# zzzzxxxx111/Rover-SLAM

Hardware: AMD Instinct MI355X
Metric: frames/s SuperPoint+LightGlue 640x480 (higher is better)
Workload: dtype f32; 1 GPU; configs[3] per GPU: 33 synthetic 640x480 u8 frames resident in HBM, SuperPoint extract (Kmax=1024, thr=0.0005) + LightGlue match of 32 consecutive pairs (9 layers, filter 0.1); 32 frames counted per GPU per step; seeded synthetic weights (centred descriptor head + calibrated LightGlue law, frames shifted by multiples of 8 px); the same resident frames every step (compute-bound path, no data-depend; frames_per_gpu=32, kmax=1024, lg_fold_wo=1, pairing=calibrated

## Files before the change

### include/rover_fe.h

```cpp
#ifndef ROVER_FE_H
#define ROVER_FE_H
#include <stddef.h>
#include <stdint.h>

#ifdef __cplusplus
extern "C" {
#endif

typedef struct rfe_ctx rfe_ctx;

typedef enum {
    RFE_OK = 0,
    RFE_ERR_INVALID = -1,
    RFE_ERR_NO_DEVICE = -2,
    RFE_ERR_HIP = -3,
    RFE_ERR_IO = -4,
    RFE_ERR_NO_WEIGHTS = -5,
    RFE_ERR_OOM = -6
} rfe_status;

#define RFE_DESC_DIM 256
#define RFE_KIND_SUPERPOINT 1
#define RFE_KIND_LIGHTGLUE 2

int rfe_init(int device, rfe_ctx** out);
void rfe_destroy(rfe_ctx* ctx);
const char* rfe_last_error(rfe_ctx* ctx);
const char* rfe_version(void);

int rfe_load_weights(rfe_ctx* ctx, const char* sp_path, const char* lg_path);
int rfe_load_onnx(rfe_ctx* ctx, const char* sp_path, const char* lg_path);
int rfe_set_weights(rfe_ctx* ctx, int kind, const float* blob, int64_t count);
int64_t rfe_weight_count(int kind);
uint64_t rfe_weights_id(rfe_ctx* ctx, int kind);

typedef struct rfe_hparams {
    int32_t sp_max_keypoints;
    float sp_detection_threshold;
    int32_t sp_nms_radius;
    int32_t sp_remove_borders;
    int32_t sp_topk_always;
    int32_t lg_layers;
    int32_t lg_heads;
    float lg_filter_threshold;
} rfe_hparams;
int rfe_get_hparams(rfe_ctx* ctx, rfe_hparams* out);
int rfe_set_hparams(rfe_ctx* ctx, const rfe_hparams* in);

#define RFE_OPT_LG_FOLD_WO 1
#define RFE_OPT_LG_FP16X2 2
#define RFE_OPT_HOST_GRAPH 3
int rfe_set_option(rfe_ctx* ctx, int option, int value);
int rfe_get_option(rfe_ctx* ctx, int option, int* value);

int rfe_set_stream(rfe_ctx* ctx, void* hip_stream);
int rfe_synchronize(rfe_ctx* ctx);
int rfe_malloc(rfe_ctx* ctx, size_t bytes, void** dev_ptr);
int rfe_free(rfe_ctx* ctx, void* dev_ptr);
int rfe_host_malloc(size_t bytes, void** host_ptr);
void rfe_host_free(void* host_ptr);
int64_t rfe_workspace_bytes(rfe_ctx* ctx);
int rfe_memcpy_h2d(rfe_ctx* ctx, void* dst_dev, const void* src_host, size_t bytes);
int rfe_memcpy_d2h(rfe_ctx* ctx, void* dst_host, const void* src_dev, size_t bytes);

int rfe_extract_u8(rfe_ctx* ctx, const uint8_t* img, int H, int W, int stride, int B, int Kmax,
                   float thr, int32_t* n, int32_t* kxy, float* score, float* desc);
int rfe_extract_u8_dev(rfe_ctx* ctx, const uint8_t* img_dev, int H, int W, int stride, int B,
                       int Kmax, float thr, int32_t* n_dev, int32_t* kxy_dev, float* score_dev,
                       float* desc_dev);

int rfe_extract_f32(rfe_ctx* ctx, const float* img, int H, int W, int stride, int B, int Kmax,
                    float thr, int32_t* n, int32_t* kxy, float* score, float* desc);
int rfe_extract_f32_dev(rfe_ctx* ctx, const float* img_dev, int H, int W, int stride, int B,
                        int Kmax, float thr, int32_t* n_dev, int32_t* kxy_dev, float* score_dev,
                        float* desc_dev);

int rfe_extract_u8_bin(rfe_ctx* ctx, const uint8_t* img, int H, int W, int stride, int B, int Kmax, float thr, int32_t* n,
                       int32_t* kxy, float* score, float* desc, uint8_t* desc_bin);
int rfe_extract_u8_bin_dev(rfe_ctx* ctx, const uint8_t* img_dev, int H, int W, int stride, int B, int Kmax, float thr,
                           int32_t* n_dev, int32_t* kxy_dev, float* score_dev, float* desc_dev, uint8_t* desc_bin_dev);

#define RFE_MAX_LEVELS 16
int rfe_pyramid_geometry(int H, int W, int nlevels, float scale_factor, int32_t* level_h, int32_t* level_w, float* level_scale);
int rfe_extract_pyramid_u8(rfe_ctx* ctx, const uint8_t* img, int H, int W, int stride, int B, int nlevels, float scale_factor,
                           const int32_t* kmax, float thr, int32_t* n, int32_t* level_n, float* kpts, int32_t* octave,
                           float* score, float* desc, uint8_t* levels);
int rfe_extract_pyramid_u8_dev(rfe_ctx* ctx, const uint8_t* img_dev, int H, int W, int stride, int B, int nlevels, float scale_factor,
                               const int32_t* kmax, float thr, int32_t* n_dev, int32_t* level_n_dev, float* kpts_dev,
                               int32_t* octave_dev, float* score_dev, float* desc_dev, uint8_t* levels_dev);

int rfe_match(rfe_ctx* ctx, const float* k0n, const float* k1n, const float* d0, const float* d1,
              const int32_t* m, const int32_t* n, int P, int Mmax, int Nmax, float filter_thr,
              int32_t* S, int32_t* pairs, float* ms);
int rfe_match_dev(rfe_ctx* ctx, const float* k0n, const float* k1n, const float* d0,
                  const float* d1, const int32_t* m, const int32_t* n, int P, int Mmax, int Nmax,
                  float filter_thr, int32_t* S, int32_t* pairs, float* ms);

int rfe_match_fused(rfe_ctx* ctx, const float* kpts0_xy, int M, const float* kpts1_xy, int N,
                    const float* desc0, const float* desc1, int rows, int cols, float filter_thr,
                    float match_thresh, int32_t* vnMatches12);

int rfe_extract_match_stream_dev(rfe_ctx* ctx, const uint8_t* img_dev, int H, int W, int stride,
                                 int B, int Kmax, float thr, float filter_thr, int32_t* n_dev,
                                 int32_t* kxy_dev, float* score_dev, float* desc_dev,
                                 int32_t* S_dev, int32_t* pairs_dev, float* ms_dev);

int rfe_stereo_match(rfe_ctx* ctx, const uint8_t* imgL, const uint8_t* imgR, int H, int W, int stride,
                     const float* kL, int N, const float* kR, int Nr, const float* dL, const float* dR,
                     float mb, float mbf, float* uRight, float* depth);
int rfe_stereo_match_dev(rfe_ctx* ctx, const uint8_t* imgL, const uint8_t* imgR, int H, int W, int stride,
                         const float* kL, int N, const float* kR, int Nr, const float* dL, const float* dR,
                         float mb, float mbf, float* uRight, float* depth);

int rfe_stereo_frame_dev(rfe_ctx* ctx, const uint8_t* imgL_dev, const uint8_t* imgR_dev, int H, int W, int stride, int Kmax,
                         float thr, float filter_thr, float mb, float mbf, int reset, int32_t* n_dev, int32_t* kxy_dev,
                         float* score_dev, float* desc_dev, float* uRight_dev, float* depth_dev, int32_t* S_dev,
                         int32_t* pairs_dev, float* ms_dev);

#define RFE_STEREO_SAD_LEVEL  0
#define RFE_STEREO_SAD_LEVEL0 1
int rfe_stereo_match_pyramid(rfe_ctx* ctx, const uint8_t* levelsL, const uint8_t* levelsR, int H, int W, int nlevels, float scale_factor,
                             const float* kL, const int32_t* octL, int N, const float* kR, const int32_t* octR, int Nr,
                             const float* dL, const float* dR, float mb, float mbf, int sad_source, float* uRight, float* depth);
int rfe_stereo_match_pyramid_dev(rfe_ctx* ctx, const uint8_t* levelsL, const uint8_t* levelsR, int H, int W, int nlevels, float scale_factor,
                                 const float* kL, const int32_t* octL, int N, const float* kR, const int32_t* octR, int Nr,
                                 const float* dL, const float* dR, float mb, float mbf, int sad_source, float* uRight, float* depth);
int rfe_stereo_frame_pyramid_dev(rfe_ctx* ctx, const uint8_t* imgL_dev, const uint8_t* imgR_dev, int H, int W, int stride,
                                 int nlevels, float scale_factor, const int32_t* kmax, float thr, float filter_thr, float mb, float mbf,
                                 int sad_source, int reset, int32_t* n_dev, int32_t* level_n_dev, float* kpts_dev, int32_t* octave_dev,
                                 float* score_dev, float* desc_dev, float* uRight_dev, float* depth_dev, int32_t* S_dev,
                                 int32_t* pairs_dev, float* ms_dev);

int rfe_l2_distance_matrix(rfe_ctx* ctx, const float* a, int M, const float* b, int N, float* out);
int rfe_binarize_descriptors(rfe_ctx* ctx, const float* desc, int rows, uint8_t* out);

int rfe_search_candidates(rfe_ctx* ctx, const float* q, int Nq, const float* f, int Nf, const int32_t* offsets,
                          const int32_t* cand, const uint8_t* skip, int32_t* best_idx, float* best_dist, float* second_dist);
int rfe_distinctive_descriptors(rfe_ctx* ctx, const float* desc, const int32_t* offsets, int Np, int32_t* best, float* median);

int rfe_l2_distance_matrix_dev(rfe_ctx* ctx, const float* a_dev, int M, const float* b_dev, int N, float* out_dev);
int rfe_binarize_descriptors_dev(rfe_ctx* ctx, const float* desc_dev, int rows, uint8_t* out_dev);
int rfe_search_candidates_dev(rfe_ctx* ctx, const float* q_dev, int Nq, const float* f_dev, int Nf, const int32_t* offsets_dev,
                              const int32_t* cand_dev, const uint8_t* skip_dev, int32_t* best_idx_dev, float* best_dist_dev,
                              float* second_dist_dev);
int rfe_distinctive_descriptors_dev(rfe_ctx* ctx, const float* desc_dev, const int32_t* offsets_dev, int Np, int total, int maxn,
                                    int32_t* best_dev, float* median_dev);

int rfe_search_by_projection_dev(rfe_ctx* ctx, const float* q_dev, const float* proj_dev, const float* radius_dev,
                                 const int32_t* pred_level_dev, const uint8_t* observed_dev, int Nq, const float* f_dev,
                                 const float* kpts_dev, const int32_t* kxy_dev, const int32_t* octave_dev, const uint8_t* skip_dev, int Nf,
                                 const int32_t* nf_dev, float min_x, float min_y, float max_x, float max_y, float th_high, int cand_cap,
                                 int32_t* assign_dev, int32_t* best_idx_dev, float* best_dist_dev, float* second_dist_dev,
                                 int32_t* stats_dev);
int rfe_search_by_projection(rfe_ctx* ctx, const float* q, const float* proj, const float* radius, const int32_t* pred_level,
                             const uint8_t* observed, int Nq, const float* f, const float* kpts, const int32_t* kxy, const int32_t* octave,
                             const uint8_t* skip, int Nf, float min_x, float min_y, float max_x, float max_y, float th_high,
                             int32_t* assign, int32_t* best_idx, float* best_dist, float* second_dist, int32_t* stats);

typedef struct rfe_pool rfe_pool;
#define RFE_POOL_AUTO 0
#define RFE_POOL_RCCL 1
#define RFE_POOL_COPY 2
int rfe_pool_create(const int* devices, int n, rfe_pool** out);
void rfe_pool_destroy(rfe_pool* pool);
const char* rfe_pool_last_error(rfe_pool* pool);
int rfe_pool_size(rfe_pool* pool);
rfe_ctx* rfe_pool_ctx(rfe_pool* pool, int member);
int rfe_pool_has_rccl(rfe_pool* pool);
int rfe_pool_set_weights(rfe_pool* pool, int kind, const float* blob, int64_t count);
int rfe_pool_load_weights(rfe_pool* pool, const char* sp_path, const char* lg_path);
int rfe_pool_set_option(rfe_pool* pool, int option, int value);
int rfe_pool_set_hparams(rfe_pool* pool, const rfe_hparams* in);
int rfe_pool_shard(int F, int n, int member, int* first_frame, int* frames, int* pairs);
int rfe_pool_extract_match_stream(rfe_pool* pool, const uint8_t* img_host, int H, int W, int stride, int F, int Kmax, float thr,
                                  float filter_thr, int transport, int32_t* n, int32_t* kxy, float* score, float* desc,
                                  int32_t* S, int32_t* pairs, float* ms);

int rfe_profile_enable(rfe_ctx* ctx, int on);
int rfe_profile_filter(rfe_ctx* ctx, const char* stage);
int rfe_profile_reset(rfe_ctx* ctx);
int rfe_profile_read(rfe_ctx* ctx, char* names, size_t names_cap, double* ms, int64_t* calls, int cap);

int rfe_k_conv3x3(rfe_ctx* ctx, const float* in_dev, int B, int H, int W, int Cin,
                  const float* w_oihw_host, const float* bias_host, int Cout, int relu, int pool,
                  float* out_dev);
int rfe_k_linear(rfe_ctx* ctx, const float* a_dev, int M, int K, const float* w_nk_host,
                 const float* bias_host, int N, int relu, float* out_dev);
int rfe_k_scoremap(rfe_ctx* ctx, const uint8_t* img_dev, int H, int W, int stride, int B,
                   float* scoremap_dev ,
                   float* nms_dev , float* descmap_dev );
int rfe_k_select(rfe_ctx* ctx, const float* nms_dev , int B, int H, int W, int Kmax, float thr, int topk_always,
                 int32_t* n_dev, int32_t* kxy_dev, float* score_dev);
int rfe_k_select_keys(rfe_ctx* ctx, const float* nms_dev , int B, int H, int W, int Kmax, float thr, int topk_always,
                      int32_t* n_dev, int32_t* kxy_dev, float* score_dev);
int rfe_k_lightglue_taps(rfe_ctx* ctx, const float* k0n, const float* k1n, const float* d0,
                         const float* d1, int M, int N, float* x0_dev, float* x1_dev,
                         float* scores_dev );

int rfe_k_lightglue_ffn(rfe_ctx* ctx, int layer, int cross, const float* x_dev, const float* second_dev, int rows, float* out_dev);
int rfe_k_attention(rfe_ctx* ctx, const float* q_dev, const float* k_dev, const float* v_dev, int ld, float* out_dev, int nseq, int Lq, int Lk,
                    const int32_t* qlen_dev, const int32_t* klen_dev, const int32_t* kv_map_dev, const float* rope_dev);
int rfe_k_lightglue_self_attention(rfe_ctx* ctx, int layer, const float* x_dev, const float* csn_dev, const int32_t* lens_dev, int nseq, int L,
                                   float* qkv_out_dev, float* ctx_out_dev, int32_t* qk_rotated);
int rfe_k_set_lightglue_tap(rfe_ctx* ctx, int pair, float* x0_dev, float* x1_dev, float* scores_dev);
int rfe_k_pool_inject_gather_failure(rfe_pool* pool, int member);
int rfe_k_onnx_convert(const char* path, int kind, int weights_only, float* blob, rfe_hparams* hp, char* err, int errlen);

#ifdef __cplusplus
}
#endif
#endif
```

### rover-slam_amd/capi.py

```python
import ctypes as C
import os

import numpy as np

_HERE = os.path.dirname(os.path.abspath(__file__))
LIB_PATH = os.environ.get("RFE_LIBRARY") or os.path.join(_HERE, "librover_fe.so")

KIND_SUPERPOINT, KIND_LIGHTGLUE = 1, 2
OPT_LG_FOLD_WO = 1
OPT_LG_FP16X2 = 2
OPT_HOST_GRAPH = 3

EXPORTS = [
    "rfe_init", "rfe_destroy", "rfe_last_error", "rfe_version", "rfe_load_weights", "rfe_load_onnx", "rfe_set_weights",
    "rfe_weight_count", "rfe_weights_id", "rfe_get_hparams", "rfe_set_hparams", "rfe_set_option", "rfe_get_option", "rfe_set_stream", "rfe_synchronize", "rfe_malloc", "rfe_free", "rfe_host_malloc", "rfe_host_free", "rfe_workspace_bytes", "rfe_memcpy_h2d",
    "rfe_memcpy_d2h", "rfe_extract_u8", "rfe_extract_u8_dev", "rfe_extract_f32", "rfe_extract_f32_dev", "rfe_extract_u8_bin", "rfe_extract_u8_bin_dev",
    "rfe_pyramid_geometry", "rfe_extract_pyramid_u8", "rfe_extract_pyramid_u8_dev", "rfe_match", "rfe_match_dev", "rfe_match_fused",
    "rfe_extract_match_stream_dev", "rfe_stereo_match", "rfe_stereo_match_dev", "rfe_stereo_frame_dev", "rfe_stereo_match_pyramid", "rfe_stereo_match_pyramid_dev", "rfe_stereo_frame_pyramid_dev",
    "rfe_l2_distance_matrix", "rfe_binarize_descriptors",
    "rfe_search_candidates", "rfe_distinctive_descriptors",
    "rfe_l2_distance_matrix_dev", "rfe_binarize_descriptors_dev", "rfe_search_candidates_dev", "rfe_distinctive_descriptors_dev",
    "rfe_search_by_projection", "rfe_search_by_projection_dev",
    "rfe_pool_create", "rfe_pool_destroy", "rfe_pool_last_error", "rfe_pool_size", "rfe_pool_ctx", "rfe_pool_has_rccl", "rfe_pool_set_weights",
    "rfe_pool_load_weights", "rfe_pool_set_option", "rfe_pool_set_hparams", "rfe_pool_shard", "rfe_pool_extract_match_stream",
    "rfe_profile_enable", "rfe_profile_filter", "rfe_profile_reset", "rfe_profile_read",
    "rfe_k_conv3x3", "rfe_k_linear", "rfe_k_scoremap", "rfe_k_select", "rfe_k_select_keys", "rfe_k_lightglue_taps", "rfe_k_set_lightglue_tap", "rfe_k_lightglue_ffn", "rfe_k_attention", "rfe_k_lightglue_self_attention", "rfe_k_pool_inject_gather_failure", "rfe_k_onnx_convert",
]

if not os.path.exists(LIB_PATH):
    raise ImportError(f"{LIB_PATH} is missing: build it with `python -c 'import __graft_entry__ as g; g.build()'` "
                      "(rover-slam_amd/csrc/Makefile). There is no CPU fallback.")

lib = C.CDLL(LIB_PATH)

_vp, _fp, _ip, _u8p = C.c_void_p, C.c_void_p, C.c_void_p, C.c_void_p
lib.rfe_init.argtypes = [C.c_int, C.POINTER(C.c_void_p)]
lib.rfe_destroy.argtypes = [C.c_void_p]
lib.rfe_destroy.restype = None
lib.rfe_last_error.argtypes = [C.c_void_p]
lib.rfe_last_error.restype = C.c_char_p
lib.rfe_version.restype = C.c_char_p
lib.rfe_load_weights.argtypes = [C.c_void_p, C.c_char_p, C.c_char_p]
lib.rfe_set_weights.argtypes = [C.c_void_p, C.c_int, _fp, C.c_int64]
lib.rfe_weight_count.argtypes = [C.c_int]
lib.rfe_weight_count.restype = C.c_int64
lib.rfe_weights_id.restype = C.c_uint64
lib.rfe_weights_id.argtypes = [C.c_void_p, C.c_int]


class HParams(C.Structure):
    _fields_ = [("sp_max_keypoints", C.c_int32), ("sp_detection_threshold", C.c_float), ("sp_nms_radius", C.c_int32),
                ("sp_remove_borders", C.c_int32), ("sp_topk_always", C.c_int32), ("lg_layers", C.c_int32), ("lg_heads", C.c_int32), ("lg_filter_threshold", C.c_float)]

    def as_dict(self):
        return {k: getattr(self, k) for k, _ in self._fields_}


lib.rfe_get_hparams.argtypes = [C.c_void_p, C.POINTER(HParams)]
lib.rfe_set_hparams.argtypes = [C.c_void_p, C.POINTER(HParams)]
lib.rfe_pool_set_hparams.argtypes = [C.c_void_p, C.POINTER(HParams)]
lib.rfe_set_option.argtypes = [C.c_void_p, C.c_int, C.c_int]
lib.rfe_get_option.argtypes = [C.c_void_p, C.c_int, C.POINTER(C.c_int)]
lib.rfe_set_stream.argtypes = [C.c_void_p, C.c_void_p]
lib.rfe_synchronize.argtypes = [C.c_void_p]
lib.rfe_malloc.argtypes = [C.c_void_p, C.c_size_t, C.POINTER(C.c_void_p)]
lib.rfe_free.argtypes = [C.c_void_p, C.c_void_p]
lib.rfe_memcpy_h2d.argtypes = [C.c_void_p, C.c_void_p, C.c_void_p, C.c_size_t]
lib.rfe_memcpy_d2h.argtypes = [C.c_void_p, C.c_void_p, C.c_void_p, C.c_size_t]
_ext = [C.c_void_p, _u8p, C.c_int, C.c_int, C.c_int, C.c_int, C.c_int, C.c_float, _ip, _ip, _fp, _fp]
lib.rfe_extract_u8.argtypes = _ext
lib.rfe_extract_f32.argtypes = _ext
lib.rfe_extract_f32_dev.argtypes = _ext
lib.rfe_extract_u8_dev.argtypes = _ext
lib.rfe_extract_u8_bin.argtypes = _ext + [_u8p]
lib.rfe_extract_u8_bin_dev.argtypes = _ext + [_u8p]
lib.rfe_pyramid_geometry.argtypes = [C.c_int, C.c_int, C.c_int, C.c_float, _ip, _ip, _fp]
_pyr = [C.c_void_p, _u8p, C.c_int, C.c_int, C.c_int, C.c_int, C.c_int, C.c_float, _ip, C.c_float, _ip, _ip, _fp, _ip, _fp, _fp, _u8p]
lib.rfe_extract_pyramid_u8.argtypes = _pyr
lib.rfe_extract_pyramid_u8_dev.argtypes = _pyr
_mt = [C.c_void_p, _fp, _fp, _fp, _fp, _ip, _ip, C.c_int, C.c_int, C.c_int, C.c_float, _ip, _ip, _fp]
lib.rfe_match.argtypes = _mt
lib.rfe_match_dev.argtypes = _mt
lib.rfe_match_fused.argtypes = [C.c_void_p, _fp, C.c_int, _fp, C.c_int, _fp, _fp, C.c_int, C.c_int, C.c_float,
                                C.c_float, _ip]
lib.rfe_extract_match_stream_dev.argtypes = [C.c_void_p, _u8p, C.c_int, C.c_int, C.c_int, C.c_int, C.c_int, C.c_float,
                                             C.c_float, _ip, _ip, _fp, _fp, _ip, _ip, _fp]
_st = [C.c_void_p, _u8p, _u8p, C.c_int, C.c_int, C.c_int, _fp, C.c_int, _fp, C.c_int, _fp, _fp, C.c_float, C.c_float, _fp, _fp]
lib.rfe_stereo_match.argtypes = _st
lib.rfe_stereo_match_dev.argtypes = _st
lib.rfe_stereo_frame_dev.argtypes = [C.c_void_p, _u8p, _u8p, C.c_int, C.c_int, C.c_int, C.c_int, C.c_float, C.c_float, C.c_float, C.c_float,
                                     C.c_int, _ip, _ip, _fp, _fp, _fp, _fp, _ip, _ip, _fp]
_stp = [C.c_void_p, _u8p, _u8p, C.c_int, C.c_int, C.c_int, C.c_float, _fp, _ip, C.c_int, _fp, _ip, C.c_int, _fp, _fp, C.c_float, C.c_float,
        C.c_int, _fp, _fp]
lib.rfe_stereo_match_pyramid.argtypes = _stp
lib.rfe_stereo_match_pyramid_dev.argtypes = _stp
lib.rfe_stereo_frame_pyramid_dev.argtypes = [C.c_void_p, _u8p, _u8p, C.c_int, C.c_int, C.c_int, C.c_int, C.c_float, _ip, C.c_float, C.c_float,
                                             C.c_float, C.c_float, C.c_int, C.c_int, _ip, _ip, _fp, _ip, _fp, _fp, _fp, _fp, _ip, _ip, _fp]
lib.rfe_l2_distance_matrix.argtypes = [C.c_void_p, _fp, C.c_int, _fp, C.c_int, _fp]
lib.rfe_binarize_descriptors.argtypes = [C.c_void_p, _fp, C.c_int, _u8p]
lib.rfe_search_candidates.argtypes = [C.c_void_p, _fp, C.c_int, _fp, C.c_int, _ip, _ip, _u8p, _ip, _fp, _fp]
lib.rfe_distinctive_descriptors.argtypes = [C.c_void_p, _fp, _ip, C.c_int, _ip, _fp]
lib.rfe_l2_distance_matrix_dev.argtypes = [C.c_void_p, _fp, C.c_int, _fp, C.c_int, _fp]
lib.rfe_binarize_descriptors_dev.argtypes = [C.c_void_p, _fp, C.c_int, _u8p]
lib.rfe_search_candidates_dev.argtypes = [C.c_void_p, _fp, C.c_int, _fp, C.c_int, _ip, _ip, _u8p, _ip, _fp, _fp]
lib.rfe_distinctive_descriptors_dev.argtypes = [C.c_void_p, _fp, _ip, C.c_int, C.c_int, C.c_int, _ip, _fp]
_psq = [C.c_void_p, _fp, _fp, _fp, _ip, _u8p, C.c_int, _fp, _fp, _ip, _ip, _u8p, C.c_int]
_psb = [C.c_float, C.c_float, C.c_float, C.c_float, C.c_float]
lib.rfe_search_by_projection.argtypes = _psq + _psb + [_ip, _ip, _fp, _fp, _ip]
lib.rfe_search_by_projection_dev.argtypes = _psq + [_ip] + _psb + [C.c_int, _ip, _ip, _fp, _fp, _ip]
lib.rfe_profile_enable.argtypes = [C.c_void_p, C.c_int]
lib.rfe_profile_filter.argtypes = [C.c_void_p, C.c_char_p]
lib.rfe_profile_reset.argtypes = [C.c_void_p]
lib.rfe_profile_read.argtypes = [C.c_void_p, C.c_char_p, C.c_size_t, C.POINTER(C.c_double), C.POINTER(C.c_int64), C.c_int]
lib.rfe_k_conv3x3.argtypes = [C.c_void_p, _fp, C.c_int, C.c_int, C.c_int, C.c_int, _fp, _fp, C.c_int, C.c_int, C.c_int, _fp]
lib.rfe_k_linear.argtypes = [C.c_void_p, _fp, C.c_int, C.c_int, _fp, _fp, C.c_int, C.c_int, _fp]
lib.rfe_k_scoremap.argtypes = [C.c_void_p, _u8p, C.c_int, C.c_int, C.c_int, C.c_int, _fp, _fp, _fp]
lib.rfe_k_select.argtypes = [C.c_void_p, _fp, C.c_int, C.c_int, C.c_int, C.c_int, C.c_float, C.c_int, _ip, _ip, _fp]
lib.rfe_k_select_keys.argtypes = lib.rfe_k_select.argtypes
lib.rfe_k_lightglue_taps.argtypes = [C.c_void_p, _fp, _fp, _fp, _fp, C.c_int, C.c_int, _fp, _fp, _fp]
lib.rfe_k_set_lightglue_tap.argtypes = [C.c_void_p, C.c_int, _fp, _fp, _fp]
lib.rfe_k_lightglue_ffn.argtypes = [C.c_void_p, C.c_int, C.c_int, _fp, _fp, C.c_int, _fp]
lib.rfe_k_lightglue_self_attention.argtypes = [C.c_void_p, C.c_int, _fp, _fp, C.c_void_p, C.c_int, C.c_int, _fp, _fp, C.POINTER(C.c_int32)]
lib.rfe_k_attention.argtypes = [C.c_void_p, _fp, _fp, _fp, C.c_int, _fp, C.c_int, C.c_int, C.c_int, C.c_void_p, C.c_void_p, C.c_void_p, _fp]


POOL_AUTO, POOL_RCCL, POOL_COPY = 0, 1, 2
lib.rfe_pool_create.argtypes = [C.POINTER(C.c_int), C.c_int, C.POINTER(C.c_void_p)]
lib.rfe_pool_destroy.argtypes = [C.c_void_p]
lib.rfe_pool_destroy.restype = None
lib.rfe_pool_last_error.argtypes = [C.c_void_p]
lib.rfe_pool_last_error.restype = C.c_char_p
lib.rfe_pool_size.argtypes = [C.c_void_p]
lib.rfe_pool_ctx.argtypes = [C.c_void_p, C.c_int]
lib.rfe_pool_ctx.restype = C.c_void_p
lib.rfe_pool_has_rccl.argtypes = [C.c_void_p]
lib.rfe_k_pool_inject_gather_failure.argtypes = [C.c_void_p, C.c_int]
lib.rfe_load_onnx.argtypes = [C.c_void_p, C.c_char_p, C.c_char_p]
lib.rfe_k_onnx_convert.argtypes = [C.c_char_p, C.c_int, C.c_int, C.POINTER(C.c_float), C.c_void_p, C.c_char_p, C.c_int]
lib.rfe_host_malloc.argtypes = [C.c_size_t, C.POINTER(C.c_void_p)]
lib.rfe_host_free.argtypes = [C.c_void_p]
lib.rfe_host_free.restype = None
lib.rfe_workspace_bytes.argtypes = [C.c_void_p]
lib.rfe_workspace_bytes.restype = C.c_int64
lib.rfe_pool_set_weights.argtypes = [C.c_void_p, C.c_int, _fp, C.c_int64]
lib.rfe_pool_load_weights.argtypes = [C.c_void_p, C.c_char_p, C.c_char_p]
lib.rfe_pool_set_option.argtypes = [C.c_void_p, C.c_int, C.c_int]
lib.rfe_pool_shard.argtypes = [C.c_int, C.c_int, C.c_int, C.POINTER(C.c_int), C.POINTER(C.c_int), C.POINTER(C.c_int)]
lib.rfe_pool_extract_match_stream.argtypes = [C.c_void_p, _u8p, C.c_int, C.c_int, C.c_int, C.c_int, C.c_int, C.c_float, C.c_float, C.c_int,
                                              _ip, _ip, _fp, _fp, _ip, _ip, _fp]


class RfeError(RuntimeError):
    pass


def _addr(a):
    if a is None:
        return None
    if isinstance(a, int):
        return a
    if isinstance(a, np.ndarray):
        assert a.flags["C_CONTIGUOUS"]
        return a.ctypes.data
    if hasattr(a, "data_ptr"):
        return a.data_ptr()
    raise TypeError(type(a))


class DevBuf:

    def __init__(self, ctx, nbytes):
        self.ctx, self.nbytes = ctx, int(nbytes)
        p = C.c_void_p()
        ctx._chk(lib.rfe_malloc(ctx.h, self.nbytes, C.byref(p)))
        self.ptr = p.value

    def upload(self, arr):
        arr = np.ascontiguousarray(arr)
        assert arr.nbytes <= self.nbytes
        self.ctx._chk(lib.rfe_memcpy_h2d(self.ctx.h, self.ptr, arr.ctypes.data, arr.nbytes))
        return self

    def download(self, shape, dtype):
        out = np.empty(shape, dtype)
        assert out.nbytes <= self.nbytes
        self.ctx._chk(lib.rfe_memcpy_d2h(self.ctx.h, out.ctypes.data, self.ptr, out.nbytes))
        return out

    def free(self):
        if self.ptr:
            lib.rfe_free(self.ctx.h, self.ptr)
            self.ptr = None


def split_levels(flat, level_h, level_w):
    out, off = [], 0
    for h, w in zip(level_h, level_w):
        out.append(flat[:, off:off + int(h) * int(w)].reshape(flat.shape[0], int(h), int(w)))
        off += int(h) * int(w)
    return out


class StereoStream:

    def __init__(self, ctx, H, W, kmax=1024, mb=0.11, mbf=0.11 * 435.0, thr=0.0005, filter_thr=0.1):
        self.ctx, self.H, self.W, self.K = ctx, H, W, kmax
        self.mb, self.mbf, self.thr, self.filter_thr = mb, mbf, thr, filter_thr
        K = kmax
        self._spec = [("n", np.int32, (2,)), ("kxy", np.int32, (2, K, 2)), ("score", np.float32, (2, K)), ("desc", np.float32, (2, K, 256)),
                      ("u_right", np.float32, (K,)), ("depth", np.float32, (K,)), ("S", np.int32, (1,)), ("pairs", np.int32, (K, 2)),
                      ("ms", np.float32, (K,))]
        self.bufs = {name: ctx.alloc(int(np.prod(shape)) * np.dtype(dt).itemsize) for name, dt, shape in self._spec}
        self.first = True

    def push(self, img_l_dev, img_r_dev, stride=None, reset=False):
        b = self.bufs
        self.ctx._chk(lib.rfe_stereo_frame_dev(self.ctx.h, _addr(img_l_dev), _addr(img_r_dev), self.H, self.W, stride or self.W, self.K,
                                               self.thr, self.filter_thr, self.mb, self.mbf, int(reset or self.first), b["n"].ptr,
                                               b["kxy"].ptr, b["score"].ptr, b["desc"].ptr, b["u_right"].ptr, b["depth"].ptr,
                                               b["S"].ptr, b["pairs"].ptr, b["ms"].ptr))
        self.first = False

    def results(self):
        self.ctx.synchronize()
        out = {name: self.bufs[name].download(shape, dt) for name, dt, shape in self._spec}
        out["S"] = int(out["S"][0])
        return out

    def close(self):
        for b in self.bufs.values():
            b.free()
        self.bufs = {}


STEREO_SAD_LEVEL, STEREO_SAD_LEVEL0 = 0, 1


class StereoPyramidStream:

    def __init__(self, ctx, H, W, nlevels=8, scale_factor=1.2, kmax=128, mb=0.11, mbf=0.11 * 435.0, thr=0.0005, filter_thr=0.1,
                 sad_source=STEREO_SAD_LEVEL):
        self.ctx, self.H, self.W, self.L, self.sf = ctx, H, W, int(nlevels), scale_factor
        self.kmax = np.full((max(self.L, 1),), int(kmax), np.int32) if np.isscalar(kmax) else np.ascontiguousarray(kmax, np.int32)
        self.mb, self.mbf, self.thr, self.filter_thr, self.sad_source = mb, mbf, thr, filter_thr, sad_source
        K = self.K = int(self.kmax.sum())
        self._spec = [("n", np.int32, (2,)), ("level_n", np.int32, (2, max(self.L, 1))), ("kpts", np.float32, (2, K, 2)),
                      ("octave", np.int32, (2, K)), ("score", np.float32, (2, K)), ("desc", np.float32, (2, K, 256)),
                      ("u_right", np.float32, (K,)), ("depth", np.float32, (K,)), ("S", np.int32, (1,)), ("pairs", np.int32, (K, 2)),
                      ("ms", np.float32, (K,))]
        self.bufs = {name: ctx.alloc(max(int(np.prod(shape)), 1) * np.dtype(dt).itemsize) for name, dt, shape in self._spec}
        self.first = True

    def push(self, img_l_dev, img_r_dev, stride=None, reset=False):
        b = self.bufs
        self.ctx._chk(lib.rfe_stereo_frame_pyramid_dev(self.ctx.h, _addr(img_l_dev), _addr(img_r_dev), self.H, self.W, stride or self.W, self.L,
                                                       self.sf, self.kmax.ctypes.data, self.thr, self.filter_thr, self.mb, self.mbf,
                                                       self.sad_source, int(reset or self.first), b["n"].ptr, b["level_n"].ptr, b["kpts"].ptr,
                                                       b["octave"].ptr, b["score"].ptr, b["desc"].ptr, b["u_right"].ptr, b["depth"].ptr,
                                                       b["S"].ptr, b["pairs"].ptr, b["ms"].ptr))
        self.first = False

    def results(self):
        self.ctx.synchronize()
        out = {name: self.bufs[name].download(shape, dt) for name, dt, shape in self._spec}
        out["S"] = int(out["S"][0])
        return out

    def close(self):
        for b in self.bufs.values():
            b.free()
        self.bufs = {}


MAX_LEVELS = 16


def pyramid_geometry(H, W, nlevels, scale_factor):
    L = max(int(nlevels), 1)
    h, w, s = np.zeros((L,), np.int32), np.zeros((L,), np.int32), np.zeros((L,), np.float32)
    rc = lib.rfe_pyramid_geometry(H, W, nlevels, scale_factor, h.ctypes.data, w.ctypes.data, s.ctypes.data)
    if rc < 0:
        raise RfeError(f"rfe_pyramid_geometry({H}, {W}, {nlevels}, {scale_factor}) failed ({rc})")
    return h, w, s


def pool_shard(F, n, member):
    a, b, c = C.c_int(), C.c_int(), C.c_int()
    rc = lib.rfe_pool_shard(F, n, member, C.byref(a), C.byref(b), C.byref(c))
    if rc < 0:
        raise RfeError(f"rfe_pool_shard({F}, {n}, {member}) failed ({rc})")
    return a.value, b.value, c.value


class Pool:

    def __init__(self, devices):
        devs = (C.c_int * len(devices))(*devices)
        h = C.c_void_p()
        rc = lib.rfe_pool_create(devs, len(devices), C.byref(h))
        if rc != 0:
            raise RfeError(f"rfe_pool_create failed ({rc}): {lib.rfe_pool_last_error(None).decode()}")
        self.h = h

    def close(self):
        if self.h:
            lib.rfe_pool_destroy(self.h)
            self.h = None

    def __del__(self):
        try:
            self.close()
        except Exception:
            pass

    def _chk(self, rc):
        if rc < 0:
            raise RfeError(f"librover_fe pool error {rc}: {lib.rfe_pool_last_error(self.h).decode()}")
        return rc

    @property
    def size(self):
        return lib.rfe_pool_size(self.h)

    @property
    def has_rccl(self):
        return bool(lib.rfe_pool_has_rccl(self.h))

    def set_weights(self, kind, blob):
        blob = np.ascontiguousarray(blob, np.float32)
        self._chk(lib.rfe_pool_set_weights(self.h, kind, blob.ctypes.data, blob.size))

    def set_option(self, option, value):
        self._chk(lib.rfe_pool_set_option(self.h, option, int(value)))

    def set_hparams(self, **kw):
        h = HParams()
        rc = lib.rfe_get_hparams(lib.rfe_pool_ctx(self.h, 0), C.byref(h))
        if rc < 0:
            raise RfeError(f"rfe_get_hparams on pool member 0 failed ({rc})")
        for k, v in kw.items():
            if not hasattr(h, k):
                raise KeyError(k)
            setattr(h, k, v)
        self._chk(lib.rfe_pool_set_hparams(self.h, C.byref(h)))

    def extract_match_stream(self, frames_u8, kmax=1024, thr=0.0005, filter_thr=0.1, transport=POOL_AUTO, with_desc=True):
        img = np.ascontiguousarray(frames_u8, np.uint8)
        F, H, W = img.shape
        P = max(F - 1, 1)
        out = {"n": np.zeros((F,), np.int32), "kxy": np.zeros((F, kmax, 2), np.int32), "S": np.zeros((P,), np.int32),
               "pairs": np.zeros((P, kmax, 2), np.int32), "ms": np.zeros((P, kmax), np.float32)}
        if with_desc:
            out["score"] = np.zeros((F, kmax), np.float32)
            out["desc"] = np.zeros((F, kmax, 256), np.float32)
        self._chk(lib.rfe_pool_extract_match_stream(self.h, img.ctypes.data, H, W, W, F, kmax, thr, filter_thr, transport, out["n"].ctypes.data,
                                                    out["kxy"].ctypes.data, out["score"].ctypes.data if with_desc else None,
                                                    out["desc"].ctypes.data if with_desc else None, out["S"].ctypes.data,
                                                    out["pairs"].ctypes.data, out["ms"].ctypes.data))
        return out


class Context:

    def __init__(self, device=0):
        h = C.c_void_p()
        rc = lib.rfe_init(device, C.byref(h))
        if rc != 0:
            raise RfeError(f"rfe_init failed ({rc}): {lib.rfe_last_error(None).decode()}")
        self.h = h

    def close(self):
        if self.h:
            lib.rfe_destroy(self.h)
            self.h = None

    def __del__(self):
        try:
            self.close()
        except Exception:
            pass

    def _chk(self, rc):
        if rc < 0:
            raise RfeError(f"librover_fe error {rc}: {lib.rfe_last_error(self.h).decode()}")
        return rc

    def set_weights(self, kind, blob):
        blob = np.ascontiguousarray(blob, np.float32)
        self._chk(lib.rfe_set_weights(self.h, kind, blob.ctypes.data, blob.size))

    def load_weights(self, sp_path=None, lg_path=None):
        self._chk(lib.rfe_load_weights(self.h, sp_path.encode() if sp_path else None, lg_path.encode() if lg_path else None))

    def get_hparams(self):
        h = HParams()
        self._chk(lib.rfe_get_hparams(self.h, C.byref(h)))
        return h.as_dict()

    def set_hparams(self, **kw):
        h = HParams()
        self._chk(lib.rfe_get_hparams(self.h, C.byref(h)))
        for k, v in kw.items():
            if not hasattr(h, k):
                raise KeyError(k)
            setattr(h, k, v)
        self._chk(lib.rfe_set_hparams(self.h, C.byref(h)))

    def set_option(self, option, value):
        self._chk(lib.rfe_set_option(self.h, option, int(value)))

    def get_option(self, option):
        v = C.c_int()
        self._chk(lib.rfe_get_option(self.h, option, C.byref(v)))
        return v.value

    def set_stream(self, stream_ptr):
        self._chk(lib.rfe_set_stream(self.h, stream_ptr))

    def workspace_bytes(self):
        return int(lib.rfe_workspace_bytes(self.h))

    def synchronize(self):
        self._chk(lib.rfe_synchronize(self.h))

    def alloc(self, nbytes):
        return DevBuf(self, nbytes)

    def extract(self, img_u8, kmax=1024, thr=0.0005, pad_cols=0, binarized=False):
        img = np.ascontiguousarray(img_u8, np.uint8)
        if img.ndim == 2:
            img = img[None]
        B, H, W = img.shape
        stride = W + pad_cols
        if pad_cols:
            wide = np.full((B, H, stride), 255, np.uint8)
            wide[:, :, :W] = img
            img = wide
        n = np.zeros((B,), np.int32)
        kxy = np.zeros((B, kmax, 2), np.int32)
        score = np.zeros((B, kmax), np.float32)
        desc = np.zeros((B, kmax, 256), np.float32)
        if binarized:
            dbin = np.zeros((B, kmax, 256), np.uint8)
            self._chk(lib.rfe_extract_u8_bin(self.h, img.ctypes.data, H, W, stride, B, kmax, thr, n.ctypes.data, kxy.ctypes.data,
                                             score.ctypes.data, desc.ctypes.data, dbin.ctypes.data))
            return n, kxy, score, desc, dbin
        self._chk(lib.rfe_extract_u8(self.h, img.ctypes.data, H, W, stride, B, kmax, thr, n.ctypes.data, kxy.ctypes.data,
                                     score.ctypes.data, desc.ctypes.data))
        return n, kxy, score, desc

    def extract_pyramid(self, frames_u8, nlevels=8, scale_factor=1.2, kmax=1024, thr=0.0005, with_levels=False, pad_cols=0):
        img = np.ascontiguousarray(frames_u8, np.uint8)
        if img.ndim == 2:
            img = img[None]
        B, H, W = img.shape
        stride = W + pad_cols
        if pad_cols:
            wide = np.full((B, H, stride), 255, np.uint8)
            wide[:, :, :W] = img
            img = wide
        L = int(nlevels)
        km = np.full((max(L, 1),), int(kmax), np.int32) if np.isscalar(kmax) else np.ascontiguousarray(kmax, np.int32)
        K = int(km.sum())
        out = {"n": np.zeros((B,), np.int32), "level_n": np.zeros((B, max(L, 1)), np.int32), "kpts": np.zeros((B, K, 2), np.float32),
               "octave": np.zeros((B, K), np.int32), "score": np.zeros((B, K), np.float32), "desc": np.zeros((B, K, 256), np.float32)}
        lv = None
        if with_levels:
            lh, lw, _ = pyramid_geometry(H, W, L, scale_factor)
            lv = np.zeros((B, int((lh.astype(np.int64) * lw).sum())), np.uint8)
        self._chk(lib.rfe_extract_pyramid_u8(self.h, img.ctypes.data, H, W, stride, B, L, scale_factor, km.ctypes.data, thr,
                                             out["n"].ctypes.data, out["level_n"].ctypes.data, out["kpts"].ctypes.data,
                                             out["octave"].ctypes.data, out["score"].ctypes.data, out["desc"].ctypes.data,
                                             None if lv is None else lv.ctypes.data))
        if with_levels:
            out["levels"] = split_levels(lv, lh, lw)
        return out

    def extract_f32(self, img_f32, kmax=1024, thr=0.0005):
        img = np.ascontiguousarray(img_f32, np.float32)
        if img.ndim == 2:
            img = img[None]
        B, H, W = img.shape
        n = np.zeros((B,), np.int32)
        kxy = np.zeros((B, kmax, 2), np.int32)
        score = np.zeros((B, kmax), np.float32)
        desc = np.zeros((B, kmax, 256), np.float32)
        self._chk(lib.rfe_extract_f32(self.h, img.ctypes.data, H, W, W, B, kmax, thr, n.ctypes.data, kxy.ctypes.data,
                                      score.ctypes.data, desc.ctypes.data))
        return n, kxy, score, desc

    def match(self, k0n, k1n, d0, d1, m, n, filter_thr=0.1):
        k0n = np.ascontiguousarray(k0n, np.float32); k1n = np.ascontiguousarray(k1n, np.float32)
        d0 = np.ascontiguousarray(d0, np.float32); d1 = np.ascontiguousarray(d1, np.float32)
        m = np.ascontiguousarray(m, np.int32); n = np.ascontiguousarray(n, np.int32)
        P, Mmax = k0n.shape[0], k0n.shape[1]
        Nmax = k1n.shape[1]
        cap = min(Mmax, Nmax)
        S = np.zeros((P,), np.int32)
        pairs = np.zeros((P, cap, 2), np.int32)
        ms = np.zeros((P, cap), np.float32)
        self._chk(lib.rfe_match(self.h, k0n.ctypes.data, k1n.ctypes.data, d0.ctypes.data, d1.ctypes.data, m.ctypes.data,
                                n.ctypes.data, P, Mmax, Nmax, filter_thr, S.ctypes.data, pairs.ctypes.data, ms.ctypes.data))
        return S, pairs, ms

    def match_fused(self, kpts0, kpts1, desc0, desc1, rows, cols, filter_thr=0.1, match_thresh=0.0):
        kpts0 = np.ascontiguousarray(kpts0, np.float32).reshape(-1, 2)
        kpts1 = np.ascontiguousarray(kpts1, np.float32).reshape(-1, 2)
        desc0 = np.ascontiguousarray(desc0, np.float32); desc1 = np.ascontiguousarray(desc1, np.float32)
        M, N = kpts0.shape[0], kpts1.shape[0]
        vn = np.full((max(M, 1),), -1, np.int32)
        size = self._chk(lib.rfe_match_fused(self.h, kpts0.ctypes.data, M, kpts1.ctypes.data, N, desc0.ctypes.data,
                                             desc1.ctypes.data, rows, cols, filter_thr, match_thresh, vn.ctypes.data))
        return size, vn[:M]

    def stereo_match(self, img_l, img_r, k_l, k_r, d_l, d_r, mb, mbf):
        il = np.ascontiguousarray(img_l, np.uint8); ir = np.ascontiguousarray(img_r, np.uint8)
        kl = np.ascontiguousarray(k_l, np.float32).reshape(-1, 2); kr = np.ascontiguousarray(k_r, np.float32).reshape(-1, 2)
        dl = np.ascontiguousarray(d_l, np.float32); dr = np.ascontiguousarray(d_r, np.float32)
        H, W = il.shape
        N, Nr = kl.shape[0], kr.shape[0]
        u = np.full((max(N, 1),), -1, np.float32); z = np.full((max(N, 1),), -1, np.float32)
        self._chk(lib.rfe_stereo_match(self.h, il.ctypes.data, ir.ctypes.data, H, W, W, kl.ctypes.data, N, kr.ctypes.data, Nr,
                                       dl.ctypes.data, dr.ctypes.data, mb, mbf, u.ctypes.data, z.ctypes.data))
        return u[:N], z[:N]

    def stereo_match_pyramid(self, levels_l, levels_r, H, W, nlevels, scale_factor, k_l, oct_l, k_r, oct_r, d_l, d_r, mb, mbf, sad_source=0):
        def flat(lv):
            if isinstance(lv, (list, tuple)):
                return np.concatenate([np.ascontiguousarray(a, np.uint8).reshape(-1) for a in lv])
            return np.ascontiguousarray(lv, np.uint8).reshape(-1)
        vl, vr = flat(levels_l), flat(levels_r)
        lh, lw, _ = pyramid_geometry(H, W, nlevels, scale_factor)
        need = int((lh.astype(np.int64) * lw).sum())
        if vl.size != need or vr.size != need:
            raise RfeError(f"stereo_match_pyramid: level buffers hold {vl.size} / {vr.size} bytes, the geometry needs {need}")
        kl = np.ascontiguousarray(k_l, np.float32).reshape(-1, 2); kr = np.ascontiguousarray(k_r, np.float32).reshape(-1, 2)
        ol = np.ascontiguousarray(oct_l, np.int32).reshape(-1); orr = np.ascontiguousarray(oct_r, np.int32).reshape(-1)
        dl = np.ascontiguousarray(d_l, np.float32).reshape(-1, 256); dr = np.ascontiguousarray(d_r, np.float32).reshape(-1, 256)
        N, Nr = kl.shape[0], kr.shape[0]
        assert ol.shape[0] == N and orr.shape[0] == Nr and dl.shape[0] == N and dr.shape[0] == Nr
        u = np.full((max(N, 1),), -1, np.float32); z = np.full((max(N, 1),), -1, np.float32)
        self._chk(lib.rfe_stereo_match_pyramid(self.h, vl.ctypes.data, vr.ctypes.data, H, W, nlevels, scale_factor, kl.ctypes.data,
                                               ol.ctypes.data, N, kr.ctypes.data, orr.ctypes.data, Nr, dl.ctypes.data, dr.ctypes.data,
                                               mb, mbf, sad_source, u.ctypes.data, z.ctypes.data))
        return u[:N], z[:N]

    def search_candidates(self, q, f, offsets, cand, skip=None):
        qa = np.ascontiguousarray(q, np.float32).reshape(-1, 256); fa = np.ascontiguousarray(f, np.float32).reshape(-1, 256)
        off = np.ascontiguousarray(offsets, np.int32); cd = np.ascontiguousarray(cand, np.int32)
        sk = None if skip is None else np.ascontiguousarray(skip, np.uint8)
        Nq = qa.shape[0]
        bi = np.empty((max(Nq, 1),), np.int32); bd = np.empty((max(Nq, 1),), np.float32); sd = np.empty((max(Nq, 1),), np.float32)
        self._chk(lib.rfe_search_candidates(self.h, qa.ctypes.data, Nq, fa.ctypes.data, fa.shape[0], off.ctypes.data,
                                            cd.ctypes.data, None if sk is None else sk.ctypes.data, bi.ctypes.data,
                                            bd.ctypes.data, sd.ctypes.data))
        return bi[:Nq], bd[:Nq], sd[:Nq]

    def search_by_projection(self, q, proj, radius, f, bounds, kpts=None, kxy=None, pred_level=None, observed=None, octave=None, skip=None,
                             th_high=1.4):
        qa = np.ascontiguousarray(q, np.float32).reshape(-1, 256); fa = np.ascontiguousarray(f, np.float32).reshape(-1, 256)
        pa = np.ascontiguousarray(proj, np.float32).reshape(-1, 2); ra = np.ascontiguousarray(radius, np.float32).reshape(-1)
        Nq, Nf = qa.shape[0], fa.shape[0]
        assert pa.shape[0] == Nq and ra.shape[0] == Nq
        opt = lambda a, dt, n: None if a is None else np.ascontiguousarray(a, dt).reshape(-1)
        ka, xa = opt(kpts, np.float32, Nf), opt(kxy, np.int32, Nf)
        lv, ob = opt(pred_level, np.int32, Nq), opt(observed, np.uint8, Nq)
        oc, sk = opt(octave, np.int32, Nf), opt(skip, np.uint8, Nf)
        asg = np.full((max(Nf, 1),), -1, np.int32); st = np.zeros((4,), np.int32)
        bi = np.full((max(Nq, 1),), -1, np.int32); bd = np.full((max(Nq, 1),), 256, np.float32); sd = np.full((max(Nq, 1),), 256, np.float32)
        n = self._chk(lib.rfe_search_by_projection(self.h, qa.ctypes.data, pa.ctypes.data, ra.ctypes.data, _addr(lv), _addr(ob), Nq,
                                                   fa.ctypes.data, _addr(ka), _addr(xa), _addr(oc), _addr(sk), Nf, *[float(b) for b in bounds],
                                                   th_high, asg.ctypes.data, bi.ctypes.data, bd.ctypes.data, sd.ctypes.data, st.ctypes.data))
        return {"assign": asg[:Nf], "best_idx": bi[:Nq], "best_dist": bd[:Nq], "second_dist": sd[:Nq], "nmatches": n, "stats": st}

    def search_by_projection_dev(self, q, proj, radius, Nq, f, Nf, bounds, cand_cap, assign, stats, kpts=None, kxy=None, pred_level=None,
                                 observed=None, octave=None, skip=None, nf_dev=None, th_high=1.4, best_idx=None, best_dist=None,
                                 second_dist=None):
        a = lambda x: x.ptr if isinstance(x, DevBuf) else _addr(x)
        self._chk(lib.rfe_search_by_projection_dev(self.h, a(q), a(proj), a(radius), a(pred_level), a(observed), Nq, a(f), a(kpts), a(kxy),
                                                   a(octave), a(skip), Nf, a(nf_dev), *[float(b) for b in bounds], th_high, cand_cap,
                                                   a(assign), a(best_idx), a(best_dist), a(second_dist), a(stats)))

    def distinctive_descriptors(self, desc, offsets):
        da = np.ascontiguousarray(desc, np.float32).reshape(-1, 256)
        off = np.ascontiguousarray(offsets, np.int32)
        Np = off.shape[0] - 1
        b = np.empty((max(Np, 1),), np.int32); m = np.empty((max(Np, 1),), np.float32)
        self._chk(lib.rfe_distinctive_descriptors(self.h, da.ctypes.data, off.ctypes.data, Np, b.ctypes.data, m.ctypes.data))
        return b[:Np], m[:Np]

    def profile(self, on=True):
        self._chk(lib.rfe_profile_enable(self.h, int(on)))

    def profile_filter(self, stage=None):
        self._chk(lib.rfe_profile_filter(self.h, stage.encode() if stage else None))

    def profile_reset(self):
        self._chk(lib.rfe_profile_reset(self.h))

    def profile_read(self):
        names = C.create_string_buffer(4096)
        ms = (C.c_double * 64)()
        calls = (C.c_int64 * 64)()
        k = self._chk(lib.rfe_profile_read(self.h, names, 4096, ms, calls, 64))
        nm = names.value.decode().split(";") if k else []
        return {nm[i]: (ms[i], calls[i]) for i in range(k)}
```

### rover-slam_amd/csrc/api_extract.hip

```cpp
#include <string.h>
#include "api_internal.h"

using namespace rfe;

namespace rfe {

static void sp_layout(Bump& a, int B, int H, int W, SpBuffers& b) {
    const size_t hw = (size_t)B * H * W, cells = hw / 64;
    b.p1 = a.take<float>(hw / 4 * 64); b.a2 = a.take<float>(hw / 4 * 64);
    b.p2 = a.take<float>(hw / 16 * 64); b.a3 = a.take<float>(hw / 16 * 128);
    b.p3 = a.take<float>(cells * 128); b.a4 = a.take<float>(cells * 128); b.f4 = a.take<float>(cells * 128);
    b.pa = a.take<float>(cells * 256); b.da = a.take<float>(cells * 256); b.dmap = a.take<float>(cells * 256);
    b.logits = a.take<float>(cells * 65);
    b.smap = a.take<float>(hw); b.nmap = a.take<float>(hw); b.ss = a.take<float>(hw);
    b.mask = a.take<uint8_t>(hw); b.supp = a.take<uint8_t>(hw);
    b.cand_score = a.take<float>(hw); b.cand_idx = a.take<int32_t>(hw);
    b.sel_keys = a.take<unsigned long long>((size_t)B * 4096); b.sel_n = a.take<int32_t>(B);
}
size_t sp_ws_bytes(int B, int H, int W) { SpBuffers b; return layout_bytes([&](Bump& a) { sp_layout(a, B, H, W, b); }); }
int sp_carve(rfe_ctx* c, int B, int H, int W, SpBuffers& b) {
    return ws_carve(c, &c->ws_sp, &c->ws_sp_bytes, [&](Bump& a) { sp_layout(a, B, H, W, b); });
}

GemmArgs gemm_plain(const float* A, int lda, const float* Bw, int ldb, const float* bias, float* C, int ldc, int M, int N, int K) {
    GemmArgs g;
    memset(&g, 0, sizeof(g));
    g.A = A; g.lda = lda; g.B = Bw; g.ldb = ldb; g.bias = bias; g.C = C; g.ldc = ldc;
    g.M = M; g.N = N; g.K = K; g.alpha = 1.0f; g.batch = 1;
    return g;
}

int sp_check(rfe_ctx* c, int H, int W, int B, int Kmax) {
    if (!c) return RFE_ERR_INVALID;
    if (!c->has_sp) return fail(c, RFE_ERR_NO_WEIGHTS, "SuperPoint weights not loaded (rfe_load_weights / rfe_set_weights)");
    if (H < 8 || W < 8 || B <= 0) return fail(c, RFE_ERR_INVALID, "extract: H and W must be at least 8, B > 0");
    if (Kmax <= 0 || Kmax > 4096) return fail(c, RFE_ERR_INVALID, "extract: Kmax must be in 1..4096");
    return RFE_OK;
}

int sp_forward_maps(rfe_ctx* c, const void* img, int H, int W, int stride, int B, SpBuffers& b, bool join, bool& forked, bool img_f32, long long frame_step,
                    float thr, bool want_maps) {
    forked = false;
    int rc = sp_carve(c, B, H, W, b);
    if (rc) return rc;
    hipStream_t s = c->stream;
    const SpWeightsDev& w = c->sp;
    const int H1 = H / 2, W1 = W / 2, H2 = H1 / 2, W2 = W1 / 2, Hc = H2 / 2, Wc = W2 / 2, cells = B * Hc * Wc;
    { ProfScope p(c, "conv1ab");
      launch_conv1ab_fused(s, img, img_f32, stride, B, H, W, w.conv1a_w, w.bias[L_1A], w.packed[L_1B], w.bias[L_1B], b.p1, frame_step); }
    { ProfScope p(c, "conv2a"); launch_conv3x3(s, b.p1, B, H1, W1, 64, w.packed[L_2A], w.bias[L_2A], 64, true, kSpLayers[L_2A].pool, b.a2, L_2A); }
    { ProfScope p(c, "conv2b"); launch_conv3x3(s, b.a2, B, H1, W1, 64, w.packed[L_2B], w.bias[L_2B], 64, true, kSpLayers[L_2B].pool, b.p2, L_2B); }
    { ProfScope p(c, "conv3a"); launch_conv3x3(s, b.p2, B, H2, W2, 64, w.packed[L_3A], w.bias[L_3A], 128, true, kSpLayers[L_3A].pool, b.a3, L_3A); }
    { ProfScope p(c, "conv3b"); launch_conv3x3(s, b.a3, B, H2, W2, 128, w.packed[L_3B], w.bias[L_3B], 128, true, kSpLayers[L_3B].pool, b.p3, L_3B); }
    { ProfScope p(c, "conv4a"); launch_conv3x3(s, b.p3, B, Hc, Wc, 128, w.packed[L_4A], w.bias[L_4A], 128, true, kSpLayers[L_4A].pool, b.a4, L_4A); }
    { ProfScope p(c, "conv4b"); launch_conv3x3(s, b.a4, B, Hc, Wc, 128, w.packed[L_4B], w.bias[L_4B], 128, true, kSpLayers[L_4B].pool, b.f4, L_4B); }
    const bool fork = !(c->prof && c->prof_filter.empty());
    hipStream_t sd = fork ? c->side_stream : s;
    if (fork) { RFE_HIP(c, hipEventRecord(c->ev_fork, s)); RFE_HIP(c, hipStreamWaitEvent(sd, c->ev_fork, 0)); }
    { ProfScope p(c, "convDa", sd); launch_conv3x3(sd, b.f4, B, Hc, Wc, 128, w.packed[L_DA], w.bias[L_DA], 256, true, kSpLayers[L_DA].pool, b.da, L_DA); }
    { ProfScope p(c, "convDb", sd); launch_gemm_nt(sd, gemm_plain(b.da, 256, w.packed[L_DB], 256, w.bias[L_DB], b.dmap, 256, cells, 256, 256)); }
    { ProfScope p(c, "sp_post", sd); launch_descmap_norm(sd, b.dmap, cells); }
    if (fork) RFE_HIP(c, hipEventRecord(c->ev_join, sd));
    { ProfScope p(c, "convPa"); launch_conv3x3(s, b.f4, B, Hc, Wc, 128, w.packed[L_PA], w.bias[L_PA], 256, true, kSpLayers[L_PA].pool, b.pa, L_PA); }
    { ProfScope p(c, "convPb"); launch_gemm_nt(s, gemm_plain(b.pa, 256, w.packed[L_PB], 256, w.bias[L_PB], b.logits, 65, cells, 65, 256)); }
    { ProfScope p(c, "sp_post");
      if (B <= 4 && c->hp.sp_nms_radius == 4) {
          if (!c->sp_cnt) { RFE_HIP(c, hipMalloc((void**)&c->sp_cnt, 8 * sizeof(int32_t))); c->sp_cnt_dirty = true; }
          if (c->sp_cnt_dirty) { RFE_HIP(c, hipMemsetAsync(c->sp_cnt, 0, 8 * sizeof(int32_t), s)); c->sp_cnt_dirty = false; }
          b.tail_fused = launch_sp_tail_lat(s, b.logits, B, Hc, Wc, c->hp.sp_nms_radius, c->hp.sp_remove_borders, thr, (unsigned long long*)b.cand_score, c->sp_cnt,
                                            want_maps ? b.smap : nullptr, want_maps ? b.nmap : nullptr);
          if (b.tail_fused) c->sp_cnt_dirty = true;
      }
      if (!b.tail_fused) {
          launch_softmax65_d2s(s, b.logits, 65, B, Hc, Wc, b.smap);
          launch_nms(s, b.smap, B, 8 * Hc, 8 * Wc, c->hp.sp_nms_radius, c->hp.sp_remove_borders, b.ss, b.mask, b.supp, b.nmap);
      } }
    if (fork && join) RFE_HIP(c, hipStreamWaitEvent(s, c->ev_join, 0));
    forked = fork && !join;
    RFE_HIP(c, hipGetLastError());
    return RFE_OK;
}

int sp_forward(rfe_ctx* c, const void* img, int H, int W, int stride, int B, int Kmax, float thr,
               int32_t* n, int32_t* kxy, float* score, float* desc, uint8_t* desc_bin, bool img_f32, long long frame_step) {
    SpBuffers b;
    bool forked;
    int rc = sp_forward_maps(c, img, H, W, stride, B, b, false, forked, img_f32, frame_step, thr);
    if (rc) return rc;
    const int Hc = H / 2 / 2 / 2, Wc = W / 2 / 2 / 2, Hs = 8 * Hc, Ws = 8 * Wc;
    { ProfScope p(c, "sp_select");
      if (b.tail_fused) {
          launch_select_keys(c->stream, (const unsigned long long*)b.cand_score, c->sp_cnt, B, Hs, Ws, Kmax, c->hp.sp_topk_always != 0, n, kxy, score);
          c->sp_cnt_dirty = false;
      } else
      launch_select(c->stream, b.nmap, B, Hs, Ws, Kmax, thr, b.cand_score, b.cand_idx, n, kxy, score, (int32_t*)b.ss , c->hp.sp_topk_always != 0, b.sel_keys, b.sel_n);
      if (forked) RFE_HIP(c, hipStreamWaitEvent(c->stream, c->ev_join, 0));
      launch_desc_sample(c->stream, b.dmap, B, Hc, Wc, Hs, Ws, n, kxy, Kmax, desc, desc_bin); }
    RFE_HIP(c, hipGetLastError());
    return RFE_OK;
}

}

static int extract_check(rfe_ctx* c, const void* img, int H, int W, int stride, int B, int Kmax, const void* n, const void* kxy, const void* score,
                         const void* desc) {
    int rc = sp_check(c, H, W, B, Kmax);
    if (rc) return rc;
    if (!img || !n || !kxy || !score || !desc || stride < W) return fail(c, RFE_ERR_INVALID, "extract: null pointer or stride < W");
    RFE_HIP(c, hipSetDevice(c->device));
    return RFE_OK;
}

extern "C" int rfe_extract_u8_bin_dev(rfe_ctx* c, const uint8_t* img, int H, int W, int stride, int B, int Kmax,
                                      float thr, int32_t* n, int32_t* kxy, float* score, float* desc, uint8_t* desc_bin) {
    int rc = extract_check(c, img, H, W, stride, B, Kmax, n, kxy, score, desc);
    if (rc) return rc;
    return sp_forward(c, img, H, W, stride, B, Kmax, thr, n, kxy, score, desc, desc_bin);
}

extern "C" int rfe_extract_u8_dev(rfe_ctx* c, const uint8_t* img, int H, int W, int stride, int B, int Kmax,
                                  float thr, int32_t* n, int32_t* kxy, float* score, float* desc) {
    return rfe_extract_u8_bin_dev(c, img, H, W, stride, B, Kmax, thr, n, kxy, score, desc, nullptr);
}

extern "C" int rfe_extract_f32_dev(rfe_ctx* c, const float* img, int H, int W, int stride, int B, int Kmax,
                                   float thr, int32_t* n, int32_t* kxy, float* score, float* desc) {
    int rc = extract_check(c, img, H, W, stride, B, Kmax, n, kxy, score, desc);
    if (rc) return rc;
    return sp_forward(c, img, H, W, stride, B, Kmax, thr, n, kxy, score, desc, nullptr, true);
}

static int extract_host(rfe_ctx* c, const void* img, size_t px, int H, int W, int stride, int B, int Kmax, float thr, int32_t* n, int32_t* kxy,
                        float* score, float* desc, uint8_t* desc_bin) {
    int rc = extract_check(c, img, H, W, stride, B, Kmax, n, kxy, score, desc);
    if (rc) return rc;
    const size_t K = (size_t)B * Kmax;
    uint8_t *d_img, *d_b; int32_t *d_n, *d_k; float *d_s, *d_d;
    HostIo io(c, HostIo::PINNED);
    io.image(d_img, (const uint8_t*)img, (size_t)W * px, (size_t)B * H, (size_t)stride * px);
    io.out(d_n, n, B); io.out(d_k, kxy, K * 2); io.out(d_s, score, K);
    io.out(d_d, desc, K * 256, true);
    io.out_opt(d_b, desc_bin, K * 256);
    if ((rc = io.upload())) return rc;
    if ((rc = ensure_ws(c, &c->ws_sp, &c->ws_sp_bytes, sp_ws_bytes(B, H, W)))) return rc;
    int thr_bits; memcpy(&thr_bits, &thr, 4);
    const std::string key = px == 1 ? host_graph_key(c, "xu8", {H, W, B, Kmax, thr_bits, desc_bin != nullptr}) : host_graph_key(c, "xf32", {H, W, B, Kmax, thr_bits});
    if ((rc = run_host_graph(c, c->g_extract, key, [&] { return sp_forward(c, d_img, H, W, W, B, Kmax, thr, d_n, d_k, d_s, d_d, d_b, px == 4); }))) return rc;
    return io.download();
}

extern "C" int rfe_extract_u8(rfe_ctx* c, const uint8_t* img, int H, int W, int stride, int B, int Kmax, float thr,
                              int32_t* n, int32_t* kxy, float* score, float* desc) {
    return extract_host(c, img, 1, H, W, stride, B, Kmax, thr, n, kxy, score, desc, nullptr);
}
extern "C" int rfe_extract_u8_bin(rfe_ctx* c, const uint8_t* img, int H, int W, int stride, int B, int Kmax, float thr,
                                  int32_t* n, int32_t* kxy, float* score, float* desc, uint8_t* desc_bin) {
    return extract_host(c, img, 1, H, W, stride, B, Kmax, thr, n, kxy, score, desc, desc_bin);
}
extern "C" int rfe_extract_f32(rfe_ctx* c, const float* img, int H, int W, int stride, int B, int Kmax, float thr,
                               int32_t* n, int32_t* kxy, float* score, float* desc) {
    return extract_host(c, img, 4, H, W, stride, B, Kmax, thr, n, kxy, score, desc, nullptr);
}

extern "C" int rfe_pyramid_geometry(int H, int W, int nlevels, float scale_factor, int32_t* level_h, int32_t* level_w, float* level_scale) {
    return pyramid_geometry(H, W, nlevels, scale_factor, level_h, level_w, level_scale);
}

namespace rfe {

int pyr_check(rfe_ctx* c, int H, int W, int stride, int B, int L, float sf, const int32_t* kmax, PyrPlan& P) {
    if (!c) return RFE_ERR_INVALID;
    if (!c->has_sp) return fail(c, RFE_ERR_NO_WEIGHTS, "SuperPoint weights not loaded (rfe_load_weights / rfe_set_weights)");
    if (L < 1 || L > RFE_MAX_LEVELS) return fail(c, RFE_ERR_INVALID, "extract_pyramid: nlevels must be in 1..16");
    if (L > 1 && !(sf > 1.0f && sf <= 4.0f)) return fail(c, RFE_ERR_INVALID, "extract_pyramid: scale_factor must be in (1, 4] when nlevels > 1");
    if (H < 8 || W < 8 || B < 1 || stride < W) return fail(c, RFE_ERR_INVALID, "extract_pyramid: H and W must be at least 8, B > 0, stride >= W");
    if (!kmax) return fail(c, RFE_ERR_INVALID, "extract_pyramid: null pointer");
    P.L = L; P.Ktot = 0;
    for (int l = 0; l < L; ++l) {
        if (kmax[l] < 0 || kmax[l] > 4096) return fail(c, RFE_ERR_INVALID, "extract_pyramid: every kmax[l] must be in 0..4096");
        P.kmax[l] = kmax[l]; P.Ktot += kmax[l];
    }
    if (P.Ktot == 0) return fail(c, RFE_ERR_INVALID, "extract_pyramid: every kmax[l] is 0");
    if (pyramid_geometry(H, W, L, sf, P.h, P.w, P.s) != RFE_OK) return fail(c, RFE_ERR_INVALID, "extract_pyramid: a level rounds to zero pixels");
    P.frame = 0;
    for (int l = 0; l < L; ++l) {
        P.off[l] = P.frame; P.frame += (size_t)P.h[l] * P.w[l];
        P.run[l] = P.kmax[l] > 0 && P.h[l] >= 8 && P.w[l] >= 8;
    }
    return RFE_OK;
}

struct PyrStage { uint8_t* levels; int32_t *n[RFE_MAX_LEVELS], *kxy[RFE_MAX_LEVELS]; float *sc[RFE_MAX_LEVELS], *desc[RFE_MAX_LEVELS]; };
static void pyr_layout(Bump& a, const PyrPlan& P, int B, bool own_levels, PyrStage& st) {
    st.levels = own_levels ? a.take<uint8_t>((size_t)B * P.frame) : nullptr;
    for (int l = 0; l < P.L; ++l) {
        if (!P.run[l]) continue;
        st.n[l] = a.take<int32_t>((size_t)B); st.kxy[l] = a.take<int32_t>((size_t)B * P.kmax[l] * 2);
        st.sc[l] = a.take<float>((size_t)B * P.kmax[l]); st.desc[l] = a.take<float>((size_t)B * P.kmax[l] * 256);
    }
}

int pyr_prepare(rfe_ctx* c, int H, int W, int B, float sf, const PyrPlan& P, bool own_levels) {
    int rc;
    if ((rc = ensure_ws(c, &c->ws_sp, &c->ws_sp_bytes, sp_ws_bytes(B, H, W)))) return rc;
    PyrStage st;
    if ((rc = ensure_ws(c, &c->ws_pyr, &c->ws_pyr_bytes, layout_bytes([&](Bump& a) { pyr_layout(a, P, B, own_levels, st); })))) return rc;
    if (!c->sp_cnt) { RFE_HIP(c, hipMalloc((void**)&c->sp_cnt, 8 * sizeof(int32_t))); c->sp_cnt_dirty = true; }
    int sf_bits; memcpy(&sf_bits, &sf, 4);
    const std::string key = std::to_string(H) + "x" + std::to_string(W) + "|" + std::to_string(P.L) + "|" + std::to_string(P.L > 1 ? sf_bits : 0);
    if (P.L > 1 && key != c->ptab_key) {
        std::vector<int2> tab;
        pyramid_tables(P.L, P.h, P.w, tab, c->ptab_off);
        c->ptab_key.clear();
        const void* before = c->ws_ptab;
        if ((rc = ensure_ws(c, &c->ws_ptab, &c->ws_ptab_bytes, tab.size() * sizeof(int2)))) return rc;
        if (before == c->ws_ptab) RFE_HIP(c, hipStreamSynchronize(c->stream));
        RFE_HIP(c, hipMemcpy(c->ws_ptab, tab.data(), tab.size() * sizeof(int2), hipMemcpyHostToDevice));
        c->ptab_key = key;
    }
    return RFE_OK;
}

int pyr_forward(rfe_ctx* c, const uint8_t* img, int H, int W, int stride, int B, const PyrPlan& P, float thr, uint8_t* lv, bool copy_level0,
                int32_t* n, int32_t* level_n, float* kpts, int32_t* octave, float* score, float* desc, long long img_frame) {
    if (img_frame == 0) img_frame = (long long)stride * H;
    hipStream_t s = c->stream;
    const bool side = !(c->prof && c->prof_filter.empty());
    hipStream_t sc = side ? c->side_stream : s;
    if (side) { RFE_HIP(c, hipEventRecord(c->ev_fork, s)); RFE_HIP(c, hipStreamWaitEvent(sc, c->ev_fork, 0)); }
    { ProfScope p(c, "sp_pyramid", sc);
      if (copy_level0) launch_pyr_resample(sc, img, img_frame, stride, H, W, lv, (long long)P.frame, H, W, B, nullptr, nullptr);
      const int2* tab = (const int2*)c->ws_ptab;
      for (int l = 1; l < P.L; ++l) {
          const uint8_t* src = l == 1 ? img : lv + P.off[l - 1];
          const long long src_frame = l == 1 ? img_frame : (long long)P.frame;
          const int src_stride = l == 1 ? stride : P.w[l - 1];
          launch_pyr_resample(sc, src, src_frame, src_stride, P.h[l - 1], P.w[l - 1], lv + P.off[l], (long long)P.frame, P.h[l], P.w[l], B,
                              tab + c->ptab_off[l], tab + c->ptab_off[l] + P.w[l]);
      } }
    if (side) RFE_HIP(c, hipEventRecord(c->ev_pyr, sc));
    PyrMergeArgs m;
    memset(&m, 0, sizeof(m));
    m.L = P.L; m.Ktot = P.Ktot;
    PyrStage st;
    Bump a(c->ws_pyr);
    pyr_layout(a, P, B, lv == (uint8_t*)c->ws_pyr, st);
    int rc;
    bool joined = !side;
    for (int l = 0; l < P.L; ++l) {
        m.kmax[l] = P.kmax[l]; m.scale[l] = P.s[l];
        if (!P.run[l]) continue;
        int32_t* ln = st.n[l]; int32_t* lk = st.kxy[l]; float* ls = st.sc[l]; float* ld = st.desc[l];
        if (l >= 1 && !joined) { RFE_HIP(c, hipStreamWaitEvent(s, c->ev_pyr, 0)); joined = true; }
        if (l == 0) rc = sp_forward(c, img, H, W, stride, B, P.kmax[0], thr, ln, lk, ls, ld, nullptr, false, img_frame);
        else rc = sp_forward(c, lv + P.off[l], P.h[l], P.w[l], P.w[l], B, P.kmax[l], thr, ln, lk, ls, ld, nullptr, false, (long long)P.frame);
        if (rc) return rc;
        m.n[l] = ln; m.kxy[l] = lk; m.sc[l] = ls; m.desc_l[l] = ld;
    }
    if (!joined) RFE_HIP(c, hipStreamWaitEvent(s, c->ev_pyr, 0));
    m.n_out = n; m.level_n = level_n; m.kpts = kpts; m.octave = octave; m.score = score; m.desc = desc;
    { ProfScope p(c, "sp_merge"); launch_pyr_merge(s, m, B); }
    RFE_HIP(c, hipGetLastError());
    return RFE_OK;
}

}

static int pyr_entry_check(rfe_ctx* c, const void* img, int H, int W, int stride, int B, int nlevels, float scale_factor, const int32_t* kmax, const void* n,
                           const void* kpts, const void* octave, const void* score, const void* desc, PyrPlan& P) {
    int rc = pyr_check(c, H, W, stride, B, nlevels, scale_factor, kmax, P);
    if (rc) return rc;
    if (!img || !n || !kpts || !octave || !score || !desc) return fail(c, RFE_ERR_INVALID, "extract_pyramid: null pointer");
    RFE_HIP(c, hipSetDevice(c->device));
    return RFE_OK;
}

extern "C" int rfe_extract_pyramid_u8_dev(rfe_ctx* c, const uint8_t* img, int H, int W, int stride, int B, int nlevels, float scale_factor,
                                          const int32_t* kmax, float thr, int32_t* n, int32_t* level_n, float* kpts, int32_t* octave,
                                          float* score, float* desc, uint8_t* levels) {
    PyrPlan P;
    int rc = pyr_entry_check(c, img, H, W, stride, B, nlevels, scale_factor, kmax, n, kpts, octave, score, desc, P);
    if (rc) return rc;
    if ((rc = pyr_prepare(c, H, W, B, scale_factor, P, levels == nullptr))) return rc;
    return pyr_forward(c, img, H, W, stride, B, P, thr, levels ? levels : (uint8_t*)c->ws_pyr, levels != nullptr, n, level_n, kpts, octave,
                       score, desc);
}

extern "C" int rfe_extract_pyramid_u8(rfe_ctx* c, const uint8_t* img, int H, int W, int stride, int B, int nlevels, float scale_factor,
                                      const int32_t* kmax, float thr, int32_t* n, int32_t* level_n, float* kpts, int32_t* octave,
                                      float* score, float* desc, uint8_t* levels) {
    PyrPlan P;
    int rc = pyr_entry_check(c, img, H, W, stride, B, nlevels, scale_factor, kmax, n, kpts, octave, score, desc, P);
    if (rc) return rc;
    const size_t K = (size_t)B * P.Ktot;
    uint8_t *d_img, *d_v; int32_t *d_n, *d_ln, *d_o; float *d_k, *d_s, *d_d;
    HostIo io(c, HostIo::PINNED);
    io.image(d_img, img, (size_t)W, (size_t)B * H, (size_t)stride);
    io.out(d_n, n, B); io.out(d_ln, level_n, (size_t)B * nlevels); io.out(d_k, kpts, K * 2); io.out(d_o, octave, K); io.out(d_s, score, K);
    io.out(d_d, desc, K * 256, true);
    io.out_opt(d_v, levels, (size_t)B * P.frame);
    if ((rc = pyr_prepare(c, H, W, B, scale_factor, P, levels == nullptr))) return rc;
    if ((rc = io.upload())) return rc;
    if ((rc = pyr_forward(c, d_img, H, W, W, B, P, thr, d_v ? d_v : (uint8_t*)c->ws_pyr, d_v != nullptr, d_n, d_ln, d_k, d_o, d_s, d_d))) return rc;
    return io.download();
}
```

### rover-slam_amd/csrc/api_hooks.hip

```cpp
#include <algorithm>
#include "api_internal.h"

using namespace rfe;

extern "C" int rfe_k_conv3x3(rfe_ctx* c, const float* in, int B, int H, int W, int Cin, const float* w, const float* bias,
                             int Cout, int relu, int pool, float* out) {
    if (!c) return RFE_ERR_INVALID;
    if ((Cin != 16 && Cin != 32 && Cin != 64 && Cin != 128) || (Cout % 64)) return fail(c, RFE_ERR_INVALID, "k_conv3x3: Cin in {16,32,64,128}, Cout % 64 == 0");
    RFE_HIP(c, hipSetDevice(c->device));
    std::vector<float> packed;
    pack_conv3x3_weights(w, Cin, Cout, pool != 0, packed);
    float *dw, *db;
    int rc = ws_carve(c, &c->ws_tmp, &c->ws_tmp_bytes, [&](Bump& a) { dw = a.take<float>(packed.size()); db = a.take<float>(Cout); });
    if (rc) return rc;
    RFE_HIP(c, hipMemcpyAsync(dw, packed.data(), packed.size() * 4, hipMemcpyHostToDevice, c->stream));
    RFE_HIP(c, hipMemcpyAsync(db, bias, (size_t)Cout * 4, hipMemcpyHostToDevice, c->stream));
    launch_conv3x3(c->stream, in, B, H, W, Cin, dw, db, Cout, relu != 0, pool != 0, out, 0);
    RFE_HIP(c, hipGetLastError());
    RFE_HIP(c, hipStreamSynchronize(c->stream));
    return RFE_OK;
}

extern "C" int rfe_k_linear(rfe_ctx* c, const float* a, int M, int K, const float* w, const float* bias, int N, int relu,
                            float* out) {
    if (!c) return RFE_ERR_INVALID;
    if (K % 32) return fail(c, RFE_ERR_INVALID, "k_linear: K % 32 == 0 required");
    RFE_HIP(c, hipSetDevice(c->device));
    float *dw, *db;
    int rc = ws_carve(c, &c->ws_tmp, &c->ws_tmp_bytes, [&](Bump& a) { dw = a.take<float>((size_t)N * K); db = a.take<float>(N); });
    if (rc) return rc;
    RFE_HIP(c, hipMemcpyAsync(dw, w, (size_t)N * K * 4, hipMemcpyHostToDevice, c->stream));
    if (bias) RFE_HIP(c, hipMemcpyAsync(db, bias, (size_t)N * 4, hipMemcpyHostToDevice, c->stream));
    GemmArgs g = gemm_plain(a, K, dw, K, bias ? db : nullptr, out, N, M, N, K);
    g.relu = relu;
    launch_gemm_nt(c->stream, g);
    RFE_HIP(c, hipGetLastError());
    RFE_HIP(c, hipStreamSynchronize(c->stream));
    return RFE_OK;
}

extern "C" int rfe_k_scoremap(rfe_ctx* c, const uint8_t* img, int H, int W, int stride, int B, float* scoremap,
                              float* nms, float* descmap) {
    int rc = sp_check(c, H, W, B, 1);
    if (rc) return rc;
    RFE_HIP(c, hipSetDevice(c->device));
    SpBuffers b;
    bool forked;
    if ((rc = sp_forward_maps(c, img, H, W, stride, B, b, true, forked, false, 0, 0.0005f, true))) return rc;
    const size_t hw = (size_t)B * (H / 8 * 8) * (W / 8 * 8);
    if (scoremap) RFE_HIP(c, hipMemcpyAsync(scoremap, b.smap, hw * 4, hipMemcpyDeviceToDevice, c->stream));
    if (nms) RFE_HIP(c, hipMemcpyAsync(nms, b.nmap, hw * 4, hipMemcpyDeviceToDevice, c->stream));
    if (descmap) RFE_HIP(c, hipMemcpyAsync(descmap, b.dmap, hw / 64 * 256 * 4, hipMemcpyDeviceToDevice, c->stream));
    RFE_HIP(c, hipStreamSynchronize(c->stream));
    return RFE_OK;
}

extern "C" int rfe_k_select(rfe_ctx* c, const float* nms, int B, int H, int W, int Kmax, float thr, int topk_always, int32_t* n, int32_t* kxy,
                            float* score) {
    int rc = sp_check(c, H, W, B, Kmax);
    if (rc) return rc;
    if (!nms || !n || !kxy || !score) return fail(c, RFE_ERR_INVALID, "k_select: null pointer");
    RFE_HIP(c, hipSetDevice(c->device));
    SpBuffers b;
    if ((rc = sp_carve(c, B, H, W, b))) return rc;
    launch_select(c->stream, nms, B, H, W, Kmax, thr, b.cand_score, b.cand_idx, n, kxy, score, (int32_t*)b.ss, topk_always != 0, b.sel_keys, b.sel_n);
    RFE_HIP(c, hipGetLastError());
    RFE_HIP(c, hipStreamSynchronize(c->stream));
    return RFE_OK;
}

extern "C" int rfe_k_select_keys(rfe_ctx* c, const float* nms, int B, int H, int W, int Kmax, float thr, int topk_always, int32_t* n, int32_t* kxy,
                                 float* score) {
    int rc = sp_check(c, H, W, B, Kmax);
    if (rc) return rc;
    if (!nms || !n || !kxy || !score || B > 4) return fail(c, RFE_ERR_INVALID, "k_select_keys: null pointer or more than four frames");
    RFE_HIP(c, hipSetDevice(c->device));
    SpBuffers b;
    if ((rc = sp_carve(c, B, H, W, b))) return rc;
    if (!c->sp_cnt) RFE_HIP(c, hipMalloc((void**)&c->sp_cnt, 8 * sizeof(int32_t)));
    RFE_HIP(c, hipMemsetAsync(c->sp_cnt, 0, 8 * sizeof(int32_t), c->stream));
    launch_keys_from_map(c->stream, nms, B, H * W, thr, (unsigned long long*)b.cand_score, c->sp_cnt);
    launch_select_keys(c->stream, (const unsigned long long*)b.cand_score, c->sp_cnt, B, H, W, Kmax, topk_always != 0, n, kxy, score);
    c->sp_cnt_dirty = false;
    RFE_HIP(c, hipGetLastError());
    RFE_HIP(c, hipStreamSynchronize(c->stream));
    int32_t left[8];
    RFE_HIP(c, hipMemcpy(left, c->sp_cnt, sizeof(left), hipMemcpyDeviceToHost));
    for (int q = 0; q < 8; ++q) if (left[q] != 0) return fail(c, RFE_ERR_HIP, "k_select_keys: the ranking kernel did not leave the candidate counters at zero");
    return RFE_OK;
}

extern "C" int rfe_k_lightglue_ffn(rfe_ctx* c, int layer, int cross, const float* x, const float* second, int rows, float* out) {
    int rc = lg_check(c, 1, 4, 4);
    if (rc) return rc;
    if (layer < 0 || layer >= LG_LAYERS || rows <= 0 || !x || !second || !out) return fail(c, RFE_ERR_INVALID, "k_lightglue_ffn: bad argument");
    RFE_HIP(c, hipSetDevice(c->device));
    const int L = 1024, P = (rows + 2 * L - 1) / (2 * L);
    LgBuffers b;
    if ((rc = lg_carve(c, P, L, b))) return rc;
    const LgLayerDev& Lw = c->lg.L[layer];
    RFE_HIP(c, hipMemcpyAsync(out, x, (size_t)rows * 1024, hipMemcpyDeviceToDevice, c->stream));
    if (cross) lg_ffn(c, b, out, second, rows, Lw.cw1, Lw.cb1, Lw.clng, Lw.clnb, Lw.cw2, Lw.cb2);
    else lg_ffn(c, b, out, second, rows, Lw.w1, Lw.b1, Lw.lng, Lw.lnb, Lw.w2, Lw.b2);
    RFE_HIP(c, hipGetLastError());
    RFE_HIP(c, hipStreamSynchronize(c->stream));
    return RFE_OK;
}

extern "C" int rfe_k_attention(rfe_ctx* c, const float* q, const float* k, const float* v, int ld, float* out, int nseq, int Lq, int Lk,
                               const int32_t* qlen, const int32_t* klen, const int32_t* kv_map, const float* rope) {
    if (!c) return RFE_ERR_INVALID;
    if (!q || !k || !v || !out || nseq <= 0 || Lq <= 0 || Lk <= 0 || ld < 256) return fail(c, RFE_ERR_INVALID, "k_attention: bad argument");
    RFE_HIP(c, hipSetDevice(c->device));
    float* part = nullptr;
    const size_t pb = lg_attention_part_bytes(nseq, Lq);
    if (pb) RFE_HIP(c, hipMalloc((void**)&part, pb));
    launch_lg_attention(c->stream, q, k, v, ld, out, nseq, Lq, Lk, qlen, klen, kv_map, part, rope, c->opt_lg_fp16x2);
    hipError_t e = hipGetLastError();
    if (e == hipSuccess) e = hipStreamSynchronize(c->stream);
    if (part) (void)hipFree(part);
    RFE_HIP(c, e);
    return RFE_OK;
}

extern "C" int rfe_k_set_lightglue_tap(rfe_ctx* c, int pair, float* x0, float* x1, float* scores) {
    if (!c) return RFE_ERR_INVALID;
    if (pair < 0) { c->tap.armed = false; return RFE_OK; }
    c->tap.armed = true; c->tap.pair = pair; c->tap.x0 = x0; c->tap.x1 = x1; c->tap.scores = scores;
    return RFE_OK;
}

extern "C" int rfe_k_lightglue_self_attention(rfe_ctx* c, int layer, const float* x, const float* csn, const int32_t* lens, int nseq, int L,
                                              float* qkv_out, float* ctx_out, int32_t* qk_rotated) {
    int rc = lg_check(c, 1, 4, 4);
    if (rc) return rc;
    if (layer < 0 || layer >= LG_LAYERS || nseq <= 0 || L <= 0 || (L % 4) || !x || !csn || !lens) return fail(c, RFE_ERR_INVALID, "k_lightglue_self_attention: bad argument");
    RFE_HIP(c, hipSetDevice(c->device));
    const int P = (nseq + 1) / 2;
    LgBuffers b;
    if ((rc = lg_carve(c, P, L, b))) return rc;
    const bool rot = lg_self_qkv_attention(c, b, c->lg.L[layer], x, csn, lens, nseq, L);
    RFE_HIP(c, hipGetLastError());
    if (qkv_out) RFE_HIP(c, hipMemcpyAsync(qkv_out, b.qkv, (size_t)nseq * L * 768 * 4, hipMemcpyDeviceToDevice, c->stream));
    if (ctx_out) RFE_HIP(c, hipMemcpyAsync(ctx_out, b.ctx, (size_t)nseq * L * 256 * 4, hipMemcpyDeviceToDevice, c->stream));
    RFE_HIP(c, hipStreamSynchronize(c->stream));
    if (qk_rotated) *qk_rotated = rot ? 1 : 0;
    return RFE_OK;
}

extern "C" int rfe_k_lightglue_taps(rfe_ctx* c, const float* k0n, const float* k1n, const float* d0, const float* d1,
                                    int M, int N, float* x0, float* x1, float* scores) {
    int rc = lg_check(c, 1, M, N);
    if (rc) return rc;
    RFE_HIP(c, hipSetDevice(c->device));
    const int L = ((std::max(M, N) + 3) / 4) * 4, cap = std::min(M, N);
    LgBuffers b;
    float *sc, *dms; int32_t *dm, *dn, *dS, *dp;
    if ((rc = lg_carve(c, 1, L, b, [&](Bump& a) {
             sc = a.take<float>((size_t)L * L);
             dm = a.take<int32_t>(1); dn = a.take<int32_t>(1); dS = a.take<int32_t>(1);
             dp = a.take<int32_t>((size_t)cap * 2); dms = a.take<float>(cap);
         }))) return rc;
    RFE_HIP(c, hipMemcpyAsync(dm, &M, 4, hipMemcpyHostToDevice, c->stream));
    RFE_HIP(c, hipMemcpyAsync(dn, &N, 4, hipMemcpyHostToDevice, c->stream));
    RFE_HIP(c, hipStreamSynchronize(c->stream));
    if ((rc = lg_stage(c, b, k0n, k1n, d0, d1, dm, dn, 1, M, N, L))) return rc;
    if ((rc = lg_forward(c, b, 1, L, 0.1f, cap, dS, dp, dms, scores ? sc : nullptr, false, true))) return rc;
    if (x0) RFE_HIP(c, hipMemcpyAsync(x0, b.x, (size_t)M * 1024, hipMemcpyDeviceToDevice, c->stream));
    if (x1) RFE_HIP(c, hipMemcpyAsync(x1, b.x + (size_t)L * 256, (size_t)N * 1024, hipMemcpyDeviceToDevice, c->stream));
    if (scores) RFE_HIP(c, hipMemcpy2DAsync(scores, (size_t)N * 4, sc, (size_t)L * 4, (size_t)N * 4, M, hipMemcpyDeviceToDevice, c->stream));
    RFE_HIP(c, hipStreamSynchronize(c->stream));
    return RFE_OK;
}
```

### rover-slam_amd/csrc/api_weights.hip

```cpp
#include <stdio.h>
#include <stdlib.h>
#include <string.h>
#include <map>
#include <mutex>
#include <tuple>
#include "api_internal.h"

using namespace rfe;

extern "C" int64_t rfe_weight_count(int kind) {
    return kind == RFE_KIND_SUPERPOINT ? SP_COUNT : kind == RFE_KIND_LIGHTGLUE ? LG_COUNT : -1;
}

namespace {
struct SpShared {
    rfe::SpWeightsDev w; int device = 0; std::vector<float> host;
    ~SpShared() {
        (void)hipSetDevice(device);
        if (w.conv1a_w) (void)hipFree(w.conv1a_w);
        for (int l = 0; l < 12; ++l) { if (w.packed[l]) (void)hipFree(w.packed[l]); if (w.bias[l]) (void)hipFree(w.bias[l]); }
    }
};
struct LgShared {
    rfe::LgWeightsDev w; int device = 0; std::vector<float> host;
    ~LgShared() { (void)hipSetDevice(device); if (w.blob) (void)hipFree(w.blob); if (w.extra) (void)hipFree(w.extra); if (w.h2) (void)hipFree(w.h2); }
};
std::mutex g_weights_mu;
std::map<std::tuple<int, int, uint64_t, int>, std::weak_ptr<void>> g_weights;

uint64_t fnv1a64(const float* p, size_t n) {
    const unsigned char* b = reinterpret_cast<const unsigned char*>(p);
    uint64_t h = 1469598103934665603ull;
    for (size_t i = 0; i < n * sizeof(float); ++i) { h ^= b[i]; h *= 1099511628211ull; }
    return h;
}
}

static int upload(rfe_ctx* c, float** dst, const float* src, size_t n) {
    if (*dst) { RFE_HIP(c, hipFree(*dst)); *dst = nullptr; }
    RFE_HIP(c, hipMalloc((void**)dst, n * sizeof(float)));
    RFE_HIP(c, hipMemcpy(*dst, src, n * sizeof(float), hipMemcpyHostToDevice));
    return RFE_OK;
}

static int set_sp_upload(rfe_ctx* c, const float* blob);
static int set_lg_upload(rfe_ctx* c, const float* blob);

template <typename Shared, typename Dev>
static int set_shared(rfe_ctx* c, int kind, const float* blob, size_t count, std::shared_ptr<void>& hold, Dev& dev, bool& has, int (*upload_fn)(rfe_ctx*, const float*)) {
    const uint64_t hash = fnv1a64(blob, count);
    std::lock_guard<std::mutex> lk(g_weights_mu);
    auto key = std::make_tuple(c->device, kind, hash, 0);
    for (;; ++std::get<3>(key)) {
        auto it = g_weights.find(key);
        if (it == g_weights.end()) break;
        auto sp = it->second.lock();
        if (!sp) break;
        if (memcmp(static_cast<Shared*>(sp.get())->host.data(), blob, count * sizeof(float)) != 0) continue;
        hold = sp; dev = static_cast<Shared*>(sp.get())->w; has = true;
        return RFE_OK;
    }
    has = false; hold.reset(); dev = Dev();
    int rc = upload_fn(c, blob);
    auto sp = std::make_shared<Shared>();
    sp->w = dev; sp->device = c->device;
    if (rc) { dev = Dev(); return rc; }
    sp->host.assign(blob, blob + count);
    hold = sp; g_weights[key] = sp;
    return RFE_OK;
}
static int set_sp(rfe_ctx* c, const float* blob) {
    return set_shared<SpShared>(c, RFE_KIND_SUPERPOINT, blob, (size_t)SP_COUNT, c->sp_hold, c->sp, c->has_sp, set_sp_upload);
}
static int set_lg(rfe_ctx* c, const float* blob) {
    return set_shared<LgShared>(c, RFE_KIND_LIGHTGLUE, blob, (size_t)LG_COUNT, c->lg_hold, c->lg, c->has_lg, set_lg_upload);
}

static int set_sp_upload(rfe_ctx* c, const float* blob) {
    size_t off = 0;
    for (int l = 0; l < 12; ++l) {
        const SpLayer& L = kSpLayers[l];
        const float* w = blob + off;
        const size_t wn = (size_t)L.cout * L.cin * L.k * L.k;
        const float* b = w + wn;
        off += wn + L.cout;
        int rc;
        if (l == L_1A) {
            std::vector<float> t(9 * 64);
            for (int co = 0; co < 64; ++co) for (int k = 0; k < 9; ++k) t[k * 64 + co] = w[co * 9 + k];
            if ((rc = upload(c, &c->sp.conv1a_w, t.data(), t.size()))) return rc;
        } else if (L.k == 3) {
            std::vector<float> t;
            pack_conv3x3_weights(w, L.cin, L.cout, L.pool, t);
            if ((rc = upload(c, &c->sp.packed[l], t.data(), t.size()))) return rc;
        } else {
            if ((rc = upload(c, &c->sp.packed[l], w, wn))) return rc;
        }
        if ((rc = upload(c, &c->sp.bias[l], b, L.cout))) return rc;
    }
    c->has_sp = true;
    return RFE_OK;
}

static int set_lg_upload(rfe_ctx* c, const float* blob) {
    int rc = upload(c, &c->lg.blob, blob, (size_t)LG_COUNT);
    if (rc) return rc;
    size_t taken = 0;
    auto take = [&](size_t n) { float* r = c->lg.blob + taken; taken += n; return r; };
    LgWeightsDev& W = c->lg;
    W.wr = take(64);
    for (int l = 0; l < LG_LAYERS; ++l) {
        LgLayerDev& L = W.L[l];
        L.wqkv = take(768 * 256); L.bqkv = take(768); L.wo = take(256 * 256); L.bo = take(256);
        L.w1 = take(512 * 512); L.b1 = take(512); L.lng = take(512); L.lnb = take(512);
        L.w2 = take(256 * 512); L.b2 = take(256);
        L.cwqk = take(256 * 256); L.cbqk = take(256); L.cwv = take(256 * 256); L.cbv = take(256);
        L.cwo = take(256 * 256); L.cbo = take(256);
        L.cw1 = take(512 * 512); L.cb1 = take(512); L.clng = take(512); L.clnb = take(512);
        L.cw2 = take(256 * 512); L.cb2 = take(256);
    }
    W.wp = take(256 * 256); W.bp = take(256); W.wm = take(256); W.bm = take(1);
    if (taken != (size_t)LG_COUNT) return fail(c, RFE_ERR_INVALID, "internal: LightGlue blob layout mismatch");
    if (W.extra) { RFE_HIP(c, hipFree(W.extra)); W.extra = nullptr; }
    const size_t per = 512 * 256 + 512 + 2 * (512 * 512 + 512);
    RFE_HIP(c, hipMalloc((void**)&W.extra, per * LG_LAYERS * sizeof(float)));
    {
        std::vector<float> w1f(512 * 512), b1f(512);
        std::vector<double> acc(256);
        size_t off = 64;
        for (int l = 0; l < LG_LAYERS; ++l) {
            LgLayerDev& L = W.L[l];
            float* base = W.extra + per * l + 512 * 256 + 512;
            L.w1f = base; L.b1f = base + 512 * 512; L.cw1f = L.b1f + 512; L.cb1f = L.cw1f + 512 * 512;
            const float* h = blob + off;
            const float* s_wo = h + 768 * 256 + 768; const float* s_bo = s_wo + 256 * 256;
            const float* s_w1 = s_bo + 256; const float* s_b1 = s_w1 + 512 * 512;
            const float* cr = s_b1 + 512 + 512 + 512 + 256 * 512 + 256;
            const float* c_wo = cr + 2 * (256 * 256 + 256); const float* c_bo = c_wo + 256 * 256;
            const float* c_w1 = c_bo + 256; const float* c_b1 = c_w1 + 512 * 512;
            off += 1250560;
            for (int blk = 0; blk < 2; ++blk) {
                const float* wo = blk ? c_wo : s_wo; const float* bo = blk ? c_bo : s_bo;
                const float* w1 = blk ? c_w1 : s_w1; const float* b1 = blk ? c_b1 : s_b1;
                for (int i = 0; i < 512; ++i) {
                    const float* w1row = w1 + (size_t)i * 512;
                    for (int j = 0; j < 256; ++j) { w1f[(size_t)i * 512 + j] = w1row[j]; acc[j] = 0.0; }
                    double bacc = b1[i];
                    for (int k = 0; k < 256; ++k) {
                        const double wv = w1row[256 + k];
                        const float* worow = wo + (size_t)k * 256;
                        for (int j = 0; j < 256; ++j) acc[j] += wv * (double)worow[j];
                        bacc += wv * (double)bo[k];
                    }
                    for (int j = 0; j < 256; ++j) w1f[(size_t)i * 512 + 256 + j] = (float)acc[j];
                    b1f[i] = (float)bacc;
                }
                RFE_HIP(c, hipMemcpy(blk ? L.cw1f : L.w1f, w1f.data(), w1f.size() * 4, hipMemcpyHostToDevice));
                RFE_HIP(c, hipMemcpy(blk ? L.cb1f : L.b1f, b1f.data(), b1f.size() * 4, hipMemcpyHostToDevice));
            }
        }
    }
    for (int l = 0; l < LG_LAYERS; ++l) {
        LgLayerDev& L = W.L[l];
        L.cwqkv = W.extra + per * l; L.cbqkv = L.cwqkv + 512 * 256;
        RFE_HIP(c, hipMemcpy(L.cwqkv, L.cwqk, 256 * 256 * 4, hipMemcpyDeviceToDevice));
        RFE_HIP(c, hipMemcpy(L.cwqkv + 256 * 256, L.cwv, 256 * 256 * 4, hipMemcpyDeviceToDevice));
        RFE_HIP(c, hipMemcpy(L.cbqkv, L.cbqk, 256 * 4, hipMemcpyDeviceToDevice));
        RFE_HIP(c, hipMemcpy(L.cbqkv + 256, L.cbv, 256 * 4, hipMemcpyDeviceToDevice));
    }
    if (W.h2) { RFE_HIP(c, hipFree(W.h2)); W.h2 = nullptr; }
    W.n_blob = ((size_t)LG_COUNT + 63) & ~(size_t)63; W.n_extra = per * LG_LAYERS;
    RFE_HIP(c, hipMalloc((void**)&W.h2, 2 * (W.n_blob + W.n_extra) * sizeof(uint16_t)));
    launch_split_f16(c->stream, W.blob, W.h2, W.h2 + W.n_blob, (size_t)LG_COUNT);
    launch_split_f16(c->stream, W.extra, W.h2 + 2 * W.n_blob, W.h2 + 2 * W.n_blob + W.n_extra, W.n_extra);
    RFE_HIP(c, hipGetLastError());
    RFE_HIP(c, hipStreamSynchronize(c->stream));
    c->has_lg = true;
    return RFE_OK;
}

static void take_hparams(rfe_hparams& to, const rfe_hparams& from, int kind) {
    if (kind == RFE_KIND_SUPERPOINT) {
        to.sp_max_keypoints = from.sp_max_keypoints; to.sp_detection_threshold = from.sp_detection_threshold; to.sp_nms_radius = from.sp_nms_radius;
        to.sp_remove_borders = from.sp_remove_borders; to.sp_topk_always = from.sp_topk_always;
    } else {
        to.lg_layers = from.lg_layers; to.lg_heads = from.lg_heads; to.lg_filter_threshold = from.lg_filter_threshold;
    }
}

extern "C" int rfe_set_weights(rfe_ctx* c, int kind, const float* blob, int64_t count) {
    if (!c || !blob) return fail(c, RFE_ERR_INVALID, "rfe_set_weights: null argument");
    RFE_HIP(c, hipSetDevice(c->device));
    if (count != rfe_weight_count(kind)) return fail(c, RFE_ERR_INVALID, "rfe_set_weights: wrong float count for this model kind");
    RFE_HIP(c, hipStreamSynchronize(c->stream));
    const int rc = kind == RFE_KIND_SUPERPOINT ? set_sp(c, blob) : set_lg(c, blob);
    ++c->settings_gen;
    if (rc == RFE_OK) {
        take_hparams(c->hp, rfe_default_hparams(), kind);
    }
    return rc;
}

extern "C" uint64_t rfe_weights_id(rfe_ctx* c, int kind) {
    if (!c) return 0;
    const void* p = kind == RFE_KIND_SUPERPOINT ? c->sp_hold.get() : kind == RFE_KIND_LIGHTGLUE ? c->lg_hold.get() : nullptr;
    return (uint64_t)(uintptr_t)p;
}

static int check_hparams(rfe_ctx* c, const rfe_hparams& h, const char* who) {
    if (h.sp_max_keypoints < 1 || h.sp_max_keypoints > 4096) return fail(c, RFE_ERR_INVALID, std::string(who) + ": sp_max_keypoints must be in 1..4096");
    if (!(h.sp_detection_threshold >= 0.f) || !(h.sp_detection_threshold < 1.f)) return fail(c, RFE_ERR_INVALID, std::string(who) + ": sp_detection_threshold must be in [0, 1)");
    if (h.sp_nms_radius < 1 || h.sp_nms_radius > NMS_MAX_RADIUS) return fail(c, RFE_ERR_INVALID, std::string(who) + ": sp_nms_radius must be in 1.." + std::to_string(NMS_MAX_RADIUS));
    if (h.sp_remove_borders < 0 || h.sp_remove_borders > 64) return fail(c, RFE_ERR_INVALID, std::string(who) + ": sp_remove_borders must be in 0..64");
    if (h.sp_topk_always != 0 && h.sp_topk_always != 1) return fail(c, RFE_ERR_INVALID, std::string(who) + ": sp_topk_always must be 0 or 1");
    if (h.lg_layers != LG_LAYERS || h.lg_heads != 4)
        return fail(c, RFE_ERR_INVALID, std::string(who) + ": the LightGlue kernels are built for 9 layers of 4 heads x 64, the file / caller says " +
                                        std::to_string(h.lg_layers) + " layers of " + std::to_string(h.lg_heads) + " heads");
    if (!(h.lg_filter_threshold >= 0.f) || !(h.lg_filter_threshold < 1.f)) return fail(c, RFE_ERR_INVALID, std::string(who) + ": lg_filter_threshold must be in [0, 1)");
    return RFE_OK;
}

static int load_rfew(rfe_ctx* c, const char* path, int want_kind) {
    FILE* f = fopen(path, "rb");
    if (!f) return fail(c, RFE_ERR_IO, std::string("cannot open weight file ") + path);
    unsigned char head[20];
    if (fread(head, 1, 20, f) != 20 || memcmp(head, "RFEW", 4) != 0) { fclose(f); return fail(c, RFE_ERR_IO, std::string("not an RFEW file: ") + path); }
    uint32_t ver, kind; uint64_t cnt;
    memcpy(&ver, head + 4, 4); memcpy(&kind, head + 8, 4); memcpy(&cnt, head + 12, 8);
    if ((ver != 1 && ver != 2) || (int)kind != want_kind || (int64_t)cnt != rfe_weight_count(want_kind)) { fclose(f); return fail(c, RFE_ERR_IO, std::string("RFEW header mismatch in ") + path); }
    rfe_hparams hp = c->hp;
    if (ver == 2) {
        uint32_t hb = 0;
        unsigned char blk[256];
        const uint32_t need = want_kind == RFE_KIND_SUPERPOINT ? 20u : 12u;
        if (fread(&hb, 4, 1, f) != 1 || hb < need || hb > sizeof(blk) || fread(blk, 1, hb, f) != hb) { fclose(f); return fail(c, RFE_ERR_IO, std::string("RFEW v2 hyper-parameter block damaged in ") + path); }
        if (want_kind == RFE_KIND_SUPERPOINT) {
            memcpy(&hp.sp_max_keypoints, blk, 4); memcpy(&hp.sp_detection_threshold, blk + 4, 4);
            memcpy(&hp.sp_nms_radius, blk + 8, 4); memcpy(&hp.sp_remove_borders, blk + 12, 4); memcpy(&hp.sp_topk_always, blk + 16, 4);
        } else {
            memcpy(&hp.lg_layers, blk, 4); memcpy(&hp.lg_heads, blk + 4, 4); memcpy(&hp.lg_filter_threshold, blk + 8, 4);
        }
        const int rc = check_hparams(c, hp, path);
        if (rc) { fclose(f); c->err = "RFEW v2 hyper-parameters refused: " + c->err; return RFE_ERR_IO; }
    }
    std::vector<float> blob(cnt);
    size_t got = fread(blob.data(), sizeof(float), cnt, f);
    fclose(f);
    if (got != cnt) return fail(c, RFE_ERR_IO, std::string("short read on ") + path);
    const int rc = rfe_set_weights(c, want_kind, blob.data(), (int64_t)cnt);
    if (rc == RFE_OK && ver == 2) take_hparams(c->hp, hp, want_kind);
    return rc;
}

extern "C" int rfe_get_hparams(rfe_ctx* c, rfe_hparams* out) {
    if (!c || !out) return RFE_ERR_INVALID;
    *out = c->hp;
    return RFE_OK;
}
extern "C" int rfe_set_hparams(rfe_ctx* c, const rfe_hparams* in) {
    if (!c || !in) return RFE_ERR_INVALID;
    const int rc = check_hparams(c, *in, "rfe_set_hparams");
    if (rc) return rc;
    c->hp = *in;
    ++c->settings_gen;
    return RFE_OK;
}

static int load_onnx(rfe_ctx* c, const char* path, int want_kind) {
    std::vector<float> blob;
    rfe_hparams hp = rfe_default_hparams();
    std::string err;
    if (!rfe::onnx_convert(path, want_kind, blob, &hp, err)) return fail(c, RFE_ERR_IO, err);
    int rc = check_hparams(c, hp, path);
    if (rc) { c->err = "graph hyper-parameters refused: " + c->err; return RFE_ERR_IO; }
    if ((int64_t)blob.size() != rfe_weight_count(want_kind)) return fail(c, RFE_ERR_IO, std::string("converted weight count mismatch for ") + path);
    rc = rfe_set_weights(c, want_kind, blob.data(), (int64_t)blob.size());
    if (rc == RFE_OK) take_hparams(c->hp, hp, want_kind);
    return rc;
}

static int load_any(rfe_ctx* c, const char* path, int want_kind) {
    FILE* f = fopen(path, "rb");
    if (!f) return fail(c, RFE_ERR_IO, std::string("cannot open weight file ") + path);
    unsigned char magic[4] = {0, 0, 0, 0};
    const size_t got = fread(magic, 1, 4, f);
    fclose(f);
    if (got == 4 && memcmp(magic, "RFEW", 4) == 0) return load_rfew(c, path, want_kind);
    return load_onnx(c, path, want_kind);
}

static int load_pair(rfe_ctx* c, const char* sp_path, const char* lg_path, int (*load)(rfe_ctx*, const char*, int)) {
    if (!c) return RFE_ERR_INVALID;
    int rc;
    if (sp_path && (rc = load(c, sp_path, RFE_KIND_SUPERPOINT))) return rc;
    if (lg_path && (rc = load(c, lg_path, RFE_KIND_LIGHTGLUE))) return rc;
    return RFE_OK;
}
extern "C" int rfe_load_weights(rfe_ctx* c, const char* sp_path, const char* lg_path) { return load_pair(c, sp_path, lg_path, load_any); }
extern "C" int rfe_load_onnx(rfe_ctx* c, const char* sp_path, const char* lg_path) { return load_pair(c, sp_path, lg_path, load_onnx); }
```

### rover-slam_amd/csrc/rfe_internal.h

```cpp
#pragma once
#include <hip/hip_runtime.h>
#include <stdint.h>
#include <stdlib.h>
#include <memory>
#include <string>
#include <vector>
#include "../../include/rover_fe.h"

typedef float f32x16 __attribute__((ext_vector_type(16)));
typedef float f32x4 __attribute__((ext_vector_type(4)));

namespace rfe {


struct SpLayer { int cin, cout, k; bool pool; };
static const SpLayer kSpLayers[12] = {
    {1, 64, 3, false}, {64, 64, 3, true}, {64, 64, 3, false}, {64, 64, 3, true}, {64, 128, 3, false}, {128, 128, 3, true},
    {128, 128, 3, false}, {128, 128, 3, false}, {128, 256, 3, false}, {256, 65, 1, false}, {128, 256, 3, false}, {256, 256, 1, false}};
enum { L_1A, L_1B, L_2A, L_2B, L_3A, L_3B, L_4A, L_4B, L_PA, L_PB, L_DA, L_DB };

constexpr int LG_LAYERS = 9;
constexpr int64_t SP_COUNT = 1300865;
constexpr int64_t LG_COUNT = 11321153;

constexpr int CONV_CK = 8;
constexpr int CONV_NT = 64;

struct SpWeightsDev {
    float* conv1a_w = nullptr;
    float* packed[12] = {nullptr};
    float* bias[12] = {nullptr};
};

struct LgLayerDev {
    float *wqkv, *bqkv, *wo, *bo, *w1, *b1, *lng, *lnb, *w2, *b2;
    float *cwqk, *cbqk, *cwv, *cbv, *cwo, *cbo, *cw1, *cb1, *clng, *clnb, *cw2, *cb2;
    float *cwqkv, *cbqkv;
    float *w1f, *b1f, *cw1f, *cb1f;
};
struct LgWeightsDev {
    float* blob = nullptr;
    float* extra = nullptr;
    float* wr;
    LgLayerDev L[LG_LAYERS];
    float *wp, *bp, *wm, *bm;
    uint16_t* h2 = nullptr;
    size_t n_blob = 0, n_extra = 0;
};

struct Stage { std::string name; double ms = 0; int64_t calls = 0; };

struct GemmArgs {
    const float* A; int lda;
    const float* A2; int lda2; int K1;
    const float* B; int ldb;
    const float* bias;
    const float* R; int ldr;
    float* C; int ldc;
    int M, N, K;
    float alpha; int relu;
    long long sA, sA2, sB, sC, sR;
    const int* m_valid;
    int batch;
    float* stats_out;
    const float* stats_in; int stats_p; const float* ln_g; const float* ln_b;
    const uint16_t* Bh; const uint16_t* Bl;
    int kperm;
    const float* rope_csn; int rope_c0, rope_c1;
};

}

inline rfe_hparams rfe_default_hparams() { return rfe_hparams{1024, 0.0005f, 4, 4, 0, rfe::LG_LAYERS, 4, 0.1f}; }

struct rfe_ctx {
    int device = 0;
    hipStream_t own_stream = nullptr;
    hipStream_t stream = nullptr;
    hipStream_t side_stream = nullptr;
    hipEvent_t ev_fork = nullptr, ev_join = nullptr;
    hipEvent_t ev_pyr = nullptr;
    std::string err;
    bool has_sp = false, has_lg = false;
    bool opt_lg_fold = true;
    bool opt_lg_fp16x2 = false;
    bool opt_host_graph = false;
    struct HostGraph {
        struct Slot { std::string key; hipGraphExec_t exec = nullptr; unsigned long long used = 0; };
        struct Seen { std::string key; int count = 0; unsigned long long used = 0; };
        Slot slot[4]; Seen seen[8]; unsigned long long tick = 0;
    };
    HostGraph g_extract, g_match;
    unsigned long long settings_gen = 0;
    rfe_hparams hp = rfe_default_hparams();
    rfe::SpWeightsDev sp;
    rfe::LgWeightsDev lg;
    std::shared_ptr<void> sp_hold, lg_hold;
    void* ws_sp = nullptr; size_t ws_sp_bytes = 0;
    void* ws_lg = nullptr; size_t ws_lg_bytes = 0;
    void* ws_io = nullptr; size_t ws_io_bytes = 0;
    void* h_pin = nullptr; size_t h_pin_bytes = 0;
    void* ws_tmp = nullptr; size_t ws_tmp_bytes = 0;
    void* ws_pyr = nullptr; size_t ws_pyr_bytes = 0;
    void* ws_ptab = nullptr; size_t ws_ptab_bytes = 0; std::string ptab_key; std::vector<size_t> ptab_off;
    int32_t* sp_cnt = nullptr;
    bool sp_cnt_dirty = false;
    void* ws_ps = nullptr; size_t ws_ps_bytes = 0;
    int ps_cap = 0;
    void* ws_st = nullptr; size_t ws_st_bytes = 0;
    int st_H = 0, st_W = 0, st_K = 0; bool st_have_prev = false; int st_flip = 0; std::string st_pyr_key;
    struct { bool armed = false; int pair = 0; float *x0 = nullptr, *x1 = nullptr, *scores = nullptr; } tap;
    bool prof = false;
    std::string prof_filter;
    std::vector<rfe::Stage> stages;
    std::vector<std::pair<int, std::pair<hipEvent_t, hipEvent_t>>> pending;
    std::vector<hipEvent_t> ev_pool;
};

namespace rfe {

int fail(rfe_ctx* c, int code, const std::string& msg);
#define RFE_HIP(ctx, call)                                                                      \
    do {                                                                                        \
        hipError_t e_ = (call);                                                                 \
        if (e_ != hipSuccess)                                                                   \
            return rfe::fail((ctx), RFE_ERR_HIP, std::string(#call) + ": " + hipGetErrorString(e_)); \
    } while (0)

struct ProfScope {
    rfe_ctx* c; int idx; hipEvent_t e0 = nullptr, e1 = nullptr;
    hipStream_t st;
    ProfScope(rfe_ctx* ctx, const char* name, hipStream_t on = nullptr);
    ~ProfScope();
};
void prof_collect(rfe_ctx* c);

int ensure_ws(rfe_ctx* c, void** p, size_t* cur, size_t need);

bool conv3x3_reads_t16(int cin, int cout, bool pool);
void pack_conv3x3_weights(const float* w_oihw, int cin, int cout, bool pool, std::vector<float>& out);
size_t packed_conv3x3_count(int cin, int cout, bool pool);
void launch_conv3x3(hipStream_t s, const float* in, int B, int H, int W, int cin,
                    const float* wpacked, const float* bias, int cout, bool relu, bool pool, float* out,
                    int tag = 0);
void launch_conv1ab_fused(hipStream_t s, const void* img, bool img_f32, int stride, int B, int H, int W, const float* w1a,
                          const float* b1a, const float* wp, const float* bias, float* out, long long frame_step = 0 );
inline void ensure_dynamic_lds(const void* kernel, int bytes, bool* done) {
    int dev = 0;
    (void)hipGetDevice(&dev);
    if (dev < 0 || dev >= 64 || !done[dev]) {
        (void)hipFuncSetAttribute(kernel, hipFuncAttributeMaxDynamicSharedMemorySize, bytes);
        if (dev >= 0 && dev < 64) done[dev] = true;
    }
}
int launch_gemm_h2(hipStream_t s, const GemmArgs& g);
void launch_split_f16(hipStream_t s, const float* x, uint16_t* hi, uint16_t* lo, size_t n);
bool gemm_nt_rope_ok(const GemmArgs& g);
int launch_gemm_nt(hipStream_t s, const GemmArgs& g);
inline bool gemm_latency_regime(const GemmArgs& g) {
    const long long b = g.batch > 0 ? g.batch : 1;
    auto tiles = [&](int bm, int bn) { return (long long)((g.M + bm - 1) / bm) * ((g.N + bn - 1) / bn) * b; };
    const bool big = (g.N % 256 == 0 && tiles(128, 256) >= 256) || tiles(128, 128) >= 256 || g.M > 8192;
    return !big;
}
bool launch_gemm_lat(hipStream_t s, const GemmArgs& g, const float* rope_csn, int rope_cols);
bool onnx_convert(const std::string& path, int kind, std::vector<float>& blob, rfe_hparams* hp, std::string& err);
bool launch_ffn2_ln_lat(hipStream_t s, const float* h, const float* w2, const float* b2, const float* ln_g, const float* ln_b, const float* R, int ldr,
                        float* C, int ldc, int M);
bool launch_lg_attention_lat(hipStream_t s, const float* q, const float* k, const float* v, int ld, float* out, int nseq, int Lq, int Lk,
                             const int* qlen, const int* klen, const int* kv_map, bool h2 = false );
void launch_softmax65_d2s(hipStream_t s, const float* logits, int ld, int B, int Hc, int Wc, float* score);
constexpr int NMS_MAX_RADIUS = 8;
void launch_nms(hipStream_t s, const float* score, int B, int H, int W, int radius , int border, float* tmp_ss,
                uint8_t* tmp_mask, uint8_t* tmp_supp, float* out);
void launch_select(hipStream_t s, const float* nms, int B, int H, int W, int Kmax, float thr,
                   float* cand_score, int32_t* cand_idx, int32_t* n_out, int32_t* kxy, float* score,
                   int32_t* chunk_cnt , bool topk_always ,
                   unsigned long long* sel_keys , int32_t* sel_n );
bool launch_sp_tail_lat(hipStream_t s, const float* logits, int B, int Hc, int Wc, int radius, int border, float thr, unsigned long long* cand_keys ,
                        int32_t* cand_cnt , float* smap_out , float* nmap_out );
void launch_select_keys(hipStream_t s, const unsigned long long* cand_keys, int32_t* cand_cnt, int B, int H, int W, int Kmax, bool topk_always,
                        int32_t* n_out, int32_t* kxy, float* score);
void launch_keys_from_map(hipStream_t s, const float* nms, int B, int HW, float thr, unsigned long long* cand_keys, int32_t* cand_cnt);
void launch_descmap_norm(hipStream_t s, float* dmap, int64_t cells);
void launch_desc_sample(hipStream_t s, const float* dmap, int B, int Hc, int Wc, int H, int W,
                        const int32_t* n, const int32_t* kxy, int Kmax, float* desc, uint8_t* desc_bin );
void launch_lg_posenc(hipStream_t s, const float* kn, const float* wr, int rows, float* csn );
void launch_lg_attention(hipStream_t s, const float* q, const float* k, const float* v, int ld ,
                         float* out, int nseq, int Lq, int Lk, const int* qlen, const int* klen,
                         const int* kv_map ,
                         float* part ,
                         const float* rope_csn = nullptr ,
                         bool fp16x2 = false );
void launch_lg_attention_h2(hipStream_t s, const float* q, const float* k, const float* v, int ld, float* out, int nseq, int Lq, int Lk,
                            const int* qlen, const int* klen, const int* kv_map, const float* rope_csn);
size_t lg_attention_part_bytes(int nseq, int Lq);
void launch_lg_ln_gelu(hipStream_t s, float* h, const float* g, const float* b, int64_t rows);
void launch_lg_assign(hipStream_t s, const float* sim, const float* z0, const float* z1, int P, int L,
                      int cap, const int* m, const int* n, float thr, float* scores_opt, float* rowlse,
                      float* collse, int32_t* a0, float* mx0, int32_t* a1, int32_t* S, int32_t* pairs,
                      float* ms, int scores_pair ,
                      const float* x, const float* wm, const float* bm, float* z );
bool lg_assign_few_pairs(int P, int L);
void launch_lg_frame_prologue(hipStream_t s, const int32_t* kxy, const float* desc, const float* wr, const int32_t* nkp, int B, int L, int rows, int cols,
                              float* kn, float* csn, float* x, int32_t* lens, int32_t* kvmap);
void launch_lg_matchability(hipStream_t s, const float* x, const float* w, const float* b, int64_t rows, float* z);
void launch_copy_f32(hipStream_t s, const float* src, float* dst, int64_t n);
void launch_normalize_kpts(hipStream_t s, const int32_t* kxy, int64_t n, int rows, int cols, float* out);

void launch_stereo_match(hipStream_t s, const uint8_t* imgL, const uint8_t* imgR, int H, int W, int stride,
                         const float* kL, int N, const float* kR, int Nr, const float* dL, const float* dR, float mb,
                         float mbf, float* uRight, float* depth, int32_t* sadv);

void launch_stereo_match_counts(hipStream_t s, const uint8_t* imgL, const uint8_t* imgR, int H, int W, int stride,
                                const int32_t* kL, const int32_t* kR, int Kmax, const int32_t* counts, const float* dL,
                                const float* dR, float mb, float mbf, float* uRight, float* depth, int32_t* sadv);

int pyramid_geometry(int H, int W, int nlevels, float scale_factor, int32_t* level_h, int32_t* level_w, float* level_scale);
void pyramid_tables(int nlevels, const int32_t* level_h, const int32_t* level_w, std::vector<int2>& tab, std::vector<size_t>& off);
void launch_pyr_resample(hipStream_t s, const uint8_t* src, long long src_frame, int src_stride, int Hs, int Ws, uint8_t* dst, long long dst_frame,
                         int Hd, int Wd, int B, const int2* cx, const int2* cy);
struct PyrMergeArgs {
    int L, Ktot;
    const int32_t* n[RFE_MAX_LEVELS];
    const int32_t* kxy[RFE_MAX_LEVELS];
    const float* sc[RFE_MAX_LEVELS];
    const float* desc_l[RFE_MAX_LEVELS];
    int kmax[RFE_MAX_LEVELS];
    float scale[RFE_MAX_LEVELS];
    int32_t* n_out; int32_t* level_n ; float* kpts; int32_t* octave; float* score; float* desc;
};
void launch_pyr_merge(hipStream_t s, const PyrMergeArgs& a, int B);

struct StereoPyrTable {
    int L;
    int32_t h[RFE_MAX_LEVELS], w[RFE_MAX_LEVELS];
    uint32_t off[RFE_MAX_LEVELS];
    float s[RFE_MAX_LEVELS], inv[RFE_MAX_LEVELS];
};
void launch_stereo_match_pyr(hipStream_t s, const uint8_t* levL, const uint8_t* levR, const StereoPyrTable& T, const float* kL,
                             const int32_t* octL, int N, const float* kR, const int32_t* octR, int Nr, const int32_t* counts,
                             const float* dL, const float* dR, float mb, float mbf, int sad_level0, float* uRight, float* depth,
                             int32_t* sadv);

void launch_l2_matrix(hipStream_t s, const float* a, int M, const float* b, int N, float* out);
void launch_binarize(hipStream_t s, const float* d, int64_t rows, uint8_t* out);
void launch_search_candidates(hipStream_t s, const float* q, int Nq, const float* f, int Nf, const int32_t* offsets, const int32_t* cand,
                              const uint8_t* skip, int32_t* best_idx, float* best_dist, float* second_dist);
void launch_distinctive(hipStream_t s, const float* desc, const int32_t* offsets, int total , int Np, int maxn,
                        float* med , int32_t* best, float* median);

__device__ __forceinline__ float desc_dist_wave(const float4 a, const float4 b) {
    const float d0 = a.x - b.x, d1 = a.y - b.y, d2 = a.z - b.z, d3 = a.w - b.w;
    double p = 0.0;
    p += (double)d0 * (double)d0; p += (double)d1 * (double)d1; p += (double)d2 * (double)d2; p += (double)d3 * (double)d3;
#pragma unroll
    for (int off = 32; off >= 1; off >>= 1) p = p + __shfl_xor(p, off);
    return (float)sqrt(p);
}

void launch_proj_grid(hipStream_t s, const float* kpts, const int32_t* kxy, int Nf, const int32_t* nf_dev, float min_x, float min_y,
                      float inv_w, float inv_h, int32_t* cell_start, int32_t* cell_items, float* fxy);
void launch_proj_count(hipStream_t s, const float* proj, const float* radius, const int32_t* pred_level, int Nq, const int32_t* cell_start,
                       const int32_t* cell_items, const float* fxy, const int32_t* octave, float min_x, float min_y, float inv_w,
                       float inv_h, int cand_cap, int32_t* seg_off, int32_t* cand_idx, int32_t* stats);
void launch_proj_fill(hipStream_t s, const float* q, int Nq, const float* f, int Nf, const int32_t* seg_off, const int32_t* cand_idx,
                      const uint8_t* skip, float* cand_dist);
void launch_proj_resolve(hipStream_t s, const int32_t* seg_off, const int32_t* cand_idx, const float* cand_dist, const uint8_t* observed,
                         int Nq, int Nf, float th_high, int32_t* assign, int32_t* best_idx, float* best_dist, float* second_dist,
                         int32_t* stats);

}
```

### rover-slam_amd/csrc/sp_conv.hip

```cpp
#include <stdlib.h>
#include "rfe_internal.h"

namespace rfe {

constexpr int TH = 8, TW = 32, IH = TH + 2, IW = TW + 2;
constexpr int TWS = IW;
constexpr int PLANE = IH * TWS;
constexpr int NT = CONV_NT;

constexpr int CK = CONV_CK;

size_t packed_conv3x3_count(int cin, int cout, bool pool) { return (size_t)cout * cin * 9 * (conv3x3_reads_t16(cin, cout, pool) ? 2 : 1); }

void pack_conv3x3_weights(const float* w, int cin, int cout, bool pool, std::vector<float>& out) {
    out.assign(packed_conv3x3_count(cin, cout, pool), 0.f);
    const int KCH = CK * 9;
    const int nch = cin / CK, nct = cout / NT;
    for (int ct = 0; ct < nct; ++ct)
        for (int ch = 0; ch < nch; ++ch)
            for (int kl = 0; kl < KCH; ++kl)
                for (int j = 0; j < NT; ++j) {
                    int co = ct * NT + j, ci = ch * CK + kl / 9, tap = kl % 9;
                    out[(((size_t)ct * nch + ch) * KCH + kl) * NT + j] = w[((size_t)co * cin + ci) * 9 + tap];
                }
    if (!conv3x3_reads_t16(cin, cout, pool)) return;
    float* t16 = out.data() + (size_t)cout * cin * 9;
    const int nst = cin / 16;
    for (int b = 0; b < cout / 16; ++b)
        for (int st = 0; st < nst; ++st)
            for (int g = 0; g < 9; ++g)
                for (int q = 0; q < 4; ++q)
                    for (int co = 0; co < 16; ++co)
                        for (int sq = 0; sq < 4; ++sq) {
                            const int kap = 16 * g + 4 * sq + q, ci = st * 16 + kap / 9, tap = kap % 9;
                            t16[((((((size_t)b * nst + st) * 9 + g) * 4 + q) * 16 + co) * 4) + sq] = w[((size_t)(b * 16 + co) * cin + ci) * 9 + tap];
                        }
}

__device__ __forceinline__ void conv_a_offsets(int (&aoff)[9], int h, int wave, int col) {
#pragma unroll
    for (int s = 0; s < 9; ++s) {
        const int k0 = 2 * s, k1 = 2 * s + 1;
        const int o0 = (k0 / 9) * PLANE + ((k0 % 9) / 3) * TWS + (k0 % 9) % 3;
        const int o1 = (k1 / 9) * PLANE + ((k1 % 9) / 3) * TWS + (k1 % 9) % 3;
        aoff[s] = (h ? o1 : o0) + (2 * wave) * TWS + col;
    }
}

template <int PLANE_ = PLANE, int BLK1_ = TWS>
__device__ __forceinline__ void conv_chunk_mma(const float* lds_in, const float* lds_w, const int (&aoff)[9], int boff,
                                               f32x16 (&acc)[2][2]) {
#pragma unroll 1
    for (int cp = 0; cp < CK / 2; ++cp) {
        const float* ap = lds_in + cp * 2 * PLANE_;
        const float* bp = lds_w + cp * 18 * NT + boff;
#pragma unroll
        for (int s = 0; s < 9; ++s) {
            const float a0 = ap[aoff[s]], a1 = ap[aoff[s] + BLK1_];
            const float b0 = bp[2 * s * NT], b1 = bp[2 * s * NT + 32];
            acc[0][0] = __builtin_amdgcn_mfma_f32_32x32x2f32(a0, b0, acc[0][0], 0, 0, 0);
            acc[0][1] = __builtin_amdgcn_mfma_f32_32x32x2f32(a0, b1, acc[0][1], 0, 0, 0);
            acc[1][0] = __builtin_amdgcn_mfma_f32_32x32x2f32(a1, b0, acc[1][0], 0, 0, 0);
            acc[1][1] = __builtin_amdgcn_mfma_f32_32x32x2f32(a1, b1, acc[1][1], 0, 0, 0);
        }
    }
}

__device__ __forceinline__ void conv_stage_weights(float* lds_w, const float* src_chunk, int tid) {
    constexpr int KCH = CK * 9, NTHR = 256;
    const float4* src = reinterpret_cast<const float4*>(src_chunk);
    float4* dst = reinterpret_cast<float4*>(lds_w);
#pragma unroll
    for (int it = 0; it < (KCH * NT / 4 + NTHR - 1) / NTHR; ++it)
        if (it * NTHR + tid < KCH * NT / 4) dst[it * NTHR + tid] = src[it * NTHR + tid];
}

template <bool POOL, bool RELU>
__device__ __forceinline__ void conv_store(const f32x16 (&acc)[2][2], float* __restrict__ out, int b, int H, int W, int COUT,
                                           int x0, int y0, int co0, int wave, int col, int h) {
    if (!POOL) {
        float* out_b = out + (size_t)b * H * W * COUT;
#pragma unroll
        for (int mb = 0; mb < 2; ++mb) {
            const int y = y0 + 2 * wave + mb;
            if (y >= H) continue;
#pragma unroll
            for (int r = 0; r < 16; ++r) {
                const int x = x0 + (r & 3) + 8 * (r >> 2) + 4 * h;
                if (x >= W) continue;
                float v0 = acc[mb][0][r], v1 = acc[mb][1][r];
                if (RELU) { v0 = fmaxf(v0, 0.f); v1 = fmaxf(v1, 0.f); }
                float* o = out_b + ((size_t)y * W + x) * COUT + co0 + col;
                o[0] = v0; o[32] = v1;
            }
        }
    } else {
        const int Ho = H >> 1, Wo = W >> 1;
        float* out_b = out + (size_t)b * Ho * Wo * COUT;
        const int yo = (y0 >> 1) + wave;
        if (yo < Ho) {
#pragma unroll
            for (int r = 0; r < 16; r += 2) {
                const int xo = (x0 >> 1) + ((r & 3) >> 1) + 4 * (r >> 2) + 2 * h;
                if (xo >= Wo) continue;
#pragma unroll
                for (int nb = 0; nb < 2; ++nb) {
                    float v = fmaxf(fmaxf(acc[0][nb][r], acc[0][nb][r + 1]), fmaxf(acc[1][nb][r], acc[1][nb][r + 1]));
                    if (RELU) v = fmaxf(v, 0.f);
                    out_b[((size_t)yo * Wo + xo) * COUT + co0 + nb * 32 + col] = v;
                }
            }
        }
    }
}

struct ConvBlock { int b, bx, by, ct; bool valid; };
__device__ __forceinline__ ConvBlock conv_decode(int nct, int gx, int gy, int ntiles) {
    const int L = blockIdx.x, xcd = L & 7, t = L >> 3;
    ConvBlock k;
    k.ct = t % nct;
    const int u = (t / nct) * 8 + xcd;
    k.valid = u < ntiles;
    k.bx = u % gx; k.by = (u / gx) % gy; k.b = u / (gx * gy);
    return k;
}
static inline unsigned conv_grid(int gx, int gy, int B, int nct) { return (unsigned)(((gx * gy * B + 7) / 8) * 8 * nct); }

template <int CIN, bool POOL, bool RELU, int TAG>
__global__ __launch_bounds__(256, 2) void conv3x3_mfma_kernel(
    const float* __restrict__ in, const float* __restrict__ wp, const float* __restrict__ bias,
    float* __restrict__ out, int H, int W, int COUT, int gx, int gy, int ntiles) {
    constexpr int KCH = CK * 9;
    __shared__ __attribute__((aligned(16))) float lds[CK * PLANE + KCH * NT];
    float* lds_in = lds;
    float* lds_w = lds + CK * PLANE;

    const int tid = threadIdx.x;
    const int lane = tid & 63;
    const int wave = __builtin_amdgcn_readfirstlane(tid >> 6);
    const int col = lane & 31, h = lane >> 5;
    const ConvBlock blk = conv_decode(COUT / NT, gx, gy, ntiles);
    if (!blk.valid) return;
    const int b = blk.b, ct = blk.ct;
    const int x0 = blk.bx * TW, y0 = blk.by * TH;
    const int co0 = ct * NT;

    f32x16 acc[2][2];
    {
        const float b0 = bias[co0 + col], b1 = bias[co0 + 32 + col];
#pragma unroll
        for (int r = 0; r < 16; ++r) { acc[0][0][r] = b0; acc[1][0][r] = b0; acc[0][1][r] = b1; acc[1][1][r] = b1; }
    }
    int aoff[9];
    conv_a_offsets(aoff, h, wave, col);
    const int boff = h * NT + col;

    const float* in_b = in + (size_t)b * H * W * CIN;
    const float* wp_ct = wp + (size_t)ct * (CIN / CK) * KCH * NT;

    constexpr int S_IT = (IH * IW * (CK / 4) + 255) / 256;
    int s_goff[S_IT], s_loff[S_IT];
#pragma unroll
    for (int it = 0; it < S_IT; ++it) {
        const int idx = tid + it * 256;
        const int cq = idx % (CK / 4), pix = idx / (CK / 4);
        const int py = pix / IW, px = pix % IW;
        const int gy = y0 - 1 + py, gx = x0 - 1 + px;
        const bool slot = idx < IH * IW * (CK / 4);
        s_loff[it] = slot ? (cq * 4) * PLANE + py * TWS + px : -1;
        s_goff[it] = (slot && gy >= 0 && gy < H && gx >= 0 && gx < W) ? (gy * W + gx) * CIN + cq * 4 : -1;
    }

    constexpr bool PAIR = (CIN / CK) % 2 == 0;
    float4 v_odd[S_IT];
    for (int ch = 0; ch < CIN / CK; ++ch) {
        __syncthreads();
#pragma unroll
        for (int it = 0; it < S_IT; ++it) {
            if (s_loff[it] < 0) continue;
            float4 v = make_float4(0.f, 0.f, 0.f, 0.f);
            if (!PAIR) {
                if (s_goff[it] >= 0) v = *reinterpret_cast<const float4*>(in_b + s_goff[it] + ch * CK);
            } else if ((ch & 1) == 0) {
                v_odd[it] = v;
                if (s_goff[it] >= 0) {
                    v = *reinterpret_cast<const float4*>(in_b + s_goff[it] + ch * CK);
                    v_odd[it] = *reinterpret_cast<const float4*>(in_b + s_goff[it] + (ch + 1) * CK);
                }
            } else {
                v = v_odd[it];
            }
            float* d = lds_in + s_loff[it];
            d[0] = v.x; d[PLANE] = v.y; d[2 * PLANE] = v.z; d[3 * PLANE] = v.w;
        }
        conv_stage_weights(lds_w, wp_ct + (size_t)ch * KCH * NT, tid);
        __syncthreads();
        conv_chunk_mma(lds_in, lds_w, aoff, boff, acc);
    }
    conv_store<POOL, RELU>(acc, out, b, H, W, COUT, x0, y0, co0, wave, col, h);
}

constexpr int STH = 4, SNT = 32;

template <int CIN, bool RELU, bool POOL = false>
__global__ __launch_bounds__(64 * STH, 4) void conv3x3_small_kernel(
    const float* __restrict__ in, const float* __restrict__ wp, const float* __restrict__ bias,
    float* __restrict__ out, int H, int W, int COUT, int gx, int gy, int ntiles) {
    constexpr int KCH = CK * 9;
    constexpr int NTH = 64 * STH, RIH = STH + 2, RPLANE = RIH * TWS;
    constexpr int LDS_WORDS = (CK * RPLANE + KCH * SNT) > (POOL ? STH * TW * SNT : 0) ? (CK * RPLANE + KCH * SNT) : STH * TW * SNT;
    __shared__ __attribute__((aligned(16))) float lds[LDS_WORDS];
    float* lds_in = lds;
    float* lds_w = lds + CK * RPLANE;
    const int tid = threadIdx.x, lane = tid & 63;
    const int wave = __builtin_amdgcn_readfirstlane(tid >> 6);
    const int col = lane & 31, h = lane >> 5;
    const ConvBlock blk = conv_decode(COUT / SNT, gx, gy, ntiles);
    if (!blk.valid) return;
    const int b = blk.b, ct = blk.ct;
    const int x0 = blk.bx * TW, y0 = blk.by * STH;
    const int co0 = ct * SNT;

    f32x16 acc;
    {
        const float b0 = bias[co0 + col];
#pragma unroll
        for (int r = 0; r < 16; ++r) acc[r] = b0;
    }
    int aoff[9];
#pragma unroll
    for (int s = 0; s < 9; ++s) {
        const int k0 = 2 * s, k1 = 2 * s + 1;
        const int o0 = (k0 / 9) * RPLANE + ((k0 % 9) / 3) * TWS + (k0 % 9) % 3;
        const int o1 = (k1 / 9) * RPLANE + ((k1 % 9) / 3) * TWS + (k1 % 9) % 3;
        aoff[s] = (h ? o1 : o0) + wave * TWS + col;
    }
    const int boff = h * SNT + col;
    const float* in_b = in + (size_t)b * H * W * CIN;
    const float* wp_ct = wp + (size_t)(ct >> 1) * (CIN / CK) * KCH * NT + (ct & 1) * SNT;

    for (int ch = 0; ch < CIN / CK; ++ch) {
        __syncthreads();
        for (int idx = tid; idx < RIH * IW * (CK / 4); idx += NTH) {
            const int cq = idx % (CK / 4), pix = idx / (CK / 4);
            const int py = pix / IW, px = pix % IW;
            const int gy = y0 - 1 + py, gx = x0 - 1 + px;
            float4 v = make_float4(0.f, 0.f, 0.f, 0.f);
            if (gy >= 0 && gy < H && gx >= 0 && gx < W)
                v = *reinterpret_cast<const float4*>(in_b + ((size_t)gy * W + gx) * CIN + ch * CK + cq * 4);
            float* d = lds_in + (cq * 4) * RPLANE + py * TWS + px;
            d[0] = v.x; d[RPLANE] = v.y; d[2 * RPLANE] = v.z; d[3 * RPLANE] = v.w;
        }
        {
            const float* src = wp_ct + (size_t)ch * KCH * NT;
            for (int idx = tid; idx < KCH * (SNT / 4); idx += NTH) {
                const int kl = idx / (SNT / 4), q = idx % (SNT / 4);
                reinterpret_cast<float4*>(lds_w)[idx] = *reinterpret_cast<const float4*>(src + kl * NT + q * 4);
            }
        }
        __syncthreads();
#pragma unroll 1
        for (int cp = 0; cp < CK / 2; ++cp) {
            const float* ap = lds_in + cp * 2 * RPLANE;
            const float* bp = lds_w + cp * 18 * SNT + boff;
#pragma unroll
            for (int s = 0; s < 9; ++s) acc = __builtin_amdgcn_mfma_f32_32x32x2f32(ap[aoff[s]], bp[2 * s * SNT], acc, 0, 0, 0);
        }
    }
    if (POOL) {
        __syncthreads();
#pragma unroll
        for (int r = 0; r < 16; ++r) {
            const int xl = (r & 3) + 8 * (r >> 2) + 4 * h;
            float v = acc[r];
            if (RELU) v = fmaxf(v, 0.f);
            lds[(wave * TW + xl) * SNT + col] = v;
        }
        __syncthreads();
        const int Ho = H >> 1, Wo = W >> 1;
        float* out_b = out + (size_t)b * Ho * Wo * COUT;
        const int chn = tid & 31;
#pragma unroll
        for (int it = 0; it < (STH / 2) * (TW / 2) / 8; ++it) {
            const int pp = (tid >> 5) + 8 * it, pr = pp / (TW / 2), pc = pp % (TW / 2);
            const int yo = (y0 >> 1) + pr, xo = (x0 >> 1) + pc;
            if (yo >= Ho || xo >= Wo) continue;
            const float* e = lds + ((2 * pr) * TW + 2 * pc) * SNT + chn;
            out_b[((size_t)yo * Wo + xo) * COUT + co0 + chn] = fmaxf(fmaxf(e[0], e[SNT]), fmaxf(e[TW * SNT], e[TW * SNT + SNT]));
        }
        return;
    }
    const int y = y0 + wave;
    if (y < H) {
        float* out_b = out + (size_t)b * H * W * COUT;
#pragma unroll
        for (int r = 0; r < 16; ++r) {
            const int x = x0 + (r & 3) + 8 * (r >> 2) + 4 * h;
            if (x >= W) continue;
            float v = acc[r];
            if (RELU) v = fmaxf(v, 0.f);
            out_b[((size_t)y * W + x) * COUT + co0 + col] = v;
        }
    }
}

constexpr int T16_H = 4, T16_W = 16, T16_IH = T16_H + 2, T16_IW = T16_W + 2, T16_PLANE = T16_IH * T16_IW, T16_NC = 32, T16_CK = 16;

typedef __attribute__((address_space(3))) void* conv_lds_ptr_t;
typedef const __attribute__((address_space(1))) void* conv_gptr_t;
constexpr int T16D_WROWS = 144, T16D_PIX = 128;
__device__ __attribute__((aligned(64))) float t16d_zero_line[16];

template <int CIN, bool RELU, int NC = T16_NC, bool POOL = false>
__global__ __launch_bounds__(256, 2) void conv3x3_t16d_kernel(
    const float* __restrict__ in, const float* __restrict__ wp, const float* __restrict__ bias,
    float* __restrict__ out, int H, int W, int COUT, int gx, int gy, int ntiles) {
    static_assert(NC == 32 || NC == 16, "32 or 16 output channels per workgroup");
    constexpr int NB = NC / 16;
    constexpr int NST = CIN / T16_CK;
    constexpr int IST_W = T16D_PIX * T16_CK, WST_W = T16D_WROWS * NC;
    extern __shared__ __attribute__((aligned(16))) float lds[];
    float* const lin = lds;
    float* const lwr = lds + 3 * IST_W;
    const int tid = threadIdx.x, lane = tid & 63;
    const int wave = __builtin_amdgcn_readfirstlane(tid >> 6);
    const int px = lane & 15, q = lane >> 4;
    const ConvBlock blk = conv_decode(COUT / NC, gx, gy, ntiles);
    if (!blk.valid) return;
    const int b = blk.b, ct = blk.ct;
    const int x0 = blk.bx * T16_W, y0 = blk.by * T16_H;
    const int co0 = ct * NC;

    f32x4 acc[NB];
#pragma unroll
    for (int nb = 0; nb < NB; ++nb) acc[nb] = *reinterpret_cast<const f32x4*>(bias + co0 + nb * 16 + 4 * q);
    int poff[4][9];
#pragma unroll
    for (int s9 = 0; s9 < 9; ++s9) {
        const int kap = 4 * s9 + q, e = kap / 9, tap = kap % 9;
        const int p = (wave + tap / 3) * T16_IW + px + tap % 3;
#pragma unroll
        for (int c4 = 0; c4 < 4; ++c4) poff[c4][s9] = p * T16_CK + e + ((c4 ^ ((p >> 2) & 3)) << 2);
    }
    const float* in_b = in + (size_t)b * H * W * CIN;
    const float* wp_t16 = wp + (size_t)COUT * CIN * 9;
    constexpr int NSLOT = 9 * NB, WCP = (NSLOT + 3) / 4, BLK_W = 9 * 256;
    int w_slot[WCP];
    const float* w_src[WCP];
#pragma unroll
    for (int u = 0; u < WCP; ++u) {
        w_slot[u] = wave + 4 * u < NSLOT ? wave + 4 * u : wave + 4 * (u - 1);
        const int nbk = w_slot[u] / 9, gs = w_slot[u] % 9;
        w_src[u] = wp_t16 + ((size_t)(ct * NB + nbk) * NST) * BLK_W + gs * 256 + lane * 4;
    }
    const float* i_src[2];
    bool i_img[2];
#pragma unroll
    for (int u = 0; u < 2; ++u) {
        const int p = (wave + 4 * u) * 16 + (lane >> 2);
        const int py = p / T16_IW, pxx = p % T16_IW;
        const int gyy = y0 - 1 + py, gxx = x0 - 1 + pxx;
        const int g = (lane & 3) ^ ((p >> 2) & 3);
        i_img[u] = p < T16_PLANE && gyy >= 0 && gyy < H && gxx >= 0 && gxx < W;
        i_src[u] = i_img[u] ? in_b + ((size_t)gyy * W + gxx) * CIN + g * 4 : t16d_zero_line + g * 4;
    }
    auto issue = [&](int st) {
        float* wdst = lwr + (st % 3) * WST_W;
        float* idst = lin + (st % 3) * IST_W;
#pragma unroll
        for (int u = 0; u < WCP; ++u)
            __builtin_amdgcn_global_load_lds((conv_gptr_t)(w_src[u] + (size_t)st * BLK_W), (conv_lds_ptr_t)(wdst + w_slot[u] * 256), 16, 0, 0);
#pragma unroll
        for (int u = 0; u < 2; ++u)
            __builtin_amdgcn_global_load_lds((conv_gptr_t)(i_src[u] + (i_img[u] ? st * T16_CK : 0)), (conv_lds_ptr_t)(idst + (wave + 4 * u) * 256), 16, 0, 0);
    };
    issue(0);
    if (NST > 1) issue(1);
    for (int st = 0; st < NST; ++st) {
        __builtin_amdgcn_sched_barrier(0);
        if (st + 1 < NST) asm volatile("s_waitcnt vmcnt(%0)\n\ts_barrier" ::"n"(WCP + 2) : "memory");
        else asm volatile("s_waitcnt vmcnt(0)\n\ts_barrier" ::: "memory");
        __builtin_amdgcn_sched_barrier(0);
        if (st + 2 < NST) issue(st + 2);
        const float* li = lin + (st % 3) * IST_W;
        const float* lw = lwr + (st % 3) * WST_W + (q * 16 + px) * 4;
#pragma unroll
        for (int g = 0; g < 9; ++g) {
            f32x4 wf[NB];
#pragma unroll
            for (int nb = 0; nb < NB; ++nb) wf[nb] = *reinterpret_cast<const f32x4*>(lw + nb * BLK_W + g * 256);
#pragma unroll
            for (int sq = 0; sq < 4; ++sq) {
                constexpr int dummy = 0; (void)dummy;
                const int s36 = 4 * g + sq;
                const float pv = li[poff[s36 / 9][s36 % 9]];
#pragma unroll
                for (int nb = 0; nb < NB; ++nb) acc[nb] = __builtin_amdgcn_mfma_f32_16x16x4f32(wf[nb][sq], pv, acc[nb], 0, 0, 0);
            }
        }
    }
    if (RELU) {
#pragma unroll
        for (int nb = 0; nb < NB; ++nb) { acc[nb][0] = fmaxf(acc[nb][0], 0.f); acc[nb][1] = fmaxf(acc[nb][1], 0.f); acc[nb][2] = fmaxf(acc[nb][2], 0.f); acc[nb][3] = fmaxf(acc[nb][3], 0.f); }
    }
    if (POOL) {
        __builtin_amdgcn_sched_barrier(0);
        asm volatile("s_waitcnt lgkmcnt(0)\n\ts_barrier" ::: "memory");
        __builtin_amdgcn_sched_barrier(0);
        float* ex = lds;
#pragma unroll
        for (int nb = 0; nb < NB; ++nb) {
            f32x4 hm;
#pragma unroll
            for (int e = 0; e < 4; ++e) hm[e] = fmaxf(acc[nb][e], __shfl_xor(acc[nb][e], 1));
            if (!(px & 1)) *reinterpret_cast<f32x4*>(ex + (wave * 8 + (px >> 1)) * NC + nb * 16 + 4 * q) = hm;
        }
        __syncthreads();
        constexpr int CG = NC / 4;
        if (tid < 2 * 8 * CG) {
            const int cg = tid % CG, ppx = (tid / CG) & 7, prow = tid / (8 * CG);
            const f32x4 a = *reinterpret_cast<const f32x4*>(ex + ((2 * prow) * 8 + ppx) * NC + cg * 4);
            const f32x4 c = *reinterpret_cast<const f32x4*>(ex + ((2 * prow + 1) * 8 + ppx) * NC + cg * 4);
            const int Ho = H >> 1, Wo = W >> 1, yo = (y0 >> 1) + prow, xo = (x0 >> 1) + ppx;
            if (yo < Ho && xo < Wo)
                *reinterpret_cast<f32x4*>(out + (((size_t)b * Ho + yo) * Wo + xo) * COUT + co0 + cg * 4) =
                    f32x4{fmaxf(a[0], c[0]), fmaxf(a[1], c[1]), fmaxf(a[2], c[2]), fmaxf(a[3], c[3])};
        }
        return;
    }
    const int y = y0 + wave, x = x0 + px;
    if (y < H && x < W) {
        float* o = out + (((size_t)b * H + y) * W + x) * COUT + co0 + 4 * q;
#pragma unroll
        for (int nb = 0; nb < NB; ++nb) *reinterpret_cast<f32x4*>(o + nb * 16) = acc[nb];
    }
}

constexpr int CIH = TH + 4, CIW = TW + 4, CPLANE = CIH * CIW;
template <int CIN, bool RELU, int TAG>
__global__ __launch_bounds__(256, 2) void conv3x3_comp_kernel(
    const float* __restrict__ in, const float* __restrict__ wp, const float* __restrict__ bias,
    float* __restrict__ out, int B, int H, int W, int COUT, int gx, int gy, int ntiles) {
    constexpr int KCH = CK * 9;
    __shared__ __attribute__((aligned(16))) float lds[CK * CPLANE + KCH * NT];
    float* lds_in = lds;
    float* lds_w = lds + CK * CPLANE;
    const int tid = threadIdx.x;
    const int lane = tid & 63;
    const int wave = __builtin_amdgcn_readfirstlane(tid >> 6);
    const int col = lane & 31, h = lane >> 5;
    const ConvBlock blk = conv_decode(COUT / NT, gx, gy, ntiles);
    if (!blk.valid) return;
    const int ct = blk.ct, co0 = ct * NT;
    const int x0 = blk.bx * TW, y0 = blk.by * TH;
    const int pair0 = y0 / H, yin = y0 % H, half0 = x0 / W, xin = x0 % W;
    const int rb = (H - yin) < TH ? (H - yin) : TH;
    const int cb = (W - xin) < TW ? (W - xin) : TW;
    auto frame_of = [&](int pr, int pc) { const int hf = half0 + pc; const int f = 2 * (pair0 + pr) + hf; return (hf <= 1 && f < B) ? f : -1; };
    if (frame_of(0, 0) < 0 && frame_of(0, 1) < 0 && frame_of(1, 0) < 0 && frame_of(1, 1) < 0) return;

    f32x16 acc[2][2];
    {
        const float b0 = bias[co0 + col], b1 = bias[co0 + 32 + col];
#pragma unroll
        for (int r = 0; r < 16; ++r) { acc[0][0][r] = b0; acc[1][0][r] = b0; acc[0][1][r] = b1; acc[1][1][r] = b1; }
    }
    int aoff[9];
    {
        const int r0 = 2 * wave;
        const int base = (r0 + (r0 >= rb ? 2 : 0)) * CIW + col + (col >= cb ? 2 : 0);
#pragma unroll
        for (int s = 0; s < 9; ++s) {
            const int k0 = 2 * s, k1 = 2 * s + 1;
            const int o0 = (k0 / 9) * CPLANE + ((k0 % 9) / 3) * CIW + (k0 % 9) % 3;
            const int o1 = (k1 / 9) * CPLANE + ((k1 % 9) / 3) * CIW + (k1 % 9) % 3;
            aoff[s] = (h ? o1 : o0) + base;
        }
    }
    const int boff = h * NT + col;
    const float* wp_ct = wp + (size_t)ct * (CIN / CK) * KCH * NT;

    constexpr int S_IT = (CIH * CIW * (CK / 4) + 255) / 256;
    int s_goff[S_IT], s_loff[S_IT];
#pragma unroll
    for (int it = 0; it < S_IT; ++it) {
        const int idx = tid + it * 256;
        const int cq = idx % (CK / 4), pix = idx / (CK / 4);
        const int lr = pix / CIW, lc = pix % CIW;
        const int pr = lr >= rb + 2, hr = lr - (pr ? rb + 2 : 0), nr = pr ? TH - rb : rb;
        const int pc = lc >= cb + 2, hc = lc - (pc ? cb + 2 : 0), nc = pc ? TW - cb : cb;
        const bool slot = idx < CIH * CIW * (CK / 4) && nr > 0 && nc > 0 && hr < nr + 2 && hc < nc + 2;
        const int y = (pr ? 0 : yin) + hr - 1, x = (pc ? 0 : xin) + hc - 1;
        const int f = frame_of(pr, pc);
        s_loff[it] = slot ? (cq * 4) * CPLANE + lr * CIW + lc : -1;
        s_goff[it] = (slot && f >= 0 && y >= 0 && y < H && x >= 0 && x < W) ? ((f * H + y) * W + x) * CIN + cq * 4 : -1;
    }
    static_assert((CIN / CK) % 2 == 0, "paired chunk fetch");
    float4 v_odd[S_IT];
    for (int ch = 0; ch < CIN / CK; ++ch) {
        __syncthreads();
#pragma unroll
        for (int it = 0; it < S_IT; ++it) {
            if (s_loff[it] < 0) continue;
            float4 v = make_float4(0.f, 0.f, 0.f, 0.f);
            if ((ch & 1) == 0) {
                v_odd[it] = v;
                if (s_goff[it] >= 0) {
                    v = *reinterpret_cast<const float4*>(in + s_goff[it] + ch * CK);
                    v_odd[it] = *reinterpret_cast<const float4*>(in + s_goff[it] + (ch + 1) * CK);
                }
            } else {
                v = v_odd[it];
            }
            float* d = lds_in + s_loff[it];
            d[0] = v.x; d[CPLANE] = v.y; d[2 * CPLANE] = v.z; d[3 * CPLANE] = v.w;
        }
        conv_stage_weights(lds_w, wp_ct + (size_t)ch * KCH * NT, tid);
        __syncthreads();
        conv_chunk_mma<CPLANE, CIW>(lds_in, lds_w, aoff, boff, acc);
    }
#pragma unroll
    for (int mb = 0; mb < 2; ++mb) {
        const int r = 2 * wave + mb, pr = r >= rb;
        const int y = pr ? r - rb : yin + r;
#pragma unroll
        for (int q = 0; q < 16; ++q) {
            const int c = (q & 3) + 8 * (q >> 2) + 4 * h, pc = c >= cb;
            const int x = pc ? c - cb : xin + c;
            const int f = frame_of(pr, pc);
            if (f < 0) continue;
            float v0 = acc[mb][0][q], v1 = acc[mb][1][q];
            if (RELU) { v0 = fmaxf(v0, 0.f); v1 = fmaxf(v1, 0.f); }
            float* o = out + (((size_t)f * H + y) * W + x) * COUT + co0 + col;
            o[0] = v0; o[32] = v1;
        }
    }
}

template <typename PX>
__device__ __forceinline__ float px_value(PX v) {
    if constexpr (sizeof(PX) == 1) return (float)v * 0.003921568859368563f;
    else return v;
}

template <typename PX>
__global__ __launch_bounds__(256, 2) void conv1ab_fused_kernel(
    const PX* __restrict__ img, int stride, const float* __restrict__ w1a , const float* __restrict__ b1a,
    const float* __restrict__ wp, const float* __restrict__ bias, float* __restrict__ out, int H, int W, long long frame_step ) {
    constexpr int CIN = 64, COUT = 64, KCH = CK * 9;
    constexpr int MH = TH + 4, MW = TW + 4;
    __shared__ __attribute__((aligned(16))) float lds[CK * PLANE + KCH * NT + MH * MW];
    float* lds_in = lds;
    float* lds_w = lds + CK * PLANE;
    float* lds_img = lds_w + KCH * NT;

    const int tid = threadIdx.x;
    const int lane = tid & 63;
    const int wave = __builtin_amdgcn_readfirstlane(tid >> 6);
    const int col = lane & 31, h = lane >> 5;
    const int b = blockIdx.z;
    const int x0 = blockIdx.x * TW, y0 = blockIdx.y * TH;

    f32x16 acc[2][2];
    {
        const float b0 = bias[col], b1 = bias[32 + col];
#pragma unroll
        for (int r = 0; r < 16; ++r) { acc[0][0][r] = b0; acc[1][0][r] = b0; acc[0][1][r] = b1; acc[1][1][r] = b1; }
    }
    int aoff[9];
    conv_a_offsets(aoff, h, wave, col);
    const int boff = h * NT + col;

    const PX* im = img + (long long)b * frame_step;
    for (int idx = tid; idx < MH * MW; idx += 256) {
        const int py = idx / MW, px = idx % MW;
        const int gy = y0 - 2 + py, gx = x0 - 2 + px;
        float v = 0.f;
        if (gy >= 0 && gy < H && gx >= 0 && gx < W) v = px_value(im[(size_t)gy * stride + gx]);
        lds_img[idx] = v;
    }

    constexpr int P_IT = (IH * IW + 255) / 256;
    int p_loff[P_IT]; bool p_inb[P_IT]; float p_iv[P_IT][9];
    __syncthreads();
#pragma unroll
    for (int it = 0; it < P_IT; ++it) {
        const int p = tid + it * 256;
        const int py = p / IW, px = p % IW;
        const int gy = y0 - 1 + py, gx = x0 - 1 + px;
        p_loff[it] = p < IH * IW ? py * TWS + px : -1;
        p_inb[it] = gy >= 0 && gy < H && gx >= 0 && gx < W;
#pragma unroll
        for (int k = 0; k < 9; ++k) p_iv[it][k] = p < IH * IW ? lds_img[(py + k / 3) * MW + px + k % 3] : 0.f;
    }

    for (int ch = 0; ch < CIN / CK; ++ch) {
        __syncthreads();
#pragma unroll
        for (int it = 0; it < P_IT; ++it) {
            if (p_loff[it] < 0) continue;
#pragma unroll
            for (int e = 0; e < CK; ++e) {
                const int c = ch * CK + e;
                float a = b1a[c];
#pragma unroll
                for (int k = 0; k < 9; ++k) a = fmaf(p_iv[it][k], w1a[k * 64 + c], a);
                lds_in[e * PLANE + p_loff[it]] = p_inb[it] ? fmaxf(a, 0.f) : 0.f;
            }
        }
        conv_stage_weights(lds_w, wp + (size_t)ch * KCH * NT, tid);
        __syncthreads();
        conv_chunk_mma(lds_in, lds_w, aoff, boff, acc);
    }
    conv_store<true, true>(acc, out, b, H, W, COUT, x0, y0, 0, wave, col, h);
}

void launch_conv1ab_fused(hipStream_t s, const void* img, bool img_f32, int stride, int B, int H, int W, const float* w1a,
                          const float* b1a, const float* wp, const float* bias, float* out, long long frame_step) {
    dim3 grid((W + TW - 1) / TW, (H + TH - 1) / TH, B);
    if (frame_step == 0) frame_step = (long long)stride * H;
    if (img_f32) hipLaunchKernelGGL((conv1ab_fused_kernel<float>), grid, dim3(256), 0, s, (const float*)img, stride, w1a, b1a, wp, bias, out, H, W, frame_step);
    else hipLaunchKernelGGL((conv1ab_fused_kernel<uint8_t>), grid, dim3(256), 0, s, (const uint8_t*)img, stride, w1a, b1a, wp, bias, out, H, W, frame_step);
}

#define RFE_CONV_LAUNCH(CIN, POOL, RELU, TAG)                                                                            \
    hipLaunchKernelGGL((conv3x3_mfma_kernel<CIN, POOL, RELU, TAG>), dim3(conv_grid(gx, gy, B, cout / NT)), dim3(256), 0, s, in, wp, bias, out, H, W, cout, gx, gy, gx * gy * B)

constexpr int CONV_T16_PX = 12000, CONV_T16_PX64 = 20000, CONV_T16P_PX128 = 20000;

bool conv3x3_reads_t16(int cin, int cout, bool pool) { return (cin == 128 || (cin == 64 && !pool)) && cout % T16_NC == 0; }

void launch_conv3x3(hipStream_t s, const float* in, int B, int H, int W, int cin, const float* wp,
                    const float* bias, int cout, bool relu, bool pool, float* out, int tag) {
    const int gx = (W + TW - 1) / TW, gy = (H + TH - 1) / TH;
    const long long px = (long long)B * H * W;
    constexpr int CONV_SMALL = 700;
    const bool small = (long long)gx * gy * B * (cout / NT) < CONV_SMALL && (cin == 64 || cin == 128);
    if (small && relu && !pool && px <= (cin == 64 ? CONV_T16_PX64 : CONV_T16_PX) && cout % T16_NC == 0) {
        const int sx = (W + T16_W - 1) / T16_W, sy = (H + T16_H - 1) / T16_H;
        constexpr int CONV_T16_NC16 = 1000;
        if (cin == 128 && (long long)sx * sy * B * (cout / T16_NC) < CONV_T16_NC16) {
            const dim3 g16(conv_grid(sx, sy, B, cout / 16));
            constexpr int b16 = 3 * (T16D_PIX * T16_CK + T16D_WROWS * 16) * 4;
            static bool l16_[64];
            ensure_dynamic_lds((const void*)conv3x3_t16d_kernel<128, true, 16>, b16, l16_);
            hipLaunchKernelGGL((conv3x3_t16d_kernel<128, true, 16>), g16, dim3(256), b16, s, in, wp, bias, out, H, W, cout, sx, sy, sx * sy * B);
            return;
        }
        const dim3 gs(conv_grid(sx, sy, B, cout / T16_NC));
        constexpr int bytes = 3 * (T16D_PIX * T16_CK + T16D_WROWS * T16_NC) * 4;
        static bool ls_[2][64];
        if (cin == 128) {
            ensure_dynamic_lds((const void*)conv3x3_t16d_kernel<128, true>, bytes, ls_[0]);
            hipLaunchKernelGGL((conv3x3_t16d_kernel<128, true>), gs, dim3(256), bytes, s, in, wp, bias, out, H, W, cout, sx, sy, sx * sy * B);
        } else {
            ensure_dynamic_lds((const void*)conv3x3_t16d_kernel<64, true>, bytes, ls_[1]);
            hipLaunchKernelGGL((conv3x3_t16d_kernel<64, true>), gs, dim3(256), bytes, s, in, wp, bias, out, H, W, cout, sx, sy, sx * sy * B);
        }
        return;
    }
    if (relu && pool && cin == 128 && px <= CONV_T16P_PX128 && cout % T16_NC == 0 && H % 2 == 0 && W % 2 == 0) {
        const int sx = (W + T16_W - 1) / T16_W, sy = (H + T16_H - 1) / T16_H;
        constexpr int b16 = 3 * (T16D_PIX * T16_CK + T16D_WROWS * 16) * 4;
        static bool lp_[64];
        ensure_dynamic_lds((const void*)conv3x3_t16d_kernel<128, true, 16, true>, b16, lp_);
        hipLaunchKernelGGL((conv3x3_t16d_kernel<128, true, 16, true>), dim3(conv_grid(sx, sy, B, cout / 16)), dim3(256), b16, s, in, wp, bias, out, H, W, cout, sx, sy, sx * sy * B);
        return;
    }
    if (small && (!pool || relu)) {
        const int sx = (W + TW - 1) / TW, sy = (H + STH - 1) / STH;
        const dim3 gs(conv_grid(sx, sy, B, cout / SNT));
        if (pool) {
            if (cin == 128) hipLaunchKernelGGL((conv3x3_small_kernel<128, true, true>), gs, dim3(256), 0, s, in, wp, bias, out, H, W, cout, sx, sy, sx * sy * B);
            else hipLaunchKernelGGL((conv3x3_small_kernel<64, true, true>), gs, dim3(256), 0, s, in, wp, bias, out, H, W, cout, sx, sy, sx * sy * B);
        }
        else if (cin == 128 && relu) hipLaunchKernelGGL((conv3x3_small_kernel<128, true>), gs, dim3(256), 0, s, in, wp, bias, out, H, W, cout, sx, sy, sx * sy * B);
        else if (cin == 128) hipLaunchKernelGGL((conv3x3_small_kernel<128, false>), gs, dim3(256), 0, s, in, wp, bias, out, H, W, cout, sx, sy, sx * sy * B);
        else if (relu) hipLaunchKernelGGL((conv3x3_small_kernel<64, true>), gs, dim3(256), 0, s, in, wp, bias, out, H, W, cout, sx, sy, sx * sy * B);
        else hipLaunchKernelGGL((conv3x3_small_kernel<64, false>), gs, dim3(256), 0, s, in, wp, bias, out, H, W, cout, sx, sy, sx * sy * B);
        return;
    }
    if (!pool && relu && cin == 128 && (tag == L_4A || tag == L_4B || tag == L_PA || tag == L_DA) && B >= 2 &&
        H % 2 == 0 && W >= TW && H >= TH && (H % TH != 0 || W % TW != 0) &&
        (long long)B * H * W * cin < (1ll << 31)) {
        const int cx = (2 * W + TW - 1) / TW, cy = (((B + 1) / 2) * H + TH - 1) / TH;
        const dim3 gc(conv_grid(cx, cy, 1, cout / NT));
        switch (tag) {
            case L_4A: hipLaunchKernelGGL((conv3x3_comp_kernel<128, true, L_4A>), gc, dim3(256), 0, s, in, wp, bias, out, B, H, W, cout, cx, cy, cx * cy); return;
            case L_4B: hipLaunchKernelGGL((conv3x3_comp_kernel<128, true, L_4B>), gc, dim3(256), 0, s, in, wp, bias, out, B, H, W, cout, cx, cy, cx * cy); return;
            case L_PA: hipLaunchKernelGGL((conv3x3_comp_kernel<128, true, L_PA>), gc, dim3(256), 0, s, in, wp, bias, out, B, H, W, cout, cx, cy, cx * cy); return;
            default: hipLaunchKernelGGL((conv3x3_comp_kernel<128, true, L_DA>), gc, dim3(256), 0, s, in, wp, bias, out, B, H, W, cout, cx, cy, cx * cy); return;
        }
    }
    switch (tag) {
        case L_2A: RFE_CONV_LAUNCH(64, false, true, L_2A); return;
        case L_2B: RFE_CONV_LAUNCH(64, true, true, L_2B); return;
        case L_3A: RFE_CONV_LAUNCH(64, false, true, L_3A); return;
        case L_3B: RFE_CONV_LAUNCH(128, true, true, L_3B); return;
        case L_4A: RFE_CONV_LAUNCH(128, false, true, L_4A); return;
        case L_4B: RFE_CONV_LAUNCH(128, false, true, L_4B); return;
        case L_PA: RFE_CONV_LAUNCH(128, false, true, L_PA); return;
        case L_DA: RFE_CONV_LAUNCH(128, false, true, L_DA); return;
        default: break;
    }
#define RFE_CONV_GEN(CIN)                                                    \
    do {                                                                     \
        if (pool && relu) RFE_CONV_LAUNCH(CIN, true, true, 0);               \
        else if (relu) RFE_CONV_LAUNCH(CIN, false, true, 0);                 \
        else if (pool) RFE_CONV_LAUNCH(CIN, true, false, 0);                 \
        else RFE_CONV_LAUNCH(CIN, false, false, 0);                          \
    } while (0)
    if (cin == 64) RFE_CONV_GEN(64);
    else if (cin == 128) RFE_CONV_GEN(128);
    else if (cin == 16) RFE_CONV_GEN(16);
    else if (cin == 32) RFE_CONV_GEN(32);
}

}
```

Measured before the change: 945.1 frames/s.

## Pack conv3x3 weights in per-lane MFMA fragment order with separate row image

Conv3x3 weights are now packed in an MFMA-fragment layout where each lane reads four contiguous floats per group, while the old row-major layout is kept as a separate image for the small kernels. The inner MFMA loop of the conv kernels reads B operands per lane instead of strided LDS rows, which is meant to cut LDS/load instruction count and bank conflicts. A tiles selector and a packing hook are added for testing. The cost is extra weight storage for the duplicate images and more complex dispatch.

```diff
diff --git a/include/rover_fe.h b/include/rover_fe.h
--- a/include/rover_fe.h
+++ b/include/rover_fe.h
@@ -184,6 +184,10 @@
 int rfe_k_conv3x3(rfe_ctx* ctx, const float* in_dev, int B, int H, int W, int Cin,
                   const float* w_oihw_host, const float* bias_host, int Cout, int relu, int pool,
                   float* out_dev);
+int rfe_k_conv3x3_tiles(rfe_ctx* ctx, const float* in_dev, int B, int H, int W, int Cin,
+                        const float* w_oihw_host, const float* bias_host, int Cout, int relu, int pool, int tiles,
+                        float* out_dev);
+int64_t rfe_k_pack_conv3x3(const float* w_oihw_host, int Cin, int Cout, int pool, int image, float* out_host, int64_t capacity);
 int rfe_k_linear(rfe_ctx* ctx, const float* a_dev, int M, int K, const float* w_nk_host,
                  const float* bias_host, int N, int relu, float* out_dev);
 int rfe_k_scoremap(rfe_ctx* ctx, const uint8_t* img_dev, int H, int W, int stride, int B,
diff --git a/rover-slam_amd/capi.py b/rover-slam_amd/capi.py
--- a/rover-slam_amd/capi.py
+++ b/rover-slam_amd/capi.py
@@ -24,7 +24,7 @@
     "rfe_pool_create", "rfe_pool_destroy", "rfe_pool_last_error", "rfe_pool_size", "rfe_pool_ctx", "rfe_pool_has_rccl", "rfe_pool_set_weights",
     "rfe_pool_load_weights", "rfe_pool_set_option", "rfe_pool_set_hparams", "rfe_pool_shard", "rfe_pool_extract_match_stream",
     "rfe_profile_enable", "rfe_profile_filter", "rfe_profile_reset", "rfe_profile_read",
-    "rfe_k_conv3x3", "rfe_k_linear", "rfe_k_scoremap", "rfe_k_select", "rfe_k_select_keys", "rfe_k_lightglue_taps", "rfe_k_set_lightglue_tap", "rfe_k_lightglue_ffn", "rfe_k_attention", "rfe_k_lightglue_self_attention", "rfe_k_pool_inject_gather_failure", "rfe_k_onnx_convert",
+    "rfe_k_conv3x3", "rfe_k_conv3x3_tiles", "rfe_k_pack_conv3x3", "rfe_k_linear", "rfe_k_scoremap", "rfe_k_select", "rfe_k_select_keys", "rfe_k_lightglue_taps", "rfe_k_set_lightglue_tap", "rfe_k_lightglue_ffn", "rfe_k_attention", "rfe_k_lightglue_self_attention", "rfe_k_pool_inject_gather_failure", "rfe_k_onnx_convert",
 ]
 
 if not os.path.exists(LIB_PATH):
@@ -113,6 +113,9 @@
 lib.rfe_profile_reset.argtypes = [C.c_void_p]
 lib.rfe_profile_read.argtypes = [C.c_void_p, C.c_char_p, C.c_size_t, C.POINTER(C.c_double), C.POINTER(C.c_int64), C.c_int]
 lib.rfe_k_conv3x3.argtypes = [C.c_void_p, _fp, C.c_int, C.c_int, C.c_int, C.c_int, _fp, _fp, C.c_int, C.c_int, C.c_int, _fp]
+lib.rfe_k_conv3x3_tiles.argtypes = [C.c_void_p, _fp, C.c_int, C.c_int, C.c_int, C.c_int, _fp, _fp, C.c_int, C.c_int, C.c_int, C.c_int, _fp]
+lib.rfe_k_pack_conv3x3.argtypes = [_fp, C.c_int, C.c_int, C.c_int, C.c_int, _fp, C.c_int64]
+lib.rfe_k_pack_conv3x3.restype = C.c_int64
 lib.rfe_k_linear.argtypes = [C.c_void_p, _fp, C.c_int, C.c_int, _fp, _fp, C.c_int, C.c_int, _fp]
 lib.rfe_k_scoremap.argtypes = [C.c_void_p, _u8p, C.c_int, C.c_int, C.c_int, C.c_int, _fp, _fp, _fp]
 lib.rfe_k_select.argtypes = [C.c_void_p, _fp, C.c_int, C.c_int, C.c_int, C.c_int, C.c_float, C.c_int, _ip, _ip, _fp]
diff --git a/rover-slam_amd/csrc/api_extract.hip b/rover-slam_amd/csrc/api_extract.hip
--- a/rover-slam_amd/csrc/api_extract.hip
+++ b/rover-slam_amd/csrc/api_extract.hip
@@ -47,21 +47,21 @@
     const SpWeightsDev& w = c->sp;
     const int H1 = H / 2, W1 = W / 2, H2 = H1 / 2, W2 = W1 / 2, Hc = H2 / 2, Wc = W2 / 2, cells = B * Hc * Wc;
     { ProfScope p(c, "conv1ab");
-      launch_conv1ab_fused(s, img, img_f32, stride, B, H, W, w.conv1a_w, w.bias[L_1A], w.packed[L_1B], w.bias[L_1B], b.p1, frame_step); }
-    { ProfScope p(c, "conv2a"); launch_conv3x3(s, b.p1, B, H1, W1, 64, w.packed[L_2A], w.bias[L_2A], 64, true, kSpLayers[L_2A].pool, b.a2, L_2A); }
-    { ProfScope p(c, "conv2b"); launch_conv3x3(s, b.a2, B, H1, W1, 64, w.packed[L_2B], w.bias[L_2B], 64, true, kSpLayers[L_2B].pool, b.p2, L_2B); }
-    { ProfScope p(c, "conv3a"); launch_conv3x3(s, b.p2, B, H2, W2, 64, w.packed[L_3A], w.bias[L_3A], 128, true, kSpLayers[L_3A].pool, b.a3, L_3A); }
-    { ProfScope p(c, "conv3b"); launch_conv3x3(s, b.a3, B, H2, W2, 128, w.packed[L_3B], w.bias[L_3B], 128, true, kSpLayers[L_3B].pool, b.p3, L_3B); }
-    { ProfScope p(c, "conv4a"); launch_conv3x3(s, b.p3, B, Hc, Wc, 128, w.packed[L_4A], w.bias[L_4A], 128, true, kSpLayers[L_4A].pool, b.a4, L_4A); }
-    { ProfScope p(c, "conv4b"); launch_conv3x3(s, b.a4, B, Hc, Wc, 128, w.packed[L_4B], w.bias[L_4B], 128, true, kSpLayers[L_4B].pool, b.f4, L_4B); }
+      launch_conv1ab_fused(s, img, img_f32, stride, B, H, W, w.conv1a_w, w.bias[L_1A], sp_conv_images(w, L_1B).frag, w.bias[L_1B], b.p1, frame_step); }
+    { ProfScope p(c, "conv2a"); launch_conv3x3(s, b.p1, B, H1, W1, 64, sp_conv_images(w, L_2A), w.bias[L_2A], 64, true, kSpLayers[L_2A].pool, b.a2, L_2A); }
+    { ProfScope p(c, "conv2b"); launch_conv3x3(s, b.a2, B, H1, W1, 64, sp_conv_images(w, L_2B), w.bias[L_2B], 64, true, kSpLayers[L_2B].pool, b.p2, L_2B); }
+    { ProfScope p(c, "conv3a"); launch_conv3x3(s, b.p2, B, H2, W2, 64, sp_conv_images(w, L_3A), w.bias[L_3A], 128, true, kSpLayers[L_3A].pool, b.a3, L_3A); }
+    { ProfScope p(c, "conv3b"); launch_conv3x3(s, b.a3, B, H2, W2, 128, sp_conv_images(w, L_3B), w.bias[L_3B], 128, true, kSpLayers[L_3B].pool, b.p3, L_3B); }
+    { ProfScope p(c, "conv4a"); launch_conv3x3(s, b.p3, B, Hc, Wc, 128, sp_conv_images(w, L_4A), w.bias[L_4A], 128, true, kSpLayers[L_4A].pool, b.a4, L_4A); }
+    { ProfScope p(c, "conv4b"); launch_conv3x3(s, b.a4, B, Hc, Wc, 128, sp_conv_images(w, L_4B), w.bias[L_4B], 128, true, kSpLayers[L_4B].pool, b.f4, L_4B); }
     const bool fork = !(c->prof && c->prof_filter.empty());
     hipStream_t sd = fork ? c->side_stream : s;
     if (fork) { RFE_HIP(c, hipEventRecord(c->ev_fork, s)); RFE_HIP(c, hipStreamWaitEvent(sd, c->ev_fork, 0)); }
-    { ProfScope p(c, "convDa", sd); launch_conv3x3(sd, b.f4, B, Hc, Wc, 128, w.packed[L_DA], w.bias[L_DA], 256, true, kSpLayers[L_DA].pool, b.da, L_DA); }
+    { ProfScope p(c, "convDa", sd); launch_conv3x3(sd, b.f4, B, Hc, Wc, 128, sp_conv_images(w, L_DA), w.bias[L_DA], 256, true, kSpLayers[L_DA].pool, b.da, L_DA); }
     { ProfScope p(c, "convDb", sd); launch_gemm_nt(sd, gemm_plain(b.da, 256, w.packed[L_DB], 256, w.bias[L_DB], b.dmap, 256, cells, 256, 256)); }
     { ProfScope p(c, "sp_post", sd); launch_descmap_norm(sd, b.dmap, cells); }
     if (fork) RFE_HIP(c, hipEventRecord(c->ev_join, sd));
-    { ProfScope p(c, "convPa"); launch_conv3x3(s, b.f4, B, Hc, Wc, 128, w.packed[L_PA], w.bias[L_PA], 256, true, kSpLayers[L_PA].pool, b.pa, L_PA); }
+    { ProfScope p(c, "convPa"); launch_conv3x3(s, b.f4, B, Hc, Wc, 128, sp_conv_images(w, L_PA), w.bias[L_PA], 256, true, kSpLayers[L_PA].pool, b.pa, L_PA); }
     { ProfScope p(c, "convPb"); launch_gemm_nt(s, gemm_plain(b.pa, 256, w.packed[L_PB], 256, w.bias[L_PB], b.logits, 65, cells, 65, 256)); }
     { ProfScope p(c, "sp_post");
       if (B <= 4 && c->hp.sp_nms_radius == 4) {
diff --git a/rover-slam_amd/csrc/api_hooks.hip b/rover-slam_amd/csrc/api_hooks.hip
--- a/rover-slam_amd/csrc/api_hooks.hip
+++ b/rover-slam_amd/csrc/api_hooks.hip
@@ -3,10 +3,13 @@
 
 using namespace rfe;
 
-extern "C" int rfe_k_conv3x3(rfe_ctx* c, const float* in, int B, int H, int W, int Cin, const float* w, const float* bias,
-                             int Cout, int relu, int pool, float* out) {
+static int k_conv3x3(rfe_ctx* c, const float* in, int B, int H, int W, int Cin, const float* w, const float* bias,
+                     int Cout, int relu, int pool, float* out, int tiles) {
     if (!c) return RFE_ERR_INVALID;
     if ((Cin != 16 && Cin != 32 && Cin != 64 && Cin != 128) || (Cout % 64)) return fail(c, RFE_ERR_INVALID, "k_conv3x3: Cin in {16,32,64,128}, Cout % 64 == 0");
+    if (tiles < CONV_TILES_AUTO || tiles > CONV_TILES_COMP) return fail(c, RFE_ERR_INVALID, "k_conv3x3: tiles in 0..2");
+    if (tiles == CONV_TILES_COMP && !conv3x3_comp_ok(B, H, W, Cin, relu != 0, pool != 0))
+        return fail(c, RFE_ERR_INVALID, "k_conv3x3: the composite tiles take 128 input channels, ReLU, no pool, B >= 2, even H >= 8, W >= 32, a ragged map");
     RFE_HIP(c, hipSetDevice(c->device));
     std::vector<float> packed;
     pack_conv3x3_weights(w, Cin, Cout, pool != 0, packed);
@@ -15,10 +18,31 @@
     if (rc) return rc;
     RFE_HIP(c, hipMemcpyAsync(dw, packed.data(), packed.size() * 4, hipMemcpyHostToDevice, c->stream));
     RFE_HIP(c, hipMemcpyAsync(db, bias, (size_t)Cout * 4, hipMemcpyHostToDevice, c->stream));
-    launch_conv3x3(c->stream, in, B, H, W, Cin, dw, db, Cout, relu != 0, pool != 0, out, 0);
+    launch_conv3x3(c->stream, in, B, H, W, Cin, conv3x3_images(dw, conv3x3_image_layout(Cin, Cout, pool != 0)), db, Cout, relu != 0, pool != 0, out, 0, tiles);
     RFE_HIP(c, hipGetLastError());
     RFE_HIP(c, hipStreamSynchronize(c->stream));
     return RFE_OK;
+}
+extern "C" int rfe_k_conv3x3(rfe_ctx* c, const float* in, int B, int H, int W, int Cin, const float* w, const float* bias,
+                             int Cout, int relu, int pool, float* out) {
+    return k_conv3x3(c, in, B, H, W, Cin, w, bias, Cout, relu, pool, out, CONV_TILES_AUTO);
+}
+extern "C" int rfe_k_conv3x3_tiles(rfe_ctx* c, const float* in, int B, int H, int W, int Cin, const float* w, const float* bias,
+                                   int Cout, int relu, int pool, int tiles, float* out) {
+    return k_conv3x3(c, in, B, H, W, Cin, w, bias, Cout, relu, pool, out, tiles);
+}
+
+extern "C" int64_t rfe_k_pack_conv3x3(const float* w, int Cin, int Cout, int pool, int image, float* out, int64_t capacity) {
+    if (!w || (Cin != 16 && Cin != 32 && Cin != 64 && Cin != 128) || Cout <= 0 || (Cout % 64) || image < 0 || image > 2) return RFE_ERR_INVALID;
+    const ConvImageLayout lay = conv3x3_image_layout(Cin, Cout, pool != 0);
+    const size_t off = image == 0 ? lay.frag : image == 1 ? lay.rows : lay.t16;
+    if (off == ConvImageLayout::none) return 0;
+    const int64_t n = (int64_t)Cout * Cin * 9;
+    if (!out || capacity < n) return RFE_ERR_INVALID;
+    std::vector<float> packed;
+    pack_conv3x3_weights(w, Cin, Cout, pool != 0, packed);
+    std::copy(packed.begin() + off, packed.begin() + off + n, out);
+    return n;
 }
 
 extern "C" int rfe_k_linear(rfe_ctx* c, const float* a, int M, int K, const float* w, const float* bias, int N, int relu,
diff --git a/rover-slam_amd/csrc/api_weights.hip b/rover-slam_amd/csrc/api_weights.hip
--- a/rover-slam_amd/csrc/api_weights.hip
+++ b/rover-slam_amd/csrc/api_weights.hip
@@ -91,7 +91,7 @@
             if ((rc = upload(c, &c->sp.conv1a_w, t.data(), t.size()))) return rc;
         } else if (L.k == 3) {
             std::vector<float> t;
-            pack_conv3x3_weights(w, L.cin, L.cout, L.pool, t);
+            pack_conv3x3_weights(w, L.cin, L.cout, L.pool, t, l == L_1B);
             if ((rc = upload(c, &c->sp.packed[l], t.data(), t.size()))) return rc;
         } else {
             if ((rc = upload(c, &c->sp.packed[l], w, wn))) return rc;
diff --git a/rover-slam_amd/csrc/rfe_internal.h b/rover-slam_amd/csrc/rfe_internal.h
--- a/rover-slam_amd/csrc/rfe_internal.h
+++ b/rover-slam_amd/csrc/rfe_internal.h
@@ -137,14 +137,31 @@
 
 int ensure_ws(rfe_ctx* c, void** p, size_t* cur, size_t need);
 
+struct ConvImageLayout {
+    static constexpr size_t none = ~(size_t)0;
+    size_t frag = 0, rows = none, t16 = none, count = 0;
+};
+struct ConvImages { const float* frag = nullptr; const float* rows = nullptr; const float* t16 = nullptr; };
 bool conv3x3_reads_t16(int cin, int cout, bool pool);
-void pack_conv3x3_weights(const float* w_oihw, int cin, int cout, bool pool, std::vector<float>& out);
-size_t packed_conv3x3_count(int cin, int cout, bool pool);
+ConvImageLayout conv3x3_image_layout(int cin, int cout, bool pool, bool fused_only = false);
+inline ConvImages conv3x3_images(const float* base, const ConvImageLayout& l) {
+    ConvImages im;
+    im.frag = base + l.frag;
+    if (l.rows != ConvImageLayout::none) im.rows = base + l.rows;
+    if (l.t16 != ConvImageLayout::none) im.t16 = base + l.t16;
+    return im;
+}
+inline ConvImages sp_conv_images(const SpWeightsDev& w, int l) {
+    return conv3x3_images(w.packed[l], conv3x3_image_layout(kSpLayers[l].cin, kSpLayers[l].cout, kSpLayers[l].pool, l == L_1B));
+}
+void pack_conv3x3_weights(const float* w_oihw, int cin, int cout, bool pool, std::vector<float>& out, bool fused_only = false);
+enum { CONV_TILES_AUTO = 0, CONV_TILES_PLAIN = 1, CONV_TILES_COMP = 2 };
+bool conv3x3_comp_ok(int B, int H, int W, int cin, bool relu, bool pool);
 void launch_conv3x3(hipStream_t s, const float* in, int B, int H, int W, int cin,
-                    const float* wpacked, const float* bias, int cout, bool relu, bool pool, float* out,
-                    int tag = 0);
+                    const ConvImages& wpacked, const float* bias, int cout, bool relu, bool pool, float* out,
+                    int tag = 0, int tiles = CONV_TILES_AUTO);
 void launch_conv1ab_fused(hipStream_t s, const void* img, bool img_f32, int stride, int B, int H, int W, const float* w1a,
-                          const float* b1a, const float* wp, const float* bias, float* out, long long frame_step = 0 );
+                          const float* b1a, const float* wp_frag, const float* bias, float* out, long long frame_step = 0 );
 inline void ensure_dynamic_lds(const void* kernel, int bytes, bool* done) {
     int dev = 0;
     (void)hipGetDevice(&dev);
diff --git a/rover-slam_amd/csrc/sp_conv.hip b/rover-slam_amd/csrc/sp_conv.hip
--- a/rover-slam_amd/csrc/sp_conv.hip
+++ b/rover-slam_amd/csrc/sp_conv.hip
@@ -10,21 +10,43 @@
 
 constexpr int CK = CONV_CK;
 
-size_t packed_conv3x3_count(int cin, int cout, bool pool) { return (size_t)cout * cin * 9 * (conv3x3_reads_t16(cin, cout, pool) ? 2 : 1); }
-
-void pack_conv3x3_weights(const float* w, int cin, int cout, bool pool, std::vector<float>& out) {
-    out.assign(packed_conv3x3_count(cin, cout, pool), 0.f);
+ConvImageLayout conv3x3_image_layout(int cin, int cout, bool pool, bool fused_only) {
+    const size_t n = (size_t)cout * cin * 9;
+    ConvImageLayout l;
+    l.frag = 0; l.count = n;
+    if (!fused_only && (cin == 64 || cin == 128)) { l.rows = l.count; l.count += n; }
+    if (!fused_only && conv3x3_reads_t16(cin, cout, pool)) { l.t16 = l.count; l.count += n; }
+    return l;
+}
+
+void pack_conv3x3_weights(const float* w, int cin, int cout, bool pool, std::vector<float>& out, bool fused_only) {
+    const ConvImageLayout lay = conv3x3_image_layout(cin, cout, pool, fused_only);
+    out.assign(lay.count, 0.f);
     const int KCH = CK * 9;
     const int nch = cin / CK, nct = cout / NT;
+    float* frag = out.data() + lay.frag;
     for (int ct = 0; ct < nct; ++ct)
         for (int ch = 0; ch < nch; ++ch)
-            for (int kl = 0; kl < KCH; ++kl)
-                for (int j = 0; j < NT; ++j) {
-                    int co = ct * NT + j, ci = ch * CK + kl / 9, tap = kl % 9;
-                    out[(((size_t)ct * nch + ch) * KCH + kl) * NT + j] = w[((size_t)co * cin + ci) * 9 + tap];
-                }
-    if (!conv3x3_reads_t16(cin, cout, pool)) return;
-    float* t16 = out.data() + (size_t)cout * cin * 9;
+            for (int g = 0; g < 9; ++g)
+                for (int nb = 0; nb < 2; ++nb)
+                    for (int lane = 0; lane < 64; ++lane)
+                        for (int i = 0; i < 4; ++i) {
+                            const int hh = lane >> 5, col = lane & 31, kap = 2 * (4 * g + i) + hh;
+                            const int co = ct * NT + 32 * nb + col, ci = ch * CK + kap / 9, tap = kap % 9;
+                            frag[((((((size_t)ct * nch + ch) * 9 + g) * 2 + nb) * 64 + lane) * 4) + i] = w[((size_t)co * cin + ci) * 9 + tap];
+                        }
+    if (lay.rows != ConvImageLayout::none) {
+        float* rows = out.data() + lay.rows;
+        for (int ct = 0; ct < nct; ++ct)
+            for (int ch = 0; ch < nch; ++ch)
+                for (int kl = 0; kl < KCH; ++kl)
+                    for (int j = 0; j < NT; ++j) {
+                        int co = ct * NT + j, ci = ch * CK + kl / 9, tap = kl % 9;
+                        rows[(((size_t)ct * nch + ch) * KCH + kl) * NT + j] = w[((size_t)co * cin + ci) * 9 + tap];
+                    }
+    }
+    if (lay.t16 == ConvImageLayout::none) return;
+    float* t16 = out.data() + lay.t16;
     const int nst = cin / 16;
     for (int b = 0; b < cout / 16; ++b)
         for (int st = 0; st < nst; ++st)
@@ -48,22 +70,32 @@
 }
 
 template <int PLANE_ = PLANE, int BLK1_ = TWS>
-__device__ __forceinline__ void conv_chunk_mma(const float* lds_in, const float* lds_w, const int (&aoff)[9], int boff,
+__device__ __forceinline__ void conv_chunk_mma(const float* lds_in, const float* lds_w, const int (&aoff)[9], int lane,
                                                f32x16 (&acc)[2][2]) {
-#pragma unroll 1
-    for (int cp = 0; cp < CK / 2; ++cp) {
-        const float* ap = lds_in + cp * 2 * PLANE_;
-        const float* bp = lds_w + cp * 18 * NT + boff;
-#pragma unroll
-        for (int s = 0; s < 9; ++s) {
-            const float a0 = ap[aoff[s]], a1 = ap[aoff[s] + BLK1_];
-            const float b0 = bp[2 * s * NT], b1 = bp[2 * s * NT + 32];
-            acc[0][0] = __builtin_amdgcn_mfma_f32_32x32x2f32(a0, b0, acc[0][0], 0, 0, 0);
-            acc[0][1] = __builtin_amdgcn_mfma_f32_32x32x2f32(a0, b1, acc[0][1], 0, 0, 0);
-            acc[1][0] = __builtin_amdgcn_mfma_f32_32x32x2f32(a1, b0, acc[1][0], 0, 0, 0);
-            acc[1][1] = __builtin_amdgcn_mfma_f32_32x32x2f32(a1, b1, acc[1][1], 0, 0, 0);
-        }
-    }
+    const f32x4* wf = reinterpret_cast<const f32x4*>(lds_w) + lane;
+    f32x4 w0 = wf[0], w1 = wf[64];
+#pragma unroll
+    for (int g = 0; g < 9; ++g) {
+        f32x4 n0 = w0, n1 = w1;
+        if (g + 1 < 9) { n0 = wf[(2 * g + 2) * 64]; n1 = wf[(2 * g + 3) * 64]; }
+#pragma unroll
+        for (int i = 0; i < 4; ++i) {
+            const int s36 = 4 * g + i;
+            const float* ap = lds_in + (s36 / 9) * 2 * PLANE_;
+            const float a0 = ap[aoff[s36 % 9]], a1 = ap[aoff[s36 % 9] + BLK1_];
+            acc[0][0] = __builtin_amdgcn_mfma_f32_32x32x2f32(a0, w0[i], acc[0][0], 0, 0, 0);
+            acc[0][1] = __builtin_amdgcn_mfma_f32_32x32x2f32(a0, w1[i], acc[0][1], 0, 0, 0);
+            acc[1][0] = __builtin_amdgcn_mfma_f32_32x32x2f32(a1, w0[i], acc[1][0], 0, 0, 0);
+            acc[1][1] = __builtin_amdgcn_mfma_f32_32x32x2f32(a1, w1[i], acc[1][1], 0, 0, 0);
+        }
+        w0 = n0; w1 = n1;
+    }
+}
+
+__device__ __forceinline__ int conv_lane_again() {
+    int l;
+    asm volatile("v_mbcnt_lo_u32_b32 %0, -1, 0\n\tv_mbcnt_hi_u32_b32 %0, -1, %0" : "=v"(l));
+    return l;
 }
 
 __device__ __forceinline__ void conv_stage_weights(float* lds_w, const float* src_chunk, int tid) {
@@ -127,7 +159,7 @@
 static inline unsigned conv_grid(int gx, int gy, int B, int nct) { return (unsigned)(((gx * gy * B + 7) / 8) * 8 * nct); }
 
 template <int CIN, bool POOL, bool RELU, int TAG>
-__global__ __launch_bounds__(256, 2) void conv3x3_mfma_kernel(
+__global__ __launch_bounds__(256, 4) void conv3x3_mfma_kernel(
     const float* __restrict__ in, const float* __restrict__ wp, const float* __restrict__ bias,
     float* __restrict__ out, int H, int W, int COUT, int gx, int gy, int ntiles) {
     constexpr int KCH = CK * 9;
@@ -153,7 +185,6 @@
     }
     int aoff[9];
     conv_a_offsets(aoff, h, wave, col);
-    const int boff = h * NT + col;
 
     const float* in_b = in + (size_t)b * H * W * CIN;
     const float* wp_ct = wp + (size_t)ct * (CIN / CK) * KCH * NT;
@@ -195,9 +226,10 @@
         }
         conv_stage_weights(lds_w, wp_ct + (size_t)ch * KCH * NT, tid);
         __syncthreads();
-        conv_chunk_mma(lds_in, lds_w, aoff, boff, acc);
-    }
-    conv_store<POOL, RELU>(acc, out, b, H, W, COUT, x0, y0, co0, wave, col, h);
+        conv_chunk_mma(lds_in, lds_w, aoff, lane, acc);
+    }
+    const int el = conv_lane_again();
+    conv_store<POOL, RELU>(acc, out, b, H, W, COUT, x0, y0, co0, wave, el & 31, el >> 5);
 }
 
 constexpr int STH = 4, SNT = 32;
@@ -343,7 +375,6 @@
         for (int c4 = 0; c4 < 4; ++c4) poff[c4][s9] = p * T16_CK + e + ((c4 ^ ((p >> 2) & 3)) << 2);
     }
     const float* in_b = in + (size_t)b * H * W * CIN;
-    const float* wp_t16 = wp + (size_t)COUT * CIN * 9;
     constexpr int NSLOT = 9 * NB, WCP = (NSLOT + 3) / 4, BLK_W = 9 * 256;
     int w_slot[WCP];
     const float* w_src[WCP];
@@ -351,7 +382,7 @@
     for (int u = 0; u < WCP; ++u) {
         w_slot[u] = wave + 4 * u < NSLOT ? wave + 4 * u : wave + 4 * (u - 1);
         const int nbk = w_slot[u] / 9, gs = w_slot[u] % 9;
-        w_src[u] = wp_t16 + ((size_t)(ct * NB + nbk) * NST) * BLK_W + gs * 256 + lane * 4;
+        w_src[u] = wp + ((size_t)(ct * NB + nbk) * NST) * BLK_W + gs * 256 + lane * 4;
     }
     const float* i_src[2];
     bool i_img[2];
@@ -438,7 +469,7 @@
 
 constexpr int CIH = TH + 4, CIW = TW + 4, CPLANE = CIH * CIW;
 template <int CIN, bool RELU, int TAG>
-__global__ __launch_bounds__(256, 2) void conv3x3_comp_kernel(
+__global__ __launch_bounds__(256, 4) void conv3x3_comp_kernel(
     const float* __restrict__ in, const float* __restrict__ wp, const float* __restrict__ bias,
     float* __restrict__ out, int B, int H, int W, int COUT, int gx, int gy, int ntiles) {
     constexpr int KCH = CK * 9;
@@ -477,7 +508,6 @@
             aoff[s] = (h ? o1 : o0) + base;
         }
     }
-    const int boff = h * NT + col;
     const float* wp_ct = wp + (size_t)ct * (CIN / CK) * KCH * NT;
 
     constexpr int S_IT = (CIH * CIW * (CK / 4) + 255) / 256;
@@ -517,21 +547,22 @@
         }
         conv_stage_weights(lds_w, wp_ct + (size_t)ch * KCH * NT, tid);
         __syncthreads();
-        conv_chunk_mma<CPLANE, CIW>(lds_in, lds_w, aoff, boff, acc);
-    }
+        conv_chunk_mma<CPLANE, CIW>(lds_in, lds_w, aoff, lane, acc);
+    }
+    const int el = conv_lane_again(), ecol = el & 31, eh = el >> 5;
 #pragma unroll
     for (int mb = 0; mb < 2; ++mb) {
         const int r = 2 * wave + mb, pr = r >= rb;
         const int y = pr ? r - rb : yin + r;
 #pragma unroll
         for (int q = 0; q < 16; ++q) {
-            const int c = (q & 3) + 8 * (q >> 2) + 4 * h, pc = c >= cb;
+            const int c = (q & 3) + 8 * (q >> 2) + 4 * eh, pc = c >= cb;
             const int x = pc ? c - cb : xin + c;
             const int f = frame_of(pr, pc);
             if (f < 0) continue;
             float v0 = acc[mb][0][q], v1 = acc[mb][1][q];
             if (RELU) { v0 = fmaxf(v0, 0.f); v1 = fmaxf(v1, 0.f); }
-            float* o = out + (((size_t)f * H + y) * W + x) * COUT + co0 + col;
+            float* o = out + (((size_t)f * H + y) * W + x) * COUT + co0 + ecol;
             o[0] = v0; o[32] = v1;
         }
     }
@@ -544,7 +575,7 @@
 }
 
 template <typename PX>
-__global__ __launch_bounds__(256, 2) void conv1ab_fused_kernel(
+__global__ __launch_bounds__(256, 4) void conv1ab_fused_kernel(
     const PX* __restrict__ img, int stride, const float* __restrict__ w1a , const float* __restrict__ b1a,
     const float* __restrict__ wp, const float* __restrict__ bias, float* __restrict__ out, int H, int W, long long frame_step ) {
     constexpr int CIN = 64, COUT = 64, KCH = CK * 9;
@@ -569,7 +600,6 @@
     }
     int aoff[9];
     conv_a_offsets(aoff, h, wave, col);
-    const int boff = h * NT + col;
 
     const PX* im = img + (long long)b * frame_step;
     for (int idx = tid; idx < MH * MW; idx += 256) {
@@ -610,9 +640,10 @@
         }
         conv_stage_weights(lds_w, wp + (size_t)ch * KCH * NT, tid);
         __syncthreads();
-        conv_chunk_mma(lds_in, lds_w, aoff, boff, acc);
-    }
-    conv_store<true, true>(acc, out, b, H, W, COUT, x0, y0, 0, wave, col, h);
+        conv_chunk_mma(lds_in, lds_w, aoff, lane, acc);
+    }
+    const int el = conv_lane_again();
+    conv_store<true, true>(acc, out, b, H, W, COUT, x0, y0, 0, wave, el & 31, el >> 5);
 }
 
 void launch_conv1ab_fused(hipStream_t s, const void* img, bool img_f32, int stride, int B, int H, int W, const float* w1a,
@@ -624,18 +655,23 @@
 }
 
 #define RFE_CONV_LAUNCH(CIN, POOL, RELU, TAG)                                                                            \
-    hipLaunchKernelGGL((conv3x3_mfma_kernel<CIN, POOL, RELU, TAG>), dim3(conv_grid(gx, gy, B, cout / NT)), dim3(256), 0, s, in, wp, bias, out, H, W, cout, gx, gy, gx * gy * B)
+    hipLaunchKernelGGL((conv3x3_mfma_kernel<CIN, POOL, RELU, TAG>), dim3(conv_grid(gx, gy, B, cout / NT)), dim3(256), 0, s, in, wp.frag, bias, out, H, W, cout, gx, gy, gx * gy * B)
 
 constexpr int CONV_T16_PX = 12000, CONV_T16_PX64 = 20000, CONV_T16P_PX128 = 20000;
 
 bool conv3x3_reads_t16(int cin, int cout, bool pool) { return (cin == 128 || (cin == 64 && !pool)) && cout % T16_NC == 0; }
 
-void launch_conv3x3(hipStream_t s, const float* in, int B, int H, int W, int cin, const float* wp,
-                    const float* bias, int cout, bool relu, bool pool, float* out, int tag) {
+bool conv3x3_comp_ok(int B, int H, int W, int cin, bool relu, bool pool) {
+    return !pool && relu && cin == 128 && B >= 2 && H % 2 == 0 && W >= TW && H >= TH && (H % TH != 0 || W % TW != 0) && (long long)B * H * W * cin < (1ll << 31);
+}
+
+void launch_conv3x3(hipStream_t s, const float* in, int B, int H, int W, int cin, const ConvImages& wp,
+                    const float* bias, int cout, bool relu, bool pool, float* out, int tag, int tiles) {
     const int gx = (W + TW - 1) / TW, gy = (H + TH - 1) / TH;
     const long long px = (long long)B * H * W;
+    if (tiles == CONV_TILES_COMP) tag = L_4A;
     constexpr int CONV_SMALL = 700;
-    const bool small = (long long)gx * gy * B * (cout / NT) < CONV_SMALL && (cin == 64 || cin == 128);
+    const bool small = tiles == CONV_TILES_AUTO && (long long)gx * gy * B * (cout / NT) < CONV_SMALL && (cin == 64 || cin == 128);
     if (small && relu && !pool && px <= (cin == 64 ? CONV_T16_PX64 : CONV_T16_PX) && cout % T16_NC == 0) {
         const int sx = (W + T16_W - 1) / T16_W, sy = (H + T16_H - 1) / T16_H;
         constexpr int CONV_T16_NC16 = 1000;
@@ -644,7 +680,7 @@
             constexpr int b16 = 3 * (T16D_PIX * T16_CK + T16D_WROWS * 16) * 4;
             static bool l16_[64];
             ensure_dynamic_lds((const void*)conv3x3_t16d_kernel<128, true, 16>, b16, l16_);
-            hipLaunchKernelGGL((conv3x3_t16d_kernel<128, true, 16>), g16, dim3(256), b16, s, in, wp, bias, out, H, W, cout, sx, sy, sx * sy * B);
+            hipLaunchKernelGGL((conv3x3_t16d_kernel<128, true, 16>), g16, dim3(256), b16, s, in, wp.t16, bias, out, H, W, cout, sx, sy, sx * sy * B);
             return;
         }
         const dim3 gs(conv_grid(sx, sy, B, cout / T16_NC));
@@ -652,44 +688,42 @@
         static bool ls_[2][64];
         if (cin == 128) {
             ensure_dynamic_lds((const void*)conv3x3_t16d_kernel<128, true>, bytes, ls_[0]);
-            hipLaunchKernelGGL((conv3x3_t16d_kernel<128, true>), gs, dim3(256), bytes, s, in, wp, bias, out, H, W, cout, sx, sy, sx * sy * B);
+            hipLaunchKernelGGL((conv3x3_t16d_kernel<128, true>), gs, dim3(256), bytes, s, in, wp.t16, bias, out, H, W, cout, sx, sy, sx * sy * B);
         } else {
             ensure_dynamic_lds((const void*)conv3x3_t16d_kernel<64, true>, bytes, ls_[1]);
-            hipLaunchKernelGGL((conv3x3_t16d_kernel<64, true>), gs, dim3(256), bytes, s, in, wp, bias, out, H, W, cout, sx, sy, sx * sy * B);
+            hipLaunchKernelGGL((conv3x3_t16d_kernel<64, true>), gs, dim3(256), bytes, s, in, wp.t16, bias, out, H, W, cout, sx, sy, sx * sy * B);
         }
         return;
     }
-    if (relu && pool && cin == 128 && px <= CONV_T16P_PX128 && cout % T16_NC == 0 && H % 2 == 0 && W % 2 == 0) {
+    if (tiles == CONV_TILES_AUTO && relu && pool && cin == 128 && px <= CONV_T16P_PX128 && cout % T16_NC == 0 && H % 2 == 0 && W % 2 == 0) {
         const int sx = (W + T16_W - 1) / T16_W, sy = (H + T16_H - 1) / T16_H;
         constexpr int b16 = 3 * (T16D_PIX * T16_CK + T16D_WROWS * 16) * 4;
         static bool lp_[64];
         ensure_dynamic_lds((const void*)conv3x3_t16d_kernel<128, true, 16, true>, b16, lp_);
-        hipLaunchKernelGGL((conv3x3_t16d_kernel<128, true, 16, true>), dim3(conv_grid(sx, sy, B, cout / 16)), dim3(256), b16, s, in, wp, bias, out, H, W, cout, sx, sy, sx * sy * B);
+        hipLaunchKernelGGL((conv3x3_t16d_kernel<128, true, 16, true>), dim3(conv_grid(sx, sy, B, cout / 16)), dim3(256), b16, s, in, wp.t16, bias, out, H, W, cout, sx, sy, sx * sy * B);
         return;
     }
     if (small && (!pool || relu)) {
         const int sx = (W + TW - 1) / TW, sy = (H + STH - 1) / STH;
         const dim3 gs(conv_grid(sx, sy, B, cout / SNT));
         if (pool) {
-            if (cin == 128) hipLaunchKernelGGL((conv3x3_small_kernel<128, true, true>), gs, dim3(256), 0, s, in, wp, bias, out, H, W, cout, sx, sy, sx * sy * B);
-            else hipLaunchKernelGGL((conv3x3_small_kernel<64, true, true>), gs, dim3(256), 0, s, in, wp, bias, out, H, W, cout, sx, sy, sx * sy * B);
-        }
-        else if (cin == 128 && relu) hipLaunchKernelGGL((conv3x3_small_kernel<128, true>), gs, dim3(256), 0, s, in, wp, bias, out, H, W, cout, sx, sy, sx * sy * B);
-        else if (cin == 128) hipLaunchKernelGGL((conv3x3_small_kernel<128, false>), gs, dim3(256), 0, s, in, wp, bias, out, H, W, cout, sx, sy, sx * sy * B);
-        else if (relu) hipLaunchKernelGGL((conv3x3_small_kernel<64, true>), gs, dim3(256), 0, s, in, wp, bias, out, H, W, cout, sx, sy, sx * sy * B);
-        else hipLaunchKernelGGL((conv3x3_small_kernel<64, false>), gs, dim3(256), 0, s, in, wp, bias, out, H, W, cout, sx, sy, sx * sy * B);
+            if (cin == 128) hipLaunchKernelGGL((conv3x3_small_kernel<128, true, true>), gs, dim3(256), 0, s, in, wp.rows, bias, out, H, W, cout, sx, sy, sx * sy * B);
+            else hipLaunchKernelGGL((conv3x3_small_kernel<64, true, true>), gs, dim3(256), 0, s, in, wp.rows, bias, out, H, W, cout, sx, sy, sx * sy * B);
+        }
+        else if (cin == 128 && relu) hipLaunchKernelGGL((conv3x3_small_kernel<128, true>), gs, dim3(256), 0, s, in, wp.rows, bias, out, H, W, cout, sx, sy, sx * sy * B);
+        else if (cin == 128) hipLaunchKernelGGL((conv3x3_small_kernel<128, false>), gs, dim3(256), 0, s, in, wp.rows, bias, out, H, W, cout, sx, sy, sx * sy * B);
+        else if (relu) hipLaunchKernelGGL((conv3x3_small_kernel<64, true>), gs, dim3(256), 0, s, in, wp.rows, bias, out, H, W, cout, sx, sy, sx * sy * B);
+        else hipLaunchKernelGGL((conv3x3_small_kernel<64, false>), gs, dim3(256), 0, s, in, wp.rows, bias, out, H, W, cout, sx, sy, sx * sy * B);
         return;
     }
-    if (!pool && relu && cin == 128 && (tag == L_4A || tag == L_4B || tag == L_PA || tag == L_DA) && B >= 2 &&
-        H % 2 == 0 && W >= TW && H >= TH && (H % TH != 0 || W % TW != 0) &&
-        (long long)B * H * W * cin < (1ll << 31)) {
+    if (tiles != CONV_TILES_PLAIN && (tag == L_4A || tag == L_4B || tag == L_PA || tag == L_DA) && conv3x3_comp_ok(B, H, W, cin, relu, pool)) {
         const int cx = (2 * W + TW - 1) / TW, cy = (((B + 1) / 2) * H + TH - 1) / TH;
         const dim3 gc(conv_grid(cx, cy, 1, cout / NT));
         switch (tag) {
-            case L_4A: hipLaunchKernelGGL((conv3x3_comp_kernel<128, true, L_4A>), gc, dim3(256), 0, s, in, wp, bias, out, B, H, W, cout, cx, cy, cx * cy); return;
-            case L_4B: hipLaunchKernelGGL((conv3x3_comp_kernel<128, true, L_4B>), gc, dim3(256), 0, s, in, wp, bias, out, B, H, W, cout, cx, cy, cx * cy); return;
-            case L_PA: hipLaunchKernelGGL((conv3x3_comp_kernel<128, true, L_PA>), gc, dim3(256), 0, s, in, wp, bias, out, B, H, W, cout, cx, cy, cx * cy); return;
-            default: hipLaunchKernelGGL((conv3x3_comp_kernel<128, true, L_DA>), gc, dim3(256), 0, s, in, wp, bias, out, B, H, W, cout, cx, cy, cx * cy); return;
+            case L_4A: hipLaunchKernelGGL((conv3x3_comp_kernel<128, true, L_4A>), gc, dim3(256), 0, s, in, wp.frag, bias, out, B, H, W, cout, cx, cy, cx * cy); return;
+            case L_4B: hipLaunchKernelGGL((conv3x3_comp_kernel<128, true, L_4B>), gc, dim3(256), 0, s, in, wp.frag, bias, out, B, H, W, cout, cx, cy, cx * cy); return;
+            case L_PA: hipLaunchKernelGGL((conv3x3_comp_kernel<128, true, L_PA>), gc, dim3(256), 0, s, in, wp.frag, bias, out, B, H, W, cout, cx, cy, cx * cy); return;
+            default: hipLaunchKernelGGL((conv3x3_comp_kernel<128, true, L_DA>), gc, dim3(256), 0, s, in, wp.frag, bias, out, B, H, W, cout, cx, cy, cx * cy); return;
         }
     }
     switch (tag) {
```

Result: no change. 939.4 frames/s (-0.6%).
